# parthjaggi/flow

Hardware: AMD Instinct MI355X
Metric: env-steps/sec (higher is better)
Workload: dtype mixed

## Files before the change

flow_amd/build.py:

```python
import concurrent.futures
import hashlib
import os
import shutil
import subprocess

PKG = os.path.dirname(os.path.abspath(__file__))
ROOT = os.path.dirname(PKG)
CSRC = os.path.join(PKG, "csrc")
SRC = os.path.join(CSRC, "flowsim.hip")
PART = os.path.join(CSRC, "flowsim_part.hip")
OBJ = os.path.join(CSRC, "_obj")
LIB = os.path.join(PKG, "libflowsim.so")

VALIDATED_ROCM = "7.2"

HEADERS = ["flowsim_sim.h", "flowsim_launch.h", "flowsim_kernels.h", "flowsim_open.h", "flowsim_wide.h",
           "flowsim_pair.h", "flowsim_pair_step_a.inc", "flowsim_pair_step_a_sm.inc", "flowsim_fig8.h", "flowsim_ringrl.h", "flowsim_policy.h", "flowsim_queue.h", "flowsim_queue_consts.h", "flowsim_dropq.h",
           "flowsim_part.hip"]
DEPS = [SRC] + [os.path.join(CSRC, h) for h in HEADERS] + [os.path.join(ROOT, "include", "flowsim.h")]
assert all(os.path.exists(d) for d in DEPS)
_known = set(os.path.basename(d) for d in DEPS)
assert all(f in _known for f in os.listdir(CSRC) if f.endswith((".h", ".inc", ".hip"))), "flow_amd/build.py: a source under csrc/ is not in DEPS"

COMMON_FLAGS = ["--offload-arch=gfx950", "-O3", "-ffp-contract=off", "-std=c++17", "-Wall", "-Wno-unused-function"]
HIPCC_FLAGS = COMMON_FLAGS + ["-fPIC", "-shared"]


def parts():
    out = [("main", SRC, [])]
    for t, tn in (("float", "f32"), ("double", "f64")):
        for seg in (8, 16, 32, 64):
            out.append(("seg%d_%s" % (seg, tn), PART, ["-DFS_PART_T=" + t, "-DFS_PART_SEG=%d" % seg]))
        for w in (2, 4):
            out.append(("wide%d_%s" % (w, tn), PART, ["-DFS_PART_T=" + t, "-DFS_PART_WIDE=%d" % w]))
    out.append(("queue_f32", PART, ["-DFS_PART_T=float", "-DFS_PART_QUEUE=1"] +
                (["-DFS_QDIAG=1"] if os.environ.get("FLOWSIM_QDIAG") else [])))
    return out


def find_hipcc():
    for cand in (os.environ.get("HIPCC"), shutil.which("hipcc"), "/opt/rocm/bin/hipcc"):
        if cand and os.path.exists(cand):
            return cand
    raise RuntimeError("hipcc not found: libflowsim.so cannot be built (no CPU fallback exists)")


def include_flags():
    return ["-I" + os.path.join(ROOT, "include"), "-I" + CSRC]


def _stamp(extra):
    h = hashlib.sha256()
    for d in DEPS:
        h.update(os.path.relpath(d, ROOT).encode())
        with open(d, "rb") as f:
            h.update(hashlib.sha256(f.read()).digest())
    h.update(" ".join(COMMON_FLAGS + extra).encode())
    return h.hexdigest()[:16]


def _have_stamp(out):
    if not (os.path.exists(out) and os.path.exists(out + ".stamp")):
        return None
    with open(out + ".stamp") as f:
        return f.read().strip()


def needs_build():
    if not os.path.exists(LIB):
        return True
    t = os.path.getmtime(LIB)
    if any(os.path.getmtime(d) > t for d in DEPS):
        return True
    return any(_have_stamp(os.path.join(OBJ, name + ".o")) != _stamp(extra) for name, _, extra in parts())


def _compile(job):
    name, src, extra, out, verbose = job
    cmd = [find_hipcc()] + COMMON_FLAGS + ["-fPIC", "-c"] + extra + include_flags() + ["-o", out + ".tmp", src]
    if verbose:
        print(" ".join(cmd), flush=True)
    res = subprocess.run(cmd, capture_output=True, text=True)
    if res.returncode != 0:
        raise RuntimeError("hipcc failed (%s):\n%s%s" % (name, res.stdout, res.stderr))
    os.replace(out + ".tmp", out)
    return out


def _jobs():
    return max(1, min(len(parts()), int(os.environ.get("FLOWSIM_BUILD_JOBS", os.cpu_count() or 4))))


def build_variant(lib, defines, names=None, verbose=False):
    build()
    obj_dir = os.path.join(OBJ, os.path.basename(lib))
    os.makedirs(obj_dir, exist_ok=True)
    objs, todo = [], []
    for name, src, extra in parts():
        if names and name not in names:
            objs.append(os.path.join(OBJ, name + ".o"))
            continue
        out = os.path.join(obj_dir, name + ".o")
        objs.append(out)
        todo.append((name, src, extra + list(defines), out, verbose))
    with concurrent.futures.ThreadPoolExecutor(_jobs()) as pool:
        list(pool.map(_compile, todo))
    res = subprocess.run([find_hipcc(), "--offload-arch=gfx950", "-shared", "-fPIC", "-o", lib] + objs,
                         capture_output=True, text=True)
    if res.returncode != 0:
        raise RuntimeError("hipcc link failed:\n" + res.stdout + res.stderr)
    return lib


def build(force=False, verbose=False, only=None):
    if not force and not only and not needs_build():
        return LIB
    os.makedirs(OBJ, exist_ok=True)
    objs, todo, stamps = [], [], {}
    for name, src, extra in parts():
        out = os.path.join(OBJ, name + ".o")
        stamp, have = _stamp(extra), _have_stamp(out)
        objs.append(out)
        if force or (only and name in only) or (not only and have != stamp) or not os.path.exists(out):
            todo.append((name, src, extra, out, verbose))
            stamps[out] = stamp
    with concurrent.futures.ThreadPoolExecutor(_jobs()) as pool:
        for out in pool.map(_compile, todo):
            with open(out + ".stamp", "w") as f:
                f.write(stamps[out])
    cmd = [find_hipcc(), "--offload-arch=gfx950", "-shared", "-fPIC", "-o", LIB + ".tmp"] + objs
    if verbose:
        print(" ".join(cmd), flush=True)
    res = subprocess.run(cmd, capture_output=True, text=True)
    if res.returncode != 0:
        raise RuntimeError("hipcc link failed:\n" + res.stdout + res.stderr)
    os.replace(LIB + ".tmp", LIB)
    return LIB


USER_DIR = os.path.join(PKG, "_user")
USER_SIGNATURE = ("template <typename T>\n__device__ __forceinline__ T fs_user_accel(T v, T v_lead, T h, bool has_lead, "
                  "T v_follow, T h_follow, T dt, T max_accel, const T* p)")


def user_header(body):
    body = "\n".join("  " + ln.strip() for ln in str(body).strip().splitlines())
    return ("// generated by flow_amd.build.build_user -- the get_accel of a flow_amd.controllers.CompiledController\n"
            "%s {\n%s\n}\n" % (USER_SIGNATURE, body))


def build_user(body, verbose=False):
    text = user_header(body)
    tag = hashlib.sha256((text + _stamp([])).encode()).hexdigest()[:16]
    out_dir = os.path.join(USER_DIR, tag)
    lib = os.path.join(out_dir, "libflowsim.so")
    if os.path.exists(lib):
        return lib
    build()
    if not all(os.path.exists(os.path.join(OBJ, name + ".o")) for name, _, _ in parts()):
        build(force=True)
    os.makedirs(out_dir, exist_ok=True)
    for stale in os.listdir(USER_DIR):
        tagfile = os.path.join(USER_DIR, stale, "sources.stamp")
        if stale != tag and os.path.exists(tagfile) and open(tagfile).read().strip() != _stamp([]):
            shutil.rmtree(os.path.join(USER_DIR, stale), ignore_errors=True)
    with open(os.path.join(out_dir, "sources.stamp"), "w") as f:
        f.write(_stamp([]))
    hdr = os.path.join(out_dir, "user_controller.h")
    with open(hdr, "w") as f:
        f.write(text)
    objs, todo = [], []
    for name, src, extra in parts():
        if name.startswith("queue"):
            objs.append(os.path.join(OBJ, name + ".o"))
            continue
        out = os.path.join(out_dir, name + ".o")
        objs.append(out)
        todo.append((name, src, extra + ['-DFS_USER_CONTROLLER_HEADER="%s"' % hdr], out, verbose))
    with concurrent.futures.ThreadPoolExecutor(_jobs()) as pool:
        list(pool.map(_compile, todo))
    res = subprocess.run([find_hipcc(), "--offload-arch=gfx950", "-shared", "-fPIC", "-o", lib + ".tmp"] + objs,
                         capture_output=True, text=True)
    if res.returncode != 0:
        raise RuntimeError("hipcc link failed:\n" + res.stdout + res.stderr)
    os.replace(lib + ".tmp", lib)
    for job in todo:
        os.remove(job[3])
    return lib


def device_asm(out_dir, names=None):
    os.makedirs(out_dir, exist_ok=True)
    jobs = []
    for name, src, extra in parts():
        if names and name not in names:
            continue
        out = os.path.join(out_dir, name + ".s")
        jobs.append((name, [find_hipcc()] + COMMON_FLAGS + ["-S", "--cuda-device-only"] + extra + include_flags() +
                     ["-o", out, src], out))

    def run(job):
        res = subprocess.run(job[1], capture_output=True, text=True)
        if res.returncode != 0:
            raise RuntimeError("hipcc -S failed (%s):\n%s" % (job[0], res.stderr[-2000:]))
        return job[0], job[2]

    with concurrent.futures.ThreadPoolExecutor(_jobs()) as pool:
        return dict(pool.map(run, jobs))


if __name__ == "__main__":
    import sys
    print(build(force="--force" in sys.argv, verbose=True, only=[a for a in sys.argv[1:] if not a.startswith("-")]))
```

flow_amd/csrc/flowsim.hip:

```cpp
#include "flowsim_sim.h"

namespace fsim {

int validate(const fs_config* c) {
  if (!c) return fail(FS_ERR_INVALID, "fs_create: cfg is NULL");
  if (c->struct_size != sizeof(fs_config))
    return fail(FS_ERR_INVALID, "fs_create: struct_size mismatch (header/library out of sync)");
  if (c->abi_version != FS_ABI_VERSION) return fail(FS_ERR_INVALID, "fs_create: abi_version mismatch");
  if (c->precision != FS_F32 && c->precision != FS_F64 && c->precision != FS_MIXED && c->precision != FS_F16S)
    return fail(FS_ERR_INVALID, "fs_create: bad precision");
  if (c->precision == FS_F16S && (c->network != FS_NET_MERGE || c->num_vehicles > 64))
    return fail(FS_ERR_UNSUPPORTED, "fs_create: FS_F16S (half state, float32 integrator) is built for FS_NET_MERGE "
                                    "(k_steps_open, <= 64 vehicle slots)");
  if (c->precision == FS_MIXED && (c->network == FS_NET_MERGE || c->network == FS_NET_BOTTLENECK)) {
  } else if (c->precision == FS_MIXED) {
    const bool fig8 = c->network == FS_NET_FIGURE_EIGHT;
    const char* why = nullptr;
    if ((c->network != FS_NET_RING && !fig8) || c->num_lanes > 1) why = "network (single-lane ring or figure eight)";
    else if (c->env != FS_ENV_ACCEL && c->env != FS_ENV_WAVE_ATTENUATION_PO) why = "env (AccelEnv or WaveAttenuationPOEnv)";
    else if (c->evaluate) why = "evaluate";
    else if (c->sims_per_step != 1) why = "sims_per_step (1)";
    else if (c->integrator != FS_EULER) why = "integrator (Euler)";
    else if (c->junction_mode && !fig8) why = "junction_mode";
    else if (c->track_aux && !fig8) why = "track_aux (the scalar Env's previous-speed / acceleration fields: VecFlowEnv(track_aux=False))";
    else if (c->sort_vehicles || c->obs_perm) why = "sort_vehicles / shuffled ids";
    else if (!fig8 && (c->num_vehicles < 2 || c->num_vehicles > 64 || (c->num_vehicles % 2) != 0)) why = "num_vehicles (even, 2..64)";
    else if (!c->vehicles) why = "vehicles (NULL)";
    for (int i = 0; !why && i < c->num_vehicles; ++i) {
      const fs_vehicle_spec& v = c->vehicles[i];
      if (v.controller != FS_CTRL_IDM && v.controller != FS_CTRL_RL && !(fig8 && v.controller == FS_CTRL_SIM))
        why = "vehicles[].controller (IDMController / RLController)";
      else if (v.fail_safe != FS_FAILSAFE_NONE) why = "vehicles[].fail_safe";
    }
    if (why)
      return fail(FS_ERR_UNSUPPORTED, std::string("fs_create: FS_MIXED does not support this configuration: ") + why);
  }
  if (c->network < FS_NET_RING || c->network > FS_NET_BOTTLENECK)
    return fail(FS_ERR_UNSUPPORTED, "fs_create: network not built");
  const bool open_net = c->network == FS_NET_MERGE || c->network == FS_NET_BOTTLENECK;
  const bool merge_env = c->env == FS_ENV_MERGE_PO || c->env == FS_ENV_MERGE_MA;
  const bool bn_env = c->env == FS_ENV_BOTTLENECK_DV || c->env == FS_ENV_BOTTLENECK;
  if ((c->network == FS_NET_MERGE) != merge_env)
    return fail(FS_ERR_INVALID, "fs_create: the merge envs and FS_NET_MERGE go together");
  if (c->network == FS_NET_MERGE && !c->track_followers)
    return fail(FS_ERR_INVALID, "fs_create: the merge observations need track_followers = 1");
  if ((c->network == FS_NET_BOTTLENECK) != bn_env)
    return fail(FS_ERR_INVALID, "fs_create: the bottleneck envs and FS_NET_BOTTLENECK go together");
  if (c->network == FS_NET_BOTTLENECK) {
    if (c->num_vehicles <= 32)
      return fail(FS_ERR_UNSUPPORTED, "fs_create: the bottleneck heads need more than 32 vehicle slots per replica");
    if (!(c->merge1_x <= c->merge2_x) || !(c->merge2_x < c->end_x) || !(c->zipper_distance >= 0))
      return fail(FS_ERR_INVALID, "fs_create: need merge1_x <= merge2_x < end_x and zipper_distance >= 0");
    if (c->junction.enabled) return fail(FS_ERR_INVALID, "fs_create: the priority-junction model is for FS_NET_MERGE");
    if (c->obs_outflow_window < 1 || c->obs_outflow_window > 20 || c->reward_outflow_window < 1 ||
        c->reward_outflow_window > 20)
      return fail(FS_ERR_INVALID, "fs_create: outflow windows must be 1..20 sub-steps");
    if (c->evaluate) return fail(FS_ERR_UNSUPPORTED, "fs_create: evaluate mode of the bottleneck envs is not built");
    if (c->num_paths != 0 && c->num_paths != 4 && c->num_paths != 8)
      return fail(FS_ERR_UNSUPPORTED, "fs_create: num_paths (4 * scaling) must be 4 or 8");
    if (c->num_paths == 8 && c->num_vehicles <= 64)
      return fail(FS_ERR_UNSUPPORTED, "fs_create: num_paths = 8 (scaling 2) is built in the workgroup-per-replica kernel: "
                                      "more than 64 vehicle slots per replica");
    if (c->env == FS_ENV_BOTTLENECK_DV) {
      const int max_cells = c->num_vehicles > 64 ? 128 : 64;
      if (c->num_obs_cells < 1 || c->num_obs_cells > max_cells || !c->obs_cells)
        return fail(FS_ERR_INVALID, "fs_create: 1..64 observation cells (1..128 with more than 64 vehicle slots)");
      for (int k = 0; k < c->num_obs_cells; ++k)
        if (c->obs_cells[k].lane < 0 || c->obs_cells[k].lane > 63) return fail(FS_ERR_INVALID, "fs_create: cell lane");
      for (int k = 0; k < c->num_rl; ++k)
        if (c->act_cells && (c->act_cells[k].lane < 0 || c->act_cells[k].lane > 63))
          return fail(FS_ERR_INVALID, "fs_create: cell lane");
      if (c->num_rl < 0 || c->num_rl > 64 || (c->num_rl > 0 && !c->act_cells))
        return fail(FS_ERR_INVALID, "fs_create: 0..64 action cells");
    }
  }
  if (open_net) {
    if (c->num_lanes > 1) return fail(FS_ERR_UNSUPPORTED, "fs_create: multi-lane merge is not built");
    if (c->num_segments < 2 || c->num_segments > 2 * FS_MAX_SEGMENTS || !c->segments)
      return fail(FS_ERR_INVALID, "fs_create: FS_NET_MERGE needs the segment tables of both routes");
    int per_route[2] = {0, 0};
    for (int k = 0; k < c->num_segments; ++k) {
      const fs_segment& sg = c->segments[k];
      if (sg.route < 0 || sg.route > (c->network == FS_NET_MERGE ? 1 : 0))
        return fail(FS_ERR_INVALID, "fs_create: segment route out of range");
      if (k > 0 && sg.route < c->segments[k - 1].route)
        return fail(FS_ERR_INVALID, "fs_create: segment rows must be grouped by route");
      if (k > 0 && sg.route == c->segments[k - 1].route && !(sg.start > c->segments[k - 1].start))
        return fail(FS_ERR_INVALID, "fs_create: segment starts must increase");
      if (++per_route[sg.route] > FS_MAX_SEGMENTS) return fail(FS_ERR_INVALID, "fs_create: too many segments");
    }
    if (!per_route[0] || (c->network == FS_NET_MERGE && !per_route[1]))
      return fail(FS_ERR_INVALID, "fs_create: a route has no segment");
    if (c->num_inflows < 0 || c->num_inflows > FS_MAX_INFLOWS || (c->num_inflows > 0 && !c->inflows))
      return fail(FS_ERR_INVALID, "fs_create: bad inflow table");
    for (int f = 0; f < c->num_inflows; ++f) {
      const fs_inflow& fl = c->inflows[f];
      if (c->network == FS_NET_MERGE ? (fl.route < 0 || fl.route > 1)
                                     : (fl.route < -1 || fl.route > (c->num_paths == 8 ? 7 : 3)))
        return fail(FS_ERR_INVALID, "fs_create: inflow route out of range");
      if (fl.probability > 1.0) return fail(FS_ERR_INVALID, "fs_create: inflow probability > 1");
      if (!(fl.probability >= 0.0) && !(fl.period > 0)) return fail(FS_ERR_INVALID, "fs_create: inflow period <= 0");
      if (!(fl.depart_speed >= 0) || !(fl.depart_pos >= 0)) return fail(FS_ERR_INVALID, "fs_create: bad inflow departure");
      bool type_ok = false;
      for (int i = 0; i < c->num_vehicles; ++i) type_ok = type_ok || c->vehicles[i].type == fl.type;
      if (!type_ok) return fail(FS_ERR_INVALID, "fs_create: inflow of a vehicle type that has no slot");
    }
    if (!c->init_alive || !c->init_lane) return fail(FS_ERR_INVALID, "fs_create: FS_NET_MERGE needs init_alive and init_lane (routes)");
    if (!(c->box_in < c->merge_x) || !(c->merge_x < c->end_x) || !(c->net_length > 0))
      return fail(FS_ERR_INVALID, "fs_create: need box_in < merge_x < end_x and net_length > 0");
  }
  if (c->network == FS_NET_RING && (c->num_segments != 0 || c->junction.enabled))
    return fail(FS_ERR_INVALID, "fs_create: a ring takes no segment table / junction");
  if (c->network == FS_NET_FIGURE_EIGHT) {
    if (c->num_segments < 1 || c->num_segments > FS_MAX_SEGMENTS || !c->segments)
      return fail(FS_ERR_INVALID, "fs_create: figure eight needs 1..FS_MAX_SEGMENTS segments");
    if (c->num_lanes > 1) return fail(FS_ERR_UNSUPPORTED, "fs_create: multi-lane figure eight is not built");
    if (c->segments[0].start != 0.0) return fail(FS_ERR_INVALID, "fs_create: segment 0 must start at 0");
    for (int k = 1; k < c->num_segments; ++k)
      if (!(c->segments[k].start > c->segments[k - 1].start))
        return fail(FS_ERR_INVALID, "fs_create: segment starts must increase");
  }
  if (c->env < FS_ENV_ACCEL || c->env > FS_ENV_LANE_CHANGE_ACCEL_PO) return fail(FS_ERR_INVALID, "fs_create: bad env");
  const bool lc_env = c->env == FS_ENV_LANE_CHANGE_ACCEL || c->env == FS_ENV_LANE_CHANGE_ACCEL_PO;
  if (lc_env && c->network != FS_NET_RING)
    return fail(FS_ERR_UNSUPPORTED, "fs_create: the lane-change envs are built for rings (k_steps_ml)");
  if (c->env == FS_ENV_LANE_CHANGE_ACCEL_PO && (c->num_rl < 1 || c->obs_perm))
    return fail(FS_ERR_INVALID, "fs_create: LaneChangeAccelPOEnv needs an RL vehicle and takes no observation permutation");
  if (c->env == FS_ENV_WAVE_ATTENUATION_PO_MA || c->env == FS_ENV_ACCEL_PO_MA) {
    if (open_net || c->num_lanes > 1)
      return fail(FS_ERR_UNSUPPORTED, "fs_create: the multi-agent ring heads are built for single-lane closed loops");
    if (c->num_rl < 1) return fail(FS_ERR_INVALID, "fs_create: a multi-agent ring env needs an RL vehicle");
    if (c->sort_vehicles || c->obs_perm) return fail(FS_ERR_INVALID, "fs_create: sort_vehicles / shuffled ids belong to AccelEnv");
  }
  if (c->num_lanes > 1 && c->env == FS_ENV_WAVE_ATTENUATION_PO)
    return fail(FS_ERR_UNSUPPORTED, "fs_create: WaveAttenuationPOEnv on a multi-lane ring is not built");
  if (c->num_lanes > 64) return fail(FS_ERR_INVALID, "fs_create: num_lanes > 64");
  if (c->init_lane && !open_net)
    for (size_t e = 0; e < size_t(c->num_replicas > 0 ? c->num_replicas : 0) * (c->num_vehicles > 0 ? c->num_vehicles : 0); ++e)
      if (c->init_lane[e] < 0 || c->init_lane[e] >= (c->num_lanes < 1 ? 1 : c->num_lanes))
        return fail(FS_ERR_INVALID, "fs_create: init_lane out of range");
  if (c->num_replicas < 1) return fail(FS_ERR_INVALID, "fs_create: num_replicas < 1");
  if (c->replica_offset < 0) return fail(FS_ERR_INVALID, "fs_create: replica_offset < 0");
  if (c->sort_vehicles || c->obs_perm) {
    if (c->env != FS_ENV_ACCEL && !lc_env && c->sort_vehicles)
      return fail(FS_ERR_INVALID, "fs_create: sort_vehicles belongs to AccelEnv / LaneChangeAccelEnv");
    if (c->network == FS_NET_MERGE || c->network == FS_NET_BOTTLENECK ||
        (c->num_lanes > 1 && c->sort_vehicles && !lc_env))
      return fail(FS_ERR_UNSUPPORTED, "fs_create: sort_vehicles / shuffled ids are built for closed loops "
                                      "(sort_vehicles on multi-lane rings: LaneChangeAccelEnv)");
    if (c->obs_perm) {
      unsigned long long seen = 0ull;
      for (int i = 0; i < c->num_vehicles && i < 64; ++i) {
        const int q = c->obs_perm[i];
        if (q < 0 || q >= c->num_vehicles || (seen >> q) & 1ull)
          return fail(FS_ERR_INVALID, "fs_create: obs_perm is not a permutation");
        seen |= 1ull << q;
      }
    }
  }
  if (c->num_vehicles < 1) return fail(FS_ERR_INVALID, "fs_create: num_vehicles < 1");
  if (c->num_vehicles > 64 && c->network != FS_NET_BOTTLENECK)
    return fail(FS_ERR_UNSUPPORTED, "fs_create: more than 64 vehicles per replica is built for FS_NET_BOTTLENECK only");
  if (c->num_vehicles > FS_MAX_SLOTS_WIDE)
    return fail(FS_ERR_UNSUPPORTED, "fs_create: more than 256 vehicle slots per replica is not built");
  if (c->num_rl < 0 || (c->num_rl > c->num_vehicles && c->env != FS_ENV_BOTTLENECK_DV))
    return fail(FS_ERR_INVALID, "fs_create: bad num_rl");
  if (c->sims_per_step < 1) return fail(FS_ERR_INVALID, "fs_create: sims_per_step < 1");
  if (c->warmup_steps < 0) return fail(FS_ERR_INVALID, "fs_create: warmup_steps < 0");
  if (!(c->sim_step > 0)) return fail(FS_ERR_INVALID, "fs_create: sim_step <= 0");
  if (!(c->slowdown_ramp > 0) || c->slowdown_ramp > 1) return fail(FS_ERR_INVALID, "fs_create: slowdown_ramp not in (0,1]");
  if (c->junction_length < 0) return fail(FS_ERR_INVALID, "fs_create: junction_length < 0");
  if (!c->vehicles || (!c->ring_length && !open_net) || !c->init_pos)
    return fail(FS_ERR_INVALID, "fs_create: NULL table pointer");
  int seen_rl = 0;
  unsigned long long rl_mask = 0ull;
  for (int i = 0; i < c->num_vehicles; ++i) {
    const fs_vehicle_spec& v = c->vehicles[i];
    if (v.controller < FS_CTRL_SIM || v.controller > FS_CTRL_USER)
      return fail(FS_ERR_INVALID, "fs_create: unknown controller id");
    if (v.fail_safe < FS_FAILSAFE_NONE || v.fail_safe > FS_FAILSAFE_SAFE_VELOCITY)
      return fail(FS_ERR_INVALID, "fs_create: unknown fail_safe id");
    if (open_net && v.controller == FS_CTRL_PISATURATION)
      return fail(FS_ERR_UNSUPPORTED, "fs_create: PISaturation on an open network is not built");
    if (v.controller == FS_CTRL_RL && (c->env == FS_ENV_MERGE_PO || bn_env)) {
      ++seen_rl;
    } else if (v.controller == FS_CTRL_RL) {
      if (v.rl_index < 0 || v.rl_index >= c->num_rl) return fail(FS_ERR_INVALID, "fs_create: rl_index out of range");
      if (rl_mask & (1ull << v.rl_index)) return fail(FS_ERR_INVALID, "fs_create: rl_index used twice");
      rl_mask |= 1ull << v.rl_index;
      ++seen_rl;
    }
    if (!(v.length > 0)) return fail(FS_ERR_INVALID, "fs_create: vehicle length <= 0");
  }
  if (c->env == FS_ENV_MERGE_PO && c->num_rl > 32)
    return fail(FS_ERR_UNSUPPORTED, "fs_create: MergePOEnv with more than 32 controlled places (num_rl) is not built");
  if (seen_rl != c->num_rl && c->env != FS_ENV_MERGE_PO && !bn_env)
    return fail(FS_ERR_INVALID, "fs_create: num_rl does not match the RL slots");
  if (open_net) {
    for (size_t e = 0; e < size_t(c->num_replicas) * c->num_vehicles; ++e) {
      if (!c->init_alive[e]) continue;
      const int rt = c->init_lane[e];
      if (rt < 0 || rt > (c->network == FS_NET_MERGE ? 1 : (c->num_paths == 8 ? 7 : 3)))
        return fail(FS_ERR_INVALID, "fs_create: initial route out of range");
      const double x = c->init_pos[e];
      if (!(x >= c->route_start[c->network == FS_NET_MERGE ? rt : 0]) || !(x < c->end_x))
        return fail(FS_ERR_INVALID, "fs_create: init_pos outside the route");
    }
    return FS_OK;
  }
  if (c->env == FS_ENV_WAVE_ATTENUATION_PO && c->num_rl < 1)
    return fail(FS_ERR_INVALID, "fs_create: WaveAttenuationPOEnv needs an RL vehicle");
  for (int r = 0; r < c->num_replicas; ++r) {
    double need = 0;
    for (int i = 0; i < c->num_vehicles; ++i) need += c->vehicles[i].length;
    const double L = c->ring_length[r] + 4 * c->junction_length;
    if (!(c->ring_length[r] > 0) || need > L * (c->num_lanes < 1 ? 1 : c->num_lanes))
      return fail(FS_ERR_NOSPACE, "fs_create: vehicles do not fit on the ring");
    for (int i = 0; i < c->num_vehicles; ++i) {
      const double x = c->init_pos[size_t(r) * c->num_vehicles + i];
      if (!(x >= 0) || !(x < L)) return fail(FS_ERR_INVALID, "fs_create: init_pos outside [0, length)");
    }
  }
  return FS_OK;
}

template <typename T>
int create_typed(const fs_config* cfg, fs_handle* out) {
  Sim<T>* s = new (std::nothrow) Sim<T>();
  if (!s) return fail(FS_ERR_HIP, "fs_create: out of host memory");
  s->cfg = *cfg;
  s->mixed = cfg->precision == FS_MIXED;
  s->f16s = cfg->precision == FS_F16S;
  s->veh.assign(cfg->vehicles, cfg->vehicles + cfg->num_vehicles);
  if (cfg->num_segments > 0) s->segs.assign(cfg->segments, cfg->segments + cfg->num_segments);
  if (cfg->obs_perm) s->obs_perm.assign(cfg->obs_perm, cfg->obs_perm + cfg->num_vehicles);
  if (cfg->network == FS_NET_MERGE || cfg->network == FS_NET_BOTTLENECK) {
    if (cfg->num_inflows > 0) s->inflows.assign(cfg->inflows, cfg->inflows + cfg->num_inflows);
    s->init_alive.assign(cfg->init_alive, cfg->init_alive + size_t(cfg->num_replicas) * cfg->num_vehicles);
    if (cfg->env == FS_ENV_BOTTLENECK_DV) {
      s->obs_cells.assign(cfg->obs_cells, cfg->obs_cells + cfg->num_obs_cells);
      if (cfg->num_rl > 0) s->act_cells.assign(cfg->act_cells, cfg->act_cells + cfg->num_rl);
    }
  }
  s->obs_dim = (cfg->env == FS_ENV_WAVE_ATTENUATION_PO) ? 3
               : (cfg->env == FS_ENV_WAVE_ATTENUATION_PO_MA) ? 3 * cfg->num_rl
               : (cfg->env == FS_ENV_ACCEL_PO_MA) ? 6 * cfg->num_rl
               : (cfg->env == FS_ENV_BOTTLENECK_DV) ? 4 * cfg->num_obs_cells + 1
               : (cfg->env == FS_ENV_BOTTLENECK) ? 1
               : (cfg->env == FS_ENV_MERGE_PO || cfg->env == FS_ENV_MERGE_MA)
                     ? 5 * cfg->num_rl
                     : (cfg->env == FS_ENV_LANE_CHANGE_ACCEL_PO)
                           ? (4 * (cfg->num_lanes < 1 ? 1 : cfg->num_lanes) + 1) * cfg->num_rl
                           : (cfg->env == FS_ENV_LANE_CHANGE_ACCEL ? 3 : 2) * cfg->num_vehicles;
  if (s->obs_dim < 1) s->obs_dim = 1;
  s->act_dim = cfg->num_rl * ((cfg->env == FS_ENV_LANE_CHANGE_ACCEL || cfg->env == FS_ENV_LANE_CHANGE_ACCEL_PO) ? 2 : 1);
  int seg = 8;
  while (seg < cfg->num_vehicles) seg <<= 1;
  s->seg = seg;
  hipError_t e = hipSetDevice(cfg->device);
  if (e == hipSuccess) e = hipStreamCreateWithFlags(&s->own_stream, hipStreamNonBlocking);
  if (e != hipSuccess) {
    delete s;
    return fail(FS_ERR_HIP, std::string("fs_create: no usable HIP device: ") + hipGetErrorString(e));
  }
  s->stream = s->own_stream;
  {
    const std::pair<const char*, bool SimBase::*> switches[] = {
        {"FLOWSIM_FORCE_GENERIC", &SimBase::force_generic}, {"FLOWSIM_NO_FASTDIV", &SimBase::no_fastdiv},
        {"FLOWSIM_NO_LOOP_KERNEL", &SimBase::no_loop_kernel}, {"FLOWSIM_NO_LOOP_FULL", &SimBase::no_loop_full},
        {"FLOWSIM_NO_RING_RL", &SimBase::no_ring_rl}, {"FLOWSIM_NO_QUEUE", &SimBase::no_queue},
        {"FLOWSIM_NO_PAIR", &SimBase::no_pair}};
    for (const auto& sw : switches) {
      const char* v = std::getenv(sw.first);
      s->*sw.second = v && v[0] == '1';
    }
  }
  int rc = s->init();
  if (rc == FS_OK) {
    hipError_t e2 = hipStreamSynchronize(s->stream);
    if (e2 != hipSuccess) rc = fail(FS_ERR_HIP, std::string("fs_create: ") + hipGetErrorString(e2));
  }
  if (rc != FS_OK) {
    for (void* p : s->allocs) (void)hipFree(p);
    (void)hipStreamDestroy(s->own_stream);
    delete s;
    return rc;
  }
  s->cfg.vehicles = nullptr;
  s->cfg.ring_length = nullptr;
  s->cfg.init_pos = nullptr;
  s->cfg.init_vel = nullptr;
  s->cfg.init_lane = nullptr;
  s->cfg.segments = nullptr;
  s->cfg.inflows = nullptr;
  s->cfg.init_alive = nullptr;
  s->cfg.obs_cells = nullptr;
  s->cfg.obs_perm = nullptr;
  s->cfg.act_cells = nullptr;
  *out = reinterpret_cast<fs_handle>(static_cast<SimBase*>(s));
  return FS_OK;
}

inline SimBase* S(fs_handle h) { return reinterpret_cast<SimBase*>(h); }

struct DeviceGuard {
  int prev = -1;
  bool switched = false;
  explicit DeviceGuard(int want) {
    if (hipGetDevice(&prev) == hipSuccess && prev != want) switched = hipSetDevice(want) == hipSuccess;
  }
  ~DeviceGuard() {
    if (switched) (void)hipSetDevice(prev);
  }
};

}

using namespace fsim;

extern "C" {

int fs_abi_version(void) { return FS_ABI_VERSION; }

const char* fs_last_error(void) { return g_err.c_str(); }

int fs_create(const fs_config* cfg, fs_handle* out) {
  if (!out) return fail(FS_ERR_INVALID, "fs_create: out is NULL");
  *out = nullptr;
  int rc = validate(cfg);
  if (rc) return rc;
  int prev = -1;
  const bool have_prev = hipGetDevice(&prev) == hipSuccess;
  rc = (cfg->precision == FS_F32 || cfg->precision == FS_F16S) ? create_typed<float>(cfg, out)
                                                                 : create_typed<double>(cfg, out);
  if (have_prev && prev != cfg->device) (void)hipSetDevice(prev);
  return rc;
}

void fs_destroy(fs_handle h) {
  if (!h) return;
  SimBase* s = S(h);
  DeviceGuard guard(s->cfg.device);
  (void)hipStreamSynchronize(s->stream);
  for (void* p : s->allocs) (void)hipFree(p);
  (void)hipStreamDestroy(s->own_stream);
  delete s;
}

int fs_obs_dim(fs_handle h) { return h ? S(h)->obs_dim : fail(FS_ERR_INVALID, "fs_obs_dim: NULL handle"); }

int fs_action_dim(fs_handle h) { return h ? S(h)->act_dim : fail(FS_ERR_INVALID, "fs_action_dim: NULL handle"); }

int fs_set_stream(fs_handle h, void* hip_stream) {
  if (!h) return fail(FS_ERR_INVALID, "fs_set_stream: NULL handle");
  SimBase* s = S(h);
  DeviceGuard guard(s->cfg.device);
  HIP_TRY(hipStreamSynchronize(s->stream));
  s->stream = static_cast<hipStream_t>(hip_stream);
  return FS_OK;
}

int fs_use_own_stream(fs_handle h) {
  if (!h) return fail(FS_ERR_INVALID, "fs_use_own_stream: NULL handle");
  SimBase* s = S(h);
  DeviceGuard guard(s->cfg.device);
  HIP_TRY(hipStreamSynchronize(s->stream));
  s->stream = s->own_stream;
  return FS_OK;
}

int fs_sync(fs_handle h) {
  if (!h) return fail(FS_ERR_INVALID, "fs_sync: NULL handle");
  DeviceGuard guard(S(h)->cfg.device);
  HIP_TRY(hipStreamSynchronize(S(h)->stream));
  return S(h)->check_qflag();
}

int fs_reset_dev(fs_handle h, const uint8_t* mask_dev, float* obs_dev) {
  if (!h) return fail(FS_ERR_INVALID, "fs_reset_dev: NULL handle");
  SimBase* s = S(h);
  DeviceGuard guard(s->cfg.device);
  int rc = s->launch_reset(mask_dev);
  if (rc) return rc;
  float* obs = obs_dev ? obs_dev : s->d_obs;
  if (s->cfg.network == FS_NET_MERGE || s->cfg.network == FS_NET_BOTTLENECK) {
    s->after_reset = 1;
    rc = s->launch_steps(0, mask_dev, nullptr, 0, obs, s->d_rew, s->d_done, 0);
    s->after_reset = 0;
    if (rc) return rc;
    if (s->cfg.warmup_steps > 0)
      return s->launch_steps(s->cfg.warmup_steps, mask_dev, nullptr, 0, obs, s->d_rew, s->d_done, 0);
    return FS_OK;
  }
  if (s->cfg.warmup_steps > 0)
    return s->launch_steps(s->cfg.warmup_steps, mask_dev, nullptr, 0, obs, s->d_rew, s->d_done, 0);
  return s->launch_steps(0, mask_dev, nullptr, 0, obs, s->d_rew, s->d_done, 0);
}

int fs_reset(fs_handle h, const uint8_t* mask, float* obs_out) {
  if (!h) return fail(FS_ERR_INVALID, "fs_reset: NULL handle");
  SimBase* s = S(h);
  DeviceGuard guard(s->cfg.device);
  const size_t R = size_t(s->cfg.num_replicas);
  const uint8_t* dmask = nullptr;
  if (mask) {
    HIP_TRY(hipMemcpyAsync(s->d_mask, mask, R, hipMemcpyHostToDevice, s->stream));
    dmask = s->d_mask;
  }
  int rc = fs_reset_dev(h, dmask, s->d_obs);
  if (rc) return rc;
  if (obs_out)
    HIP_TRY(hipMemcpyAsync(obs_out, s->d_obs, R * s->obs_dim * sizeof(float), hipMemcpyDeviceToHost, s->stream));
  HIP_TRY(hipStreamSynchronize(s->stream));
  return FS_OK;
}

int fs_step_dev(fs_handle h, const float* actions_dev, float* obs_dev, float* rew_dev, uint8_t* done_dev) {
  if (!h) return fail(FS_ERR_INVALID, "fs_step_dev: NULL handle");
  if (!obs_dev || !rew_dev || !done_dev) return fail(FS_ERR_INVALID, "fs_step_dev: NULL output pointer");
  DeviceGuard guard(S(h)->cfg.device);
  return S(h)->launch_steps(1, nullptr, actions_dev, 0, obs_dev, rew_dev, done_dev, 0);
}

int fs_step(fs_handle h, const float* actions, float* obs, float* rew, uint8_t* done) {
  if (!h) return fail(FS_ERR_INVALID, "fs_step: NULL handle");
  if (!obs || !rew || !done) return fail(FS_ERR_INVALID, "fs_step: NULL output pointer");
  SimBase* s = S(h);
  DeviceGuard guard(s->cfg.device);
  const size_t R = size_t(s->cfg.num_replicas);
  const float* dact = nullptr;
  if (actions && s->act_dim > 0) {
    HIP_TRY(hipMemcpyAsync(s->d_actions, actions, R * s->act_dim * sizeof(float), hipMemcpyHostToDevice, s->stream));
    dact = s->d_actions;
  }
  int rc = s->launch_steps(1, nullptr, dact, 0, s->d_obs, s->d_rew, s->d_done, 0);
  if (rc) return rc;
  HIP_TRY(hipMemcpyAsync(obs, s->d_obs, R * s->obs_dim * sizeof(float), hipMemcpyDeviceToHost, s->stream));
  HIP_TRY(hipMemcpyAsync(rew, s->d_rew, R * sizeof(float), hipMemcpyDeviceToHost, s->stream));
  HIP_TRY(hipMemcpyAsync(done, s->d_done, R, hipMemcpyDeviceToHost, s->stream));
  HIP_TRY(hipStreamSynchronize(s->stream));
  return s->check_qflag();
}

int fs_rollout_dev(fs_handle h, int num_steps, const float* actions_dev, size_t action_stride_steps,
                   float* obs_dev, float* rew_dev, uint8_t* done_dev, int obs_every_step) {
  if (!h) return fail(FS_ERR_INVALID, "fs_rollout_dev: NULL handle");
  if (num_steps < 1) return fail(FS_ERR_INVALID, "fs_rollout_dev: num_steps < 1");
  if (!obs_dev || !rew_dev || !done_dev) return fail(FS_ERR_INVALID, "fs_rollout_dev: NULL output pointer");
  DeviceGuard guard(S(h)->cfg.device);
  return S(h)->launch_steps(num_steps, nullptr, actions_dev, action_stride_steps, obs_dev, rew_dev, done_dev,
                            obs_every_step ? 1 : 0);
}

int fs_get_state(fs_handle h, int field, void* dst, size_t bytes) {
  if (!h || !dst) return fail(FS_ERR_INVALID, "fs_get_state: NULL argument");
  DeviceGuard guard(S(h)->cfg.device);
  return S(h)->get_state(field, dst, bytes);
}

int fs_set_state(fs_handle h, int field, const void* src, size_t bytes) {
  if (!h || !src) return fail(FS_ERR_INVALID, "fs_set_state: NULL argument");
  DeviceGuard guard(S(h)->cfg.device);
  return S(h)->set_state(field, src, bytes);
}

int fs_add_vehicle(fs_handle h, int replica, int slot, int route, double x, double speed) {
  if (!h) return fail(FS_ERR_INVALID, "fs_add_vehicle: NULL handle");
  DeviceGuard guard(S(h)->cfg.device);
  return S(h)->add_vehicle(replica, slot, route, x, speed);
}

int fs_policy_act_dev(fs_handle h, const fs_policy* pol, const float* obs_dev, float* act_dev, float* logp_dev) {
  if (!h || !pol || !obs_dev || !act_dev || !logp_dev) return fail(FS_ERR_INVALID, "fs_policy_act_dev: NULL argument");
  DeviceGuard guard(S(h)->cfg.device);
  return S(h)->launch_policy(pol, 0, 0, obs_dev, nullptr, act_dev, logp_dev, nullptr, nullptr);
}

int fs_policy_rollout_dev(fs_handle h, const fs_policy* pol, int num_steps, int reset_done, float* obs_dev,
                          float* act_dev, float* logp_dev, float* rew_dev, uint8_t* done_dev) {
  if (!h || !pol || !obs_dev || !act_dev || !logp_dev || !rew_dev || !done_dev)
    return fail(FS_ERR_INVALID, "fs_policy_rollout_dev: NULL argument");
  if (num_steps < 1) return fail(FS_ERR_INVALID, "fs_policy_rollout_dev: num_steps < 1");
  DeviceGuard guard(S(h)->cfg.device);
  return S(h)->launch_policy(pol, num_steps, reset_done ? 1 : 0, nullptr, obs_dev, act_dev, logp_dev, rew_dev, done_dev);
}

const char* fs_last_kernel(fs_handle h) { return h ? reinterpret_cast<SimBase*>(h)->last_kernel : ""; }

int fs_dump_trajectory(fs_handle h, int replica, const char* csv_path) {
  if (!h || !csv_path) return fail(FS_ERR_INVALID, "fs_dump_trajectory: NULL argument");
  SimBase* s = S(h);
  if (replica < 0 || replica >= s->cfg.num_replicas) return fail(FS_ERR_INVALID, "fs_dump_trajectory: replica out of range");
  DeviceGuard guard(s->cfg.device);
  const size_t R = size_t(s->cfg.num_replicas), N = size_t(s->cfg.num_vehicles);
  const bool f32 = s->cfg.precision == FS_F32 || s->cfg.precision == FS_F16S;
  const size_t el = f32 ? sizeof(float) : sizeof(double);
  std::vector<char> pos(R * N * el), vel(R * N * el);
  std::vector<int32_t> tc(R), lane(R * N, 0);
  int rc = s->get_state(FS_FIELD_POS, pos.data(), pos.size());
  if (!rc) rc = s->get_state(FS_FIELD_VEL, vel.data(), vel.size());
  if (!rc) rc = s->get_state(FS_FIELD_TIME, tc.data(), R * sizeof(int32_t));
  const bool open_net = s->cfg.network == FS_NET_MERGE || s->cfg.network == FS_NET_BOTTLENECK;
  if (!rc && (open_net || s->cfg.num_lanes > 1))
    rc = s->get_state(open_net ? FS_FIELD_ROUTE : FS_FIELD_LANE, lane.data(), R * N * sizeof(int32_t));
  if (rc) return rc;
  FILE* probe = std::fopen(csv_path, "r");
  const bool fresh = probe == nullptr;
  if (probe) std::fclose(probe);
  FILE* f = std::fopen(csv_path, "a");
  if (!f) return fail(FS_ERR_INVALID, std::string("fs_dump_trajectory: cannot open ") + csv_path);
  if (fresh) std::fprintf(f, "time,id,x,speed,lane_number\n");
  const double t = double(tc[replica]) * s->cfg.sim_step;
  for (size_t i = 0; i < N; ++i) {
    const size_t e = size_t(replica) * N + i;
    if (open_net && lane[e] < 0) continue;
    const double x = f32 ? double(reinterpret_cast<const float*>(pos.data())[e]) : reinterpret_cast<const double*>(pos.data())[e];
    const double v = f32 ? double(reinterpret_cast<const float*>(vel.data())[e]) : reinterpret_cast<const double*>(vel.data())[e];
    std::fprintf(f, "%.6f,%zu,%.17g,%.17g,%d\n", t, i, x, v, int(lane[e]));
  }
  std::fclose(f);
  return FS_OK;
}

}
```

flow_amd/csrc/flowsim_launch.h:

```cpp
#pragma once
#include "flowsim_sim.h"
#ifdef FS_PART_QUEUE
#include "flowsim_queue.h"
#include "flowsim_dropq.h"
#endif

namespace fsim {

#ifdef FS_PART_QUEUE
  template <typename T>
  int Sim<T>::launch_queue(const StepArgs& a) {
    const bool po = dv.env == FS_ENV_MERGE_PO;
    const bool noise = (dv.flags & fs::FLAG_HAS_NOISE) != 0, act = a.actions != nullptr && (po || ov.ma_apply_actions != 0);
    const auto k = pick(noise, [&](auto NZ) {
      return pick(act, [&](auto ACT) {
        return pick(po, [&](auto PO) { return &fs::k_merge_queue<NZ, ACT, false, PO>; });
      });
    });
    last_kernel = "k_merge_queue";
    hipLaunchKernelGGL(k, dim3(dv.R), dim3(64), 0, stream, dv, ov, qc, a.num_steps, a.actions, a.act_stride, a.obs, a.rew,
                       a.done, a.obs_every_step, fs::PolicyView{}, static_cast<float*>(nullptr), static_cast<float*>(nullptr),
                       0);
    return launched();
  }
  template <typename T>
  int Sim<T>::launch_policy_queue(const fs::PolicyView& pv, int num_steps, int reset_done, float* obs, float* act,
                                  float* logp, float* rew, uint8_t* done) {
    const bool noise = (dv.flags & fs::FLAG_HAS_NOISE) != 0;
    if (dv.env == FS_ENV_MERGE_PO) {
      const auto kp = pick(noise, [&](auto NZ) { return &fs::k_merge_policy<NZ>; });
      last_kernel = "k_merge_policy<PO>";
      hipLaunchKernelGGL(kp, dim3(dv.R), dim3(64), 0, stream, dv, ov, qc, num_steps, obs, rew, done, pv, act, logp,
                         reset_done);
      return launched();
    }
    const auto k = pick(noise, [&](auto NZ) { return &fs::k_merge_queue<NZ, true, true>; });
    last_kernel = "k_merge_policy";
    hipLaunchKernelGGL(k, dim3(dv.R), dim3(64), 0, stream, dv, ov, qc, num_steps, static_cast<const float*>(nullptr),
                       size_t(0), obs, rew, done, 1, pv, act, logp, reset_done);
    return launched();
  }
  template <typename T>
  int Sim<T>::launch_policy_act_vec(const fs::PolicyView& pv, const float* obs_in, float* act, float* logp) {
    last_kernel = "k_policy_act_vec";
    hipLaunchKernelGGL(fs::k_policy_act_vec<16>, dim3(dv.R), dim3(64), 0, stream, pv, dv.R, dv.num_rl, dv.rep0, obs_in,
                       act, logp);
    return launched();
  }
  template <typename T>
  int Sim<T>::launch_dropq(const StepArgs& a) {
    const auto k = dv.env == FS_ENV_BOTTLENECK_DV ? &fs::k_drop_queue<true> : &fs::k_drop_queue<false>;
    last_kernel = "k_drop_queue";
    qflag_armed = true;
    hipLaunchKernelGGL(k, dim3(dv.R), dim3(256), 0, stream, dv, ov, qc, d_qflag, a.num_steps, a.actions, a.act_stride,
                       a.obs, a.rew, a.done, a.obs_every_step);
    return launched();
  }
#endif

  template <typename T>
  template <int W>
  int Sim<T>::launch_wide(const StepArgs& a) {
    constexpr int C1 = std::is_same<T, float>::value ? 1 : 0;
    const bool cset = C1 == 1 && (dv.flags & fs::FLAG_IDM_SET) && !force_generic && open_div_ok;
    const auto k = cfg.num_paths == 8 ? (cset ? &fs::k_steps_wide<T, W, C1, 8> : &fs::k_steps_wide<T, W, 0, 8>)
                                      : (cset ? &fs::k_steps_wide<T, W, C1, 4> : &fs::k_steps_wide<T, W, 0, 4>);
    last_kernel = "k_steps_wide";
    hipLaunchKernelGGL(k, dim3(dv.R), dim3(64 * W), 0, stream, dv, ov, a.num_steps, a.mask, a.actions, a.act_stride, a.obs,
                       a.rew, a.done, a.obs_every_step, after_reset);
    return launched();
  }

  template <typename T>
  template <int SEG>
  int Sim<T>::launch_open(const StepArgs& a) {
    constexpr int RPW = 64 / SEG;
    const bool idm_set = (dv.flags & fs::FLAG_IDM_SET) && !force_generic;
    const bool cset = std::is_same<T, float>::value ? idm_set && open_div_ok : idm_set && !mixed;
    const bool mset = mixed && idm_set && open_div_ok;
    constexpr int C2 = std::is_same<T, double>::value ? 2 : 0;
    auto kernel = [&](auto P, auto PO) {
      return pick(ov.n_prob > 0, [&](auto PR) {
        return cset ? &fs::k_steps_open<T, SEG, P, 1, PR, PO>
                    : mset ? &fs::k_steps_open<T, SEG, P, C2, PR, PO> : &fs::k_steps_open<T, SEG, P, 0, PR, PO>;
      });
    };
    decltype(kernel(Int<2>(), std::false_type())) k;
    last_kernel = "k_steps_open";
    if (cfg.network == FS_NET_BOTTLENECK) {
      if constexpr (SEG == 64) k = kernel(Int<4>(), std::false_type());
      else return fail(FS_ERR_UNSUPPORTED, "fs_step: FS_NET_BOTTLENECK runs on 64-lane segments only");
    } else {
      k = pick(dv.env == FS_ENV_MERGE_PO, [&](auto PO) { return kernel(Int<2>(), PO); });
      if (mset) last_kernel = "k_steps_open<mixed>";
    }
    hipLaunchKernelGGL(k, dim3((dv.R + RPW - 1) / RPW), dim3(64), 0, stream, dv, ov, a.num_steps, a.mask, a.actions,
                       a.act_stride, a.obs, a.rew, a.done, a.obs_every_step, after_reset);
    return launched();
  }

  template <typename T>
  template <int SEG>
  int Sim<T>::launch_ml(const StepArgs& a) {
    constexpr int RPW = 64 / SEG;
    const bool lcpo = dv.env == FS_ENV_LANE_CHANGE_ACCEL_PO;
    const auto k = pick(dv.lc_enabled, [&](auto LC) {
      return pick(lcpo, [&](auto PO) { return &fs::k_steps_ml<T, SEG, LC, PO>; });
    });
    last_kernel = "k_steps_ml";
    hipLaunchKernelGGL(k, dim3((dv.R + RPW - 1) / RPW), dim3(64), 0, stream, dv, a.num_steps, a.mask, a.actions,
                       a.act_stride, a.obs, a.rew, a.done, a.obs_every_step);
    return launched();
  }

  template <typename T>
  int Sim<T>::launch_loop(const StepArgs& a) {
    constexpr bool MX = !std::is_same<T, float>::value;
    const int f = dv.flags;
    const bool full = (f & fs::FLAG_HAS_NOISE) && (f & fs::FLAG_NEED_SUMO) && dv.junction_on && a.actions != nullptr &&
                      loop_delta4 && !no_loop_full && loop_fastc_ok();
    auto kernel = [&](auto H) {
      return full ? &fs::k_rollout_loop<H, true, true, MX>
                  : loop_delta4 ? &fs::k_rollout_loop<H, true, false, MX> : &fs::k_rollout_loop<H, false, false, MX>;
    };
    auto k = dv.env == FS_ENV_ACCEL ? kernel(Int<0>()) : kernel(Int<1>());
    last_kernel = full ? "k_rollout_loop<FULL>" : "k_rollout_loop";
    if constexpr (!MX) {
      if (dv.env == FS_ENV_ACCEL_PO_MA) {
        k = kernel(Int<2>());
        last_kernel = full ? "k_rollout_loop<FULL,AccelMA>" : "k_rollout_loop<AccelMA>";
      }
    }
    const int waves = (dv.R + 3) / 4;
    hipLaunchKernelGGL(k, dim3((waves + 3) / 4), dim3(256), 0, stream, dv, a.num_steps, a.actions, a.act_stride, a.obs,
                       a.rew, a.done);
    return launched();
  }

  template <typename T>
  template <int SEG>
  int Sim<T>::launch_ring(const StepArgs& a) {
    constexpr int ROW = SEG >= 16 ? SEG / 2 : 8;
    const bool fast = ringrl_fast_ok();
    const bool po = dv.env == FS_ENV_WAVE_ATTENUATION_PO;
    const bool ma_head = dv.env == FS_ENV_WAVE_ATTENUATION_PO_MA || dv.env == FS_ENV_ACCEL_PO_MA;
    const bool mc = ROW == 16 && std::is_same<T, float>::value && (ma_head || (a.actions != nullptr && dv.num_rl > 1));
    auto kernel = [&](auto H, auto MC) {
      return pick(dv.flags & fs::FLAG_HAS_NOISE, [&](auto NZ) {
        return pick(fast, [&](auto FA) { return &fs::k_ring_pair<T, ROW, H, NZ, FA, MC>; });
      });
    };
    auto single = [&](auto MC) { return po ? kernel(Int<1>(), MC) : kernel(Int<0>(), MC); };
    decltype(single(std::false_type())) k;
    if constexpr (std::is_same<T, float>::value && ROW == 16) {
      const auto MC = std::true_type();
      k = !ma_head ? pick(mc, single) : dv.env == FS_ENV_ACCEL_PO_MA ? kernel(Int<3>(), MC) : kernel(Int<2>(), MC);
    } else if constexpr (std::is_same<T, float>::value) {
      const auto MC = std::false_type();
      k = !ma_head ? single(MC) : dv.env == FS_ENV_ACCEL_PO_MA ? kernel(Int<3>(), MC) : kernel(Int<2>(), MC);
    } else {
      k = single(std::false_type());
    }
    last_kernel = ma_head ? (dv.env == FS_ENV_ACCEL_PO_MA ? "k_ring_pair<AccelMA>" : "k_ring_pair<POMA>")
                          : (po ? "k_ring_pair<PO>" : "k_ring_pair<Accel>");
    const int waves = (dv.R + (64 / ROW) - 1) / (64 / ROW);
    hipLaunchKernelGGL(k, dim3((waves + 3) / 4), dim3(256), 0, stream, dv, a.num_steps, a.mask, a.actions, a.act_stride,
                       a.obs, a.rew, a.done, a.obs_every_step);
    return launched();
  }

  template <typename T>
  int Sim<T>::launch_obs_mixed(const StepArgs& a) {
    if constexpr (std::is_same<T, double>::value) {
      const int n = dv.R * dv.N;
      last_kernel = "k_obs_mixed";
      hipLaunchKernelGGL((fs::k_obs_mixed<T>), dim3((n + 255) / 256), dim3(256), 0, stream, dv, a.obs);
      return launched();
    } else {
      return fail(FS_ERR_UNSUPPORTED, "k_obs_mixed is a float64 kernel");
    }
  }

  template <typename T>
  template <int SEG>
  int Sim<T>::launch_pair(const StepArgs& a) {
    constexpr int ROW = SEG >= 16 ? SEG / 2 : 8;
    const bool fd = fastdiv_ok(), bc = neg_speed_possible, sm = speed_mode_any;
    const bool noise = std::is_same<T, float>::value && (dv.flags & fs::FLAG_HAS_NOISE);
    auto clamped = [&](auto SM, auto NZ) {
      return delta4 && fd && !bc ? &fs::k_rollout_pair<T, ROW, true, true, false, SM, NZ>
                                 : &fs::k_rollout_pair<T, ROW, false, false, true, SM, NZ>;
    };
    decltype(&fs::k_rollout_pair<T, ROW, false, false, true>) k = nullptr;
    if (noise) {
      if constexpr (std::is_same<T, float>::value) k = pick(sm, [&](auto SM) { return clamped(SM, std::true_type()); });
    } else if (sm) {
      k = clamped(std::true_type(), std::false_type());
    } else {
      k = pick(bc, [&](auto BC) {
        return delta4 && fd ? &fs::k_rollout_pair<T, ROW, true, true, BC>
                            : delta4 ? &fs::k_rollout_pair<T, ROW, true, false, BC> : &fs::k_rollout_pair<T, ROW, false, false, BC>;
      });
    }
    last_kernel = noise ? (sm ? "k_rollout_pair+speed_mode+noise" : "k_rollout_pair+noise")
                        : (sm ? "k_rollout_pair+speed_mode" : "k_rollout_pair");
    const int waves = (dv.R + (64 / ROW) - 1) / (64 / ROW);
    hipLaunchKernelGGL(k, dim3((waves + 3) / 4), dim3(256), 0, stream, dv, a.num_steps, a.obs, a.rew, a.done);
    return launched();
  }

  template <typename T>
  template <int SEG>
  int Sim<T>::launch_idm(const StepArgs& a) {
    constexpr int RPW = 64 / SEG;
    const bool fd = fastdiv_ok();
    const auto k = pick(neg_speed_possible, [&](auto BC) {
      return delta4 && fd ? &fs::k_rollout_idm<T, SEG, true, true, BC>
                          : delta4 ? &fs::k_rollout_idm<T, SEG, true, false, BC> : &fs::k_rollout_idm<T, SEG, false, false, BC>;
    });
    last_kernel = "k_rollout_idm";
    const int waves = (dv.R + RPW - 1) / RPW;
    hipLaunchKernelGGL(k, dim3((waves + 7) / 8), dim3(512), 0, stream, dv, a.num_steps, a.obs, a.rew, a.done, d_dump);
    return launched();
  }

  template <typename T>
  template <int SEG>
  int Sim<T>::launch_k_steps(const StepArgs& a) {
    constexpr int RPW = 64 / SEG;
    auto k = &fs::k_steps<T, SEG, 0, 0>;
    last_kernel = "k_steps";
    if (fast_ok(a)) {
      k = &fs::k_steps<T, SEG, 1, 0>;
      last_kernel = "k_steps<FAST>";
    } else if ((dv.flags & fs::FLAG_IDM_SET) && !force_generic) {
      k = &fs::k_steps<T, SEG, 0, 1>;
      last_kernel = "k_steps<CSET>";
    }
    hipLaunchKernelGGL(k, dim3((dv.R + RPW - 1) / RPW), dim3(64), 0, stream, dv, a.num_steps, a.mask, a.actions,
                       a.act_stride, a.obs, a.rew, a.done, a.obs_every_step);
    return launched();
  }

  template <typename T>
  int Sim<T>::launch_policy_act(const fs::PolicyView& pv, int n_ag, const float* obs_in, float* act, float* logp) {
    last_kernel = "k_policy_act";
    const bool merge = dv.env == FS_ENV_MERGE_MA;
    hipLaunchKernelGGL(fs::k_policy_act<16>, dim3((dv.R * 16 + 255) / 256), dim3(256), 0, stream, pv, dv.R, n_ag, dv.rep0,
                       obs_in, act, logp, merge ? static_cast<const int*>(dv.lane) : nullptr,
                       merge ? static_cast<const int*>(dv.ctrl) : nullptr,
                       merge ? static_cast<const int*>(dv.rl_index) : nullptr, dv.N);
    return launched();
  }

  template <typename T>
  int Sim<T>::launch_policy_row16(const fs::PolicyView& pv, int num_steps, int reset_done, float* obs, float* act,
                                  float* logp, float* rew, uint8_t* done) {
    const bool fast = ringrl_fast_ok();
    auto kernel = [&](auto H) {
      return pick(dv.flags & fs::FLAG_HAS_NOISE, [&](auto NZ) {
        return pick(fast, [&](auto FA) { return &fs::k_ring_policy<T, H, NZ, FA>; });
      });
    };
    auto k = kernel(Int<1>());
    last_kernel = "k_ring_policy";
    if constexpr (std::is_same<T, float>::value) {
      if (dv.env == FS_ENV_WAVE_ATTENUATION_PO_MA) {
        k = kernel(Int<2>());
        last_kernel = "k_ring_policy<POMA>";
      }
    }
    const int waves = (dv.R + 3) / 4;
    hipLaunchKernelGGL(k, dim3((waves + 3) / 4), dim3(256), 0, stream, dv, pv, num_steps, reset_done, cfg.warmup_steps,
                       obs, act, logp, rew, done);
    return launched();
  }

  template <typename T>
  int Sim<T>::launch_policy_loop16(const fs::PolicyView& pv, int num_steps, int reset_done, float* obs, float* act,
                                   float* logp, float* rew, uint8_t* done) {
    if constexpr (std::is_same<T, float>::value) {
      const bool fastc = loop_delta4 && loop_fastc_ok();
      auto kernel = [&](auto H) {
        return fastc ? &fs::k_loop_policy<H, true, true>
                     : loop_delta4 ? &fs::k_loop_policy<H, true, false> : &fs::k_loop_policy<H, false, false>;
      };
      const auto k = dv.env == FS_ENV_WAVE_ATTENUATION_PO ? kernel(Int<1>())
                     : dv.env == FS_ENV_ACCEL_PO_MA ? kernel(Int<2>()) : kernel(Int<0>());
      last_kernel = dv.env == FS_ENV_ACCEL_PO_MA ? "k_loop_policy<AccelMA>" : "k_loop_policy";
      const int waves = (dv.R + 3) / 4;
      hipLaunchKernelGGL(k, dim3((waves + 3) / 4), dim3(256), 0, stream, dv, pv, num_steps, reset_done, obs, act, logp, rew,
                         done);
      return launched();
    } else {
      return fail(FS_ERR_UNSUPPORTED, "k_loop_policy is a float32 kernel");
    }
  }

}
```

flow_amd/csrc/flowsim_pair.h:

```cpp
#pragma once
#include "flowsim_kernels.h"

namespace fs {

typedef float f2 __attribute__((ext_vector_type(2)));
typedef unsigned u2v __attribute__((__vector_size__(8)));

enum : int { DPP_ROW_NEWBCAST0 = 0x150, DPP_ROW_NEWBCAST8 = 0x158 };

__device__ __forceinline__ f2 fma2(f2 a, f2 b, f2 c) { return __builtin_elementwise_fma(a, b, c); }
__device__ __forceinline__ f2 splat(float a) { return f2{a, a}; }

__device__ __forceinline__ f2 pk_mul(f2 a, f2 b) { return a * b; }
__device__ __forceinline__ f2 pk_add(f2 a, f2 b) { return a + b; }
__device__ __forceinline__ f2 pk_sub(f2 a, f2 b) { return a - b; }
__device__ __forceinline__ f2 pk_fma(f2 a, f2 b, f2 c) { return fma2(a, b, c); }
__device__ __forceinline__ f2 pk_fnma(f2 a, f2 b, f2 c) { return fma2(-a, b, c); }
__device__ __forceinline__ float nonneg_else(float x, float y) {
  const unsigned a = __builtin_bit_cast(unsigned, x), b = __builtin_bit_cast(unsigned, y);
  return __builtin_bit_cast(float, min(a, b));
}

template <int ROW>
__device__ __forceinline__ float next_a(float v, bool last, int lane) {
  if (ROW == 16) {
    const float t = dpp<DPP_ROW_SHL1>(v), w = dpp<DPP_ROW_NEWBCAST0>(v);
    return last ? w : t;
  } else if (ROW == 8) {
    const float t = dpp<DPP_ROW_SHL1>(v), w0 = dpp<DPP_ROW_NEWBCAST0>(v), w8 = dpp<DPP_ROW_NEWBCAST8>(v);
    return last ? ((lane & 8) ? w8 : w0) : t;
  } else if (ROW == 32) {
    const float t = dpp<DPP_WAVE_SHL1>(v), w0 = read_lane(v, 0), w1 = read_lane(v, 32);
    return last ? ((lane & 32) ? w1 : w0) : t;
  } else {
    const float t = dpp<DPP_WAVE_SHL1>(v), w = read_lane(v, 0);
    return last ? w : t;
  }
}
template <int ROW>
__device__ __forceinline__ double next_a(double v, bool last, int lane) {
  const unsigned long long b = __builtin_bit_cast(unsigned long long, v);
  const float lo = next_a<ROW>(__builtin_bit_cast(float, unsigned(b)), last, lane);
  const float hi = next_a<ROW>(__builtin_bit_cast(float, unsigned(b >> 32)), last, lane);
  return __builtin_bit_cast(double, ((unsigned long long)__builtin_bit_cast(unsigned, hi) << 32) |
                                        __builtin_bit_cast(unsigned, lo));
}

template <bool FASTDIV>
__device__ __forceinline__ f2 div_const2(f2 x, f2 c, f2 rc) {
  if (FASTDIV) {
    const f2 q0 = pk_mul(x, rc);
    const f2 r = pk_fnma(q0, c, x);
    return pk_fma(r, rc, q0);
  }
  return f2{x.x / c.x, x.y / c.y};
}
__device__ __forceinline__ f2 div_core2(f2 n, f2 d, f2 one) {
  const f2 y0 = {__builtin_amdgcn_rcpf(d.x), __builtin_amdgcn_rcpf(d.y)};
  const f2 e = pk_fnma(d, y0, one);
  const f2 y = pk_fma(e, y0, y0);
  const f2 q0 = pk_mul(n, y);
  const f2 r0 = pk_fnma(d, q0, n);
  const f2 q1 = pk_fma(r0, y, q0);
  const f2 r1 = pk_fnma(d, q1, n);
  return pk_fma(r1, y, q1);
}

template <bool DELTA4, bool FASTDIV>
__device__ __forceinline__ f2 idm_pair(f2 v, f2 vl, f2 h, const f2* p, f2 two_sqrt_ab, f2 rc_ab, f2 rc_v0, f2 one) {
  f2 hh;
  hh.x = tabs(h.x) < 1e-3f ? 1e-3f : h.x;
  hh.y = tabs(h.y) < 1e-3f ? 1e-3f : h.y;
  const f2 num = pk_mul(v, pk_sub(v, vl));
  const f2 dq = div_const2<FASTDIV>(num, two_sqrt_ab, rc_ab);
  const f2 ratio = div_const2<FASTDIV>(v, p[0], rc_v0);
  const f2 dyn = pk_add(pk_mul(v, p[1]), dq);
  f2 s_star;
  s_star.x = tmax(dyn.x, 0.0f);
  s_star.y = tmax(dyn.y, 0.0f);
  s_star = pk_add(p[5], s_star);
  const f2 q = FASTDIV ? div_core2(s_star, hh, one) : f2{s_star.x / hh.x, s_star.y / hh.y};
  f2 pw;
  if (DELTA4) {
    const f2 r2 = pk_mul(ratio, ratio);
    pw = pk_mul(r2, r2);
  } else {
    pw = f2{pow_delta(ratio.x, p[4].x), pow_delta(ratio.y, p[4].y)};
  }
  return pk_mul(p[2], pk_sub(pk_sub(one, pw), pk_mul(q, q)));
}

struct SumoPair {
  f2 tau, min_gap, maxa, smax, rc_smax, ts, rc_ts;
  f2 floor0;
  f2 adt, ddt;
};
template <bool FASTDIV>
__device__ __forceinline__ f2 sumo_acc_pair(f2 v, f2 vl, f2 h, const SumoPair& c, f2 one) {
  f2 gap;
  gap.x = tmax(h.x, 1e-3f);
  gap.y = tmax(h.y, 1e-3f);
  const f2 num = pk_mul(v, pk_sub(v, vl));
  const f2 dq = div_const2<FASTDIV>(num, c.ts, c.rc_ts);
  const f2 dyn = pk_add(pk_mul(v, c.tau), dq);
  f2 ss;
  ss.x = tmax(0.0f, dyn.x);
  ss.y = tmax(0.0f, dyn.y);
  ss = pk_add(c.min_gap, ss);
  const f2 q = FASTDIV ? div_core2(ss, gap, one) : f2{ss.x / gap.x, ss.y / gap.y};
  const f2 r = div_const2<FASTDIV>(v, c.smax, c.rc_smax);
  const f2 r2 = pk_mul(r, r);
  return pk_mul(c.maxa, pk_sub(pk_sub(one, pk_mul(r2, r2)), pk_mul(q, q)));
}

struct PairConsts {
  f2 p0, p1, p2, p5, rc_v0, tsab, rc_ab, one, dt2, ramp2, L2, rc_L2, len_lead, gap2, vmask, tvm;
  float c1e3;
  double ms64, rc_ms64;
  unsigned long long last_mask;
};
#define FS_PAIR_A_NAME pair_step_asm_a
#define FS_PAIR_A_NZ 0
#define FS_PAIR_A_NZ_PARAM
#include "flowsim_pair_step_a.inc"
#undef FS_PAIR_A_NAME
#undef FS_PAIR_A_NZ
#undef FS_PAIR_A_NZ_PARAM
#define FS_PAIR_A_NAME pair_step_asm_a_nz
#define FS_PAIR_A_NZ 1
#define FS_PAIR_A_NZ_PARAM , f2 nz
#include "flowsim_pair_step_a.inc"
#undef FS_PAIR_A_NAME
#undef FS_PAIR_A_NZ
#undef FS_PAIR_A_NZ_PARAM
#define FS_PAIR_A_NAME pair_step_asm_a_sm
#define FS_PAIR_A_NZ 0
#define FS_PAIR_A_NZ_PARAM
#include "flowsim_pair_step_a_sm.inc"
#undef FS_PAIR_A_NAME
#undef FS_PAIR_A_NZ
#undef FS_PAIR_A_NZ_PARAM
#define FS_PAIR_A_NAME pair_step_asm_a_sm_nz
#define FS_PAIR_A_NZ 1
#define FS_PAIR_A_NZ_PARAM , f2 nz
#include "flowsim_pair_step_a_sm.inc"
#undef FS_PAIR_A_NAME
#undef FS_PAIR_A_NZ
#undef FS_PAIR_A_NZ_PARAM
__device__ __forceinline__ void pair_step_asm_b(f2& V, f2& X, f2& H, f2& DVL, f2& OV, unsigned& crash_bits, float& sq,
                                                const PairConsts& c) {
  asm volatile(
      "v_sub_f32_e32 v118, v112, v113\n"
      "v_sub_f32_e32 v132, v115, v114\n"
      "v_subrev_f32_dpp v119, v112, v113 row_shl:1 row_mask:0xf bank_mask:0xf bound_ctrl:1\n"
      "v_subrev_f32_dpp v134, v112, v113 row_newbcast:0 row_mask:0xf bank_mask:0xf\n"
      "v_sub_f32_dpp v133, v114, v115 row_shl:1 row_mask:0xf bank_mask:0xf bound_ctrl:1\n"
      "v_sub_f32_dpp v135, v114, v115 row_newbcast:0 row_mask:0xf bank_mask:0xf\n"
      "v_cndmask_b32_e64 v119, v119, v134, %[last]\n"
      "v_cndmask_b32_e64 v133, v133, v135, %[last]\n"
      "v_pk_add_f32 v[126:127], v[132:133], %[L2]\n"
      "v_min_u32_e32 v132, v132, v126\n"
      "v_min_u32_e32 v133, v133, v127\n"
      "v_pk_add_f32 v[116:117], v[132:133], %[lenlead] neg_lo:[0,1] neg_hi:[0,1]\n"
      "v_pk_add_f32 v[126:127], v[116:117], %[gap2] neg_lo:[0,1] neg_hi:[0,1]\n"
      "v_min_f32_e32 v126, v126, v127\n"
      "v_alignbit_b32 %[cb], %[cb], v126, 31\n"
      "v_pk_fma_f32 v[124:125], v[112:113], %[vmask], %[tvm]\n"
      "v_pk_mul_f32 v[124:125], v[124:125], v[124:125]\n"
      "v_add_f32_e32 %[sq], v124, v125\n"
      "v_cvt_f64_f32_e32 v[130:131], v112\n"
      "v_cvt_f64_f32_e32 v[132:133], v113\n"
      "v_mul_f64 v[134:135], v[130:131], %[rcms]\n"
      "v_mul_f64 v[136:137], v[132:133], %[rcms]\n"
      "v_fma_f64 v[130:131], -v[134:135], %[ms], v[130:131]\n"
      "v_fma_f64 v[132:133], -v[136:137], %[ms], v[132:133]\n"
      "v_fma_f64 v[134:135], v[130:131], %[rcms], v[134:135]\n"
      "v_fma_f64 v[136:137], v[132:133], %[rcms], v[136:137]\n"
      "v_cvt_f32_f64_e32 v128, v[134:135]\n"
      "v_cvt_f32_f64_e32 v129, v[136:137]\n"
      : "+{v[112:113]}"(V), "+{v[114:115]}"(X), "+{v[116:117]}"(H), "+{v[118:119]}"(DVL), "={v[128:129]}"(OV),
        [cb] "+v"(crash_bits), [sq] "=&v"(sq)
      : [L2] "v"(c.L2), [lenlead] "v"(c.len_lead), [gap2] "v"(c.gap2), [vmask] "v"(c.vmask), [tvm] "v"(c.tvm),
        [ms] "v"(c.ms64), [rcms] "v"(c.rc_ms64), [last] "s"(c.last_mask)
      : "v124", "v125", "v126", "v127", "v130", "v131", "v132", "v133", "v134", "v135", "v136", "v137");
}

struct MixedConsts {
  f2 p0, p1, p2, p5, rc_v0, tsab, rc_ab, one, gap2, vmask, tvm;
  float c1e3;
  double dt, ramp, L, rc_L, rc_ms, len_b, len_next, zero;
  unsigned long long last_mask;
};
__device__ __forceinline__ void mixed_step_asm_a(f2& V32, double& XA, double& XB, double& VA, double& VB, f2& H, f2& DVL,
                                                 f2& OV, const MixedConsts& c) {
  unsigned long long sa, sb;
  asm volatile(
      "v_cmp_nlt_f32_e64 %[sa], |v140|, %[c1e3]\n"
      "v_cmp_nlt_f32_e64 %[sb], |v141|, %[c1e3]\n"
      "v_pk_mul_f32 v[124:125], v[112:113], v[142:143]\n"
      "v_pk_mul_f32 v[126:127], v[124:125], %[rcab]\n"
      "v_pk_fma_f32 v[130:131], v[126:127], %[tsab], v[124:125] neg_lo:[1,0,0] neg_hi:[1,0,0]\n"
      "v_pk_fma_f32 v[126:127], v[130:131], %[rcab], v[126:127]\n"
      "v_cndmask_b32_e64 v120, %[c1e3], v140, %[sa]\n"
      "v_cndmask_b32_e64 v121, %[c1e3], v141, %[sb]\n"
      "v_pk_mul_f32 v[124:125], v[112:113], %[rcv0]\n"
      "v_rcp_f32_e32 v122, v120\n"
      "v_rcp_f32_e32 v123, v121\n"
      "v_pk_fma_f32 v[130:131], v[124:125], %[p0], v[112:113] neg_lo:[1,0,0] neg_hi:[1,0,0]\n"
      "v_pk_fma_f32 v[124:125], v[130:131], %[rcv0], v[124:125]\n"
      "v_pk_mul_f32 v[130:131], v[112:113], %[p1]\n"
      "v_pk_add_f32 v[130:131], v[130:131], v[126:127]\n"
      "v_pk_fma_f32 v[126:127], v[120:121], v[122:123], %[one] neg_lo:[1,0,0] neg_hi:[1,0,0]\n"
      "v_max_f32_e32 v130, 0, v130\n"
      "v_max_f32_e32 v131, 0, v131\n"
      "v_pk_fma_f32 v[122:123], v[126:127], v[122:123], v[122:123]\n"
      "v_pk_add_f32 v[130:131], %[p5], v[130:131]\n"
      "v_pk_mul_f32 v[124:125], v[124:125], v[124:125]\n"
      "v_pk_mul_f32 v[126:127], v[130:131], v[122:123]\n"
      "v_pk_mul_f32 v[124:125], v[124:125], v[124:125]\n"
      "v_pk_fma_f32 v[132:133], v[120:121], v[126:127], v[130:131] neg_lo:[1,0,0] neg_hi:[1,0,0]\n"
      "v_pk_add_f32 v[124:125], %[one], v[124:125] neg_lo:[0,1] neg_hi:[0,1]\n"
      "v_pk_fma_f32 v[126:127], v[132:133], v[122:123], v[126:127]\n"
      "v_pk_fma_f32 v[132:133], v[120:121], v[126:127], v[130:131] neg_lo:[1,0,0] neg_hi:[1,0,0]\n"
      "v_pk_fma_f32 v[126:127], v[132:133], v[122:123], v[126:127]\n"
      "v_pk_mul_f32 v[126:127], v[126:127], v[126:127]\n"
      "v_pk_add_f32 v[124:125], v[124:125], v[126:127] neg_lo:[0,1] neg_hi:[0,1]\n"
      "v_pk_mul_f32 v[124:125], %[p2], v[124:125]\n"
      "v_cvt_f64_f32_e32 v[130:131], v124\n"
      "v_cvt_f64_f32_e32 v[132:133], v125\n"
      "v_mul_f64 v[130:131], v[130:131], %[dt]\n"
      "v_mul_f64 v[132:133], v[132:133], %[dt]\n"
      "v_add_f64 v[130:131], v[118:119], v[130:131]\n"
      "v_add_f64 v[132:133], v[138:139], v[132:133]\n"
      "v_max_f64 v[130:131], v[130:131], %[zero]\n"
      "v_max_f64 v[132:133], v[132:133], %[zero]\n"
      "v_add_f64 v[130:131], v[130:131], -v[118:119]\n"
      "v_add_f64 v[132:133], v[132:133], -v[138:139]\n"
      "v_mul_f64 v[130:131], v[130:131], %[ramp]\n"
      "v_mul_f64 v[132:133], v[132:133], %[ramp]\n"
      "v_add_f64 v[118:119], v[118:119], v[130:131]\n"
      "v_add_f64 v[138:139], v[138:139], v[132:133]\n"
      "v_mul_f64 v[130:131], v[118:119], %[dt]\n"
      "v_mul_f64 v[132:133], v[138:139], %[dt]\n"
      "v_add_f64 v[130:131], v[114:115], v[130:131]\n"
      "v_add_f64 v[132:133], v[116:117], v[132:133]\n"
      "v_add_f64 v[134:135], v[130:131], -%[L]\n"
      "v_add_f64 v[136:137], v[132:133], -%[L]\n"
      "v_cvt_f32_f64_e32 v112, v[118:119]\n"
      "v_cvt_f32_f64_e32 v113, v[138:139]\n"
      "v_cmp_gt_i32_e64 %[sa], 0, v135\n"
      "v_cmp_gt_i32_e64 %[sb], 0, v137\n"
      "v_mul_f64 v[120:121], v[118:119], %[rcms]\n"
      "v_mul_f64 v[122:123], v[138:139], %[rcms]\n"
      "v_cndmask_b32_e64 v114, v134, v130, %[sa]\n"
      "v_cndmask_b32_e64 v115, v135, v131, %[sa]\n"
      "v_cndmask_b32_e64 v116, v136, v132, %[sb]\n"
      "v_cndmask_b32_e64 v117, v137, v133, %[sb]\n"
      "v_cvt_f32_f64_e32 v128, v[120:121]\n"
      "v_cvt_f32_f64_e32 v129, v[122:123]\n"
      : "+{v[112:113]}"(V32), "+{v[114:115]}"(XA), "+{v[116:117]}"(XB), "+{v[118:119]}"(VA), "+{v[138:139]}"(VB),
        "+{v[140:141]}"(H), "+{v[142:143]}"(DVL), "={v[128:129]}"(OV), [sa] "=&s"(sa), [sb] "=&s"(sb)
      : [c1e3] "v"(c.c1e3), [rcab] "v"(c.rc_ab), [tsab] "v"(c.tsab), [rcv0] "v"(c.rc_v0), [p0] "v"(c.p0),
        [p1] "v"(c.p1), [p2] "v"(c.p2), [p5] "v"(c.p5), [one] "v"(c.one), [dt] "v"(c.dt), [ramp] "v"(c.ramp),
        [L] "v"(c.L), [rcms] "v"(c.rc_ms), [zero] "v"(c.zero)
      : "v120", "v121", "v122", "v123", "v124", "v125", "v126", "v127", "v130", "v131", "v132", "v133", "v134",
        "v135", "v136", "v137");
}
struct MixedSumoConsts { double fl0a, fl0b, adta, adtb, ddta, ddtb; };
__device__ __forceinline__ void mixed_step_asm_a_sm(f2& V32, double& XA, double& XB, double& VA, double& VB, f2& H,
                                                    f2& DVL, f2& OV, const MixedConsts& c, const SumoPair& m,
                                                    const MixedSumoConsts& d) {
  unsigned long long sa, sb;
  asm volatile(
      "v_cmp_nlt_f32_e64 %[sa], |v140|, %[c1e3]\n"
      "v_cmp_nlt_f32_e64 %[sb], |v141|, %[c1e3]\n"
      "v_pk_mul_f32 v[124:125], v[112:113], v[142:143]\n"
      "v_pk_mul_f32 v[126:127], v[124:125], %[rcab]\n"
      "v_pk_mul_f32 v[150:151], v[124:125], %[rcts]\n"
      "v_pk_fma_f32 v[130:131], v[126:127], %[tsab], v[124:125] neg_lo:[1,0,0] neg_hi:[1,0,0]\n"
      "v_pk_fma_f32 v[152:153], v[150:151], %[ts], v[124:125] neg_lo:[1,0,0] neg_hi:[1,0,0]\n"
      "v_pk_fma_f32 v[126:127], v[130:131], %[rcab], v[126:127]\n"
      "v_pk_fma_f32 v[150:151], v[152:153], %[rcts], v[150:151]\n"
      "v_cndmask_b32_e64 v120, %[c1e3], v140, %[sa]\n"
      "v_cndmask_b32_e64 v121, %[c1e3], v141, %[sb]\n"
      "v_max_f32_e32 v146, v140, %[c1e3]\n"
      "v_max_f32_e32 v147, v141, %[c1e3]\n"
      "v_pk_mul_f32 v[124:125], v[112:113], %[rcv0]\n"
      "v_rcp_f32_e32 v122, v120\n"
      "v_rcp_f32_e32 v123, v121\n"
      "v_rcp_f32_e32 v148, v146\n"
      "v_rcp_f32_e32 v149, v147\n"
      "v_pk_fma_f32 v[130:131], v[124:125], %[p0], v[112:113] neg_lo:[1,0,0] neg_hi:[1,0,0]\n"
      "v_pk_mul_f32 v[154:155], v[112:113], %[rcsm]\n"
      "v_pk_fma_f32 v[124:125], v[130:131], %[rcv0], v[124:125]\n"
      "v_pk_fma_f32 v[152:153], v[154:155], %[smax], v[112:113] neg_lo:[1,0,0] neg_hi:[1,0,0]\n"
      "v_pk_mul_f32 v[130:131], v[112:113], %[p1]\n"
      "v_pk_fma_f32 v[154:155], v[152:153], %[rcsm], v[154:155]\n"
      "v_pk_add_f32 v[130:131], v[130:131], v[126:127]\n"
      "v_pk_mul_f32 v[152:153], v[112:113], %[tau]\n"
      "v_pk_fma_f32 v[126:127], v[120:121], v[122:123], %[one] neg_lo:[1,0,0] neg_hi:[1,0,0]\n"
      "v_pk_add_f32 v[150:151], v[152:153], v[150:151]\n"
      "v_pk_fma_f32 v[152:153], v[146:147], v[148:149], %[one] neg_lo:[1,0,0] neg_hi:[1,0,0]\n"
      "v_max_f32_e32 v130, 0, v130\n"
      "v_max_f32_e32 v131, 0, v131\n"
      "v_max_f32_e32 v150, 0, v150\n"
      "v_max_f32_e32 v151, 0, v151\n"
      "v_pk_fma_f32 v[122:123], v[126:127], v[122:123], v[122:123]\n"
      "v_pk_fma_f32 v[148:149], v[152:153], v[148:149], v[148:149]\n"
      "v_pk_add_f32 v[130:131], %[p5], v[130:131]\n"
      "v_pk_add_f32 v[150:151], %[mgap], v[150:151]\n"
      "v_pk_mul_f32 v[124:125], v[124:125], v[124:125]\n"
      "v_pk_mul_f32 v[154:155], v[154:155], v[154:155]\n"
      "v_pk_mul_f32 v[126:127], v[130:131], v[122:123]\n"
      "v_pk_mul_f32 v[152:153], v[150:151], v[148:149]\n"
      "v_pk_mul_f32 v[124:125], v[124:125], v[124:125]\n"
      "v_pk_mul_f32 v[154:155], v[154:155], v[154:155]\n"
      "v_pk_fma_f32 v[132:133], v[120:121], v[126:127], v[130:131] neg_lo:[1,0,0] neg_hi:[1,0,0]\n"
      "v_pk_fma_f32 v[134:135], v[146:147], v[152:153], v[150:151] neg_lo:[1,0,0] neg_hi:[1,0,0]\n"
      "v_pk_add_f32 v[124:125], %[one], v[124:125] neg_lo:[0,1] neg_hi:[0,1]\n"
      "v_pk_add_f32 v[154:155], %[one], v[154:155] neg_lo:[0,1] neg_hi:[0,1]\n"
      "v_pk_fma_f32 v[126:127], v[132:133], v[122:123], v[126:127]\n"
      "v_pk_fma_f32 v[152:153], v[134:135], v[148:149], v[152:153]\n"
      "v_pk_fma_f32 v[132:133], v[120:121], v[126:127], v[130:131] neg_lo:[1,0,0] neg_hi:[1,0,0]\n"
      "v_pk_fma_f32 v[134:135], v[146:147], v[152:153], v[150:151] neg_lo:[1,0,0] neg_hi:[1,0,0]\n"
      "v_pk_fma_f32 v[126:127], v[132:133], v[122:123], v[126:127]\n"
      "v_pk_fma_f32 v[152:153], v[134:135], v[148:149], v[152:153]\n"
      "v_pk_mul_f32 v[126:127], v[126:127], v[126:127]\n"
      "v_pk_mul_f32 v[152:153], v[152:153], v[152:153]\n"
      "v_pk_add_f32 v[124:125], v[124:125], v[126:127] neg_lo:[0,1] neg_hi:[0,1]\n"
      "v_pk_add_f32 v[154:155], v[154:155], v[152:153] neg_lo:[0,1] neg_hi:[0,1]\n"
      "v_pk_mul_f32 v[124:125], %[p2], v[124:125]\n"
      "v_pk_mul_f32 v[154:155], %[maxa], v[154:155]\n"
      "v_cvt_f64_f32_e32 v[130:131], v124\n"
      "v_cvt_f64_f32_e32 v[132:133], v125\n"
      "v_cvt_f64_f32_e32 v[134:135], v154\n"
      "v_cvt_f64_f32_e32 v[136:137], v155\n"
      "v_mul_f64 v[130:131], v[130:131], %[dt]\n"
      "v_mul_f64 v[132:133], v[132:133], %[dt]\n"
      "v_mul_f64 v[134:135], v[134:135], %[dt]\n"
      "v_mul_f64 v[136:137], v[136:137], %[dt]\n"
      "v_add_f64 v[130:131], v[118:119], v[130:131]\n"
      "v_add_f64 v[132:133], v[138:139], v[132:133]\n"
      "v_add_f64 v[134:135], v[118:119], v[134:135]\n"
      "v_add_f64 v[136:137], v[138:139], v[136:137]\n"
      "v_max_f64 v[130:131], v[130:131], %[zero]\n"
      "v_max_f64 v[132:133], v[132:133], %[zero]\n"
      "v_max_f64 v[134:135], v[134:135], %[fl0a]\n"
      "v_max_f64 v[136:137], v[136:137], %[fl0b]\n"
      "v_add_f64 v[130:131], v[130:131], -v[118:119]\n"
      "v_add_f64 v[132:133], v[132:133], -v[138:139]\n"
      "v_mul_f64 v[130:131], v[130:131], %[ramp]\n"
      "v_mul_f64 v[132:133], v[132:133], %[ramp]\n"
      "v_add_f64 v[130:131], v[118:119], v[130:131]\n"
      "v_add_f64 v[132:133], v[138:139], v[132:133]\n"
      "v_min_f64 v[130:131], v[130:131], v[134:135]\n"
      "v_min_f64 v[132:133], v[132:133], v[136:137]\n"
      "v_add_f64 v[134:135], v[118:119], %[adta]\n"
      "v_add_f64 v[136:137], v[138:139], %[adtb]\n"
      "v_min_f64 v[130:131], v[130:131], v[134:135]\n"
      "v_min_f64 v[132:133], v[132:133], v[136:137]\n"
      "v_add_f64 v[134:135], v[118:119], -%[ddta]\n"
      "v_add_f64 v[136:137], v[138:139], -%[ddtb]\n"
      "v_max_f64 v[118:119], v[130:131], v[134:135]\n"
      "v_max_f64 v[138:139], v[132:133], v[136:137]\n"
      "v_mul_f64 v[130:131], v[118:119], %[dt]\n"
      "v_mul_f64 v[132:133], v[138:139], %[dt]\n"
      "v_add_f64 v[130:131], v[114:115], v[130:131]\n"
      "v_add_f64 v[132:133], v[116:117], v[132:133]\n"
      "v_add_f64 v[134:135], v[130:131], -%[L]\n"
      "v_add_f64 v[136:137], v[132:133], -%[L]\n"
      "v_cvt_f32_f64_e32 v112, v[118:119]\n"
      "v_cvt_f32_f64_e32 v113, v[138:139]\n"
      "v_cmp_gt_i32_e64 %[sa], 0, v135\n"
      "v_cmp_gt_i32_e64 %[sb], 0, v137\n"
      "v_mul_f64 v[120:121], v[118:119], %[rcms]\n"
      "v_mul_f64 v[122:123], v[138:139], %[rcms]\n"
      "v_cndmask_b32_e64 v114, v134, v130, %[sa]\n"
      "v_cndmask_b32_e64 v115, v135, v131, %[sa]\n"
      "v_cndmask_b32_e64 v116, v136, v132, %[sb]\n"
      "v_cndmask_b32_e64 v117, v137, v133, %[sb]\n"
      "v_cvt_f32_f64_e32 v128, v[120:121]\n"
      "v_cvt_f32_f64_e32 v129, v[122:123]\n"
      : "+{v[112:113]}"(V32), "+{v[114:115]}"(XA), "+{v[116:117]}"(XB), "+{v[118:119]}"(VA), "+{v[138:139]}"(VB),
        "+{v[140:141]}"(H), "+{v[142:143]}"(DVL), "={v[128:129]}"(OV), [sa] "=&s"(sa), [sb] "=&s"(sb)
      : [c1e3] "v"(c.c1e3), [rcab] "v"(c.rc_ab), [tsab] "v"(c.tsab), [rcv0] "v"(c.rc_v0), [p0] "v"(c.p0),
        [p1] "v"(c.p1), [p2] "v"(c.p2), [p5] "v"(c.p5), [one] "v"(c.one), [dt] "v"(c.dt), [ramp] "v"(c.ramp),
        [L] "v"(c.L), [rcms] "v"(c.rc_ms), [zero] "v"(c.zero), [rcts] "v"(m.rc_ts), [ts] "v"(m.ts),
        [rcsm] "v"(m.rc_smax), [smax] "v"(m.smax), [tau] "v"(m.tau), [mgap] "v"(m.min_gap), [maxa] "v"(m.maxa),
        [fl0a] "v"(d.fl0a), [fl0b] "v"(d.fl0b), [adta] "v"(d.adta), [adtb] "v"(d.adtb), [ddta] "v"(d.ddta),
        [ddtb] "v"(d.ddtb)
      : "v120", "v121", "v122", "v123", "v124", "v125", "v126", "v127", "v130", "v131", "v132", "v133", "v134",
        "v135", "v136", "v137", "v146", "v147", "v148", "v149", "v150", "v151", "v152", "v153", "v154", "v155");
}
__device__ __forceinline__ void mixed_step_asm_b(f2& V32, double& XA, double& XB, f2& H, f2& DVL, f2& OX,
                                                 unsigned& crash_bits, float& sq, const MixedConsts& c) {
  unsigned long long sa, sb;
  asm volatile(
      "v_sub_f32_e32 v142, v112, v113\n"
      "v_subrev_f32_dpp v143, v112, v113 row_shl:1 row_mask:0xf bank_mask:0xf bound_ctrl:1\n"
      "v_subrev_f32_dpp v124, v112, v113 row_newbcast:0 row_mask:0xf bank_mask:0xf\n"
      "v_mov_b32_dpp v130, v114 row_shl:1 row_mask:0xf bank_mask:0xf bound_ctrl:1\n"
      "v_mov_b32_dpp v131, v115 row_shl:1 row_mask:0xf bank_mask:0xf bound_ctrl:1\n"
      "v_mov_b32_dpp v132, v114 row_newbcast:0 row_mask:0xf bank_mask:0xf\n"
      "v_mov_b32_dpp v133, v115 row_newbcast:0 row_mask:0xf bank_mask:0xf\n"
      "v_cndmask_b32_e64 v143, v143, v124, %[last]\n"
      "v_cndmask_b32_e64 v130, v130, v132, %[last]\n"
      "v_cndmask_b32_e64 v131, v131, v133, %[last]\n"
      "v_mul_f64 v[120:121], v[114:115], %[rcL]\n"
      "v_mul_f64 v[122:123], v[116:117], %[rcL]\n"
      "v_add_f64 v[134:135], v[116:117], -v[114:115]\n"
      "v_add_f64 v[136:137], v[130:131], -v[116:117]\n"
      "v_cvt_f32_f64_e32 v144, v[120:121]\n"
      "v_cvt_f32_f64_e32 v145, v[122:123]\n"
      "v_add_f64 v[130:131], v[134:135], %[L]\n"
      "v_add_f64 v[132:133], v[136:137], %[L]\n"
      "v_cmp_gt_i32_e64 %[sa], 0, v135\n"
      "v_cmp_gt_i32_e64 %[sb], 0, v137\n"
      "v_pk_fma_f32 v[124:125], v[112:113], %[vmask], %[tvm]\n"
      "v_pk_mul_f32 v[124:125], v[124:125], v[124:125]\n"
      "v_cndmask_b32_e64 v134, v134, v130, %[sa]\n"
      "v_cndmask_b32_e64 v135, v135, v131, %[sa]\n"
      "v_cndmask_b32_e64 v136, v136, v132, %[sb]\n"
      "v_cndmask_b32_e64 v137, v137, v133, %[sb]\n"
      "v_add_f32_e32 %[sq], v124, v125\n"
      "v_add_f64 v[134:135], v[134:135], -%[lenb]\n"
      "v_add_f64 v[136:137], v[136:137], -%[lennext]\n"
      "v_cvt_f32_f64_e32 v140, v[134:135]\n"
      "v_cvt_f32_f64_e32 v141, v[136:137]\n"
      "v_pk_add_f32 v[126:127], v[140:141], %[gap2] neg_lo:[0,1] neg_hi:[0,1]\n"
      "v_min_f32_e32 v126, v126, v127\n"
      "v_alignbit_b32 %[cb], %[cb], v126, 31\n"
      : "+{v[112:113]}"(V32), "+{v[114:115]}"(XA), "+{v[116:117]}"(XB), "+{v[140:141]}"(H), "+{v[142:143]}"(DVL),
        "={v[144:145]}"(OX), [cb] "+v"(crash_bits), [sq] "=&v"(sq), [sa] "=&s"(sa), [sb] "=&s"(sb)
      : [L] "v"(c.L), [rcL] "v"(c.rc_L), [gap2] "v"(c.gap2), [vmask] "v"(c.vmask), [tvm] "v"(c.tvm),
        [lenb] "v"(c.len_b), [lennext] "v"(c.len_next), [last] "s"(c.last_mask)
      : "v120", "v121", "v122", "v123", "v124", "v125", "v126", "v127", "v130", "v131", "v132", "v133", "v134",
        "v135", "v136", "v137");
}

template <typename T, int ROW, bool DELTA4, bool FASTDIV, bool BADCHK, bool SM = false, bool NOISE = false>
__global__ __launch_bounds__(256) void k_rollout_pair(DevView<T> s, int num_steps, float* __restrict__ obs,
                                                      float* __restrict__ rew, uint8_t* __restrict__ done) {
  constexpr bool MIXED = sizeof(T) == 8;
  static_assert(!(NOISE && MIXED), "FS_MIXED has no noise form (its C twin cannot reproduce the hardware's log / cos)");
  constexpr bool ASM = ROW == 16 && DELTA4 && FASTDIV && !BADCHK;
  constexpr int RPW = 64 / ROW;
  constexpr int PERIOD = ROW < 16 ? ROW : 16;
  const int lane = threadIdx.x & 63;
  const int wave = (blockIdx.x * blockDim.x + threadIdx.x) >> 6;
  const int row = lane / ROW;
  const int k = lane % ROW;
  const int r = wave * RPW + row;
  const int N = s.N;
  const int LP = N >> 1;
  const bool rvalid = r < s.R;
  const bool valid = rvalid && k < LP;
  const int rr = rvalid ? r : s.R - 1;
  const int kk = k < LP ? k : LP - 1;
  const bool last = (kk == LP - 1);
  const int iA = 2 * kk, iB = iA + 1;
  const size_t idx = size_t(rr) * N + iA;

  f2 p[6];
#pragma unroll
  for (int q = 0; q < 6; ++q) p[q] = f2{float(s.p[q * N + iA]), float(s.p[q * N + iB])};
  const T lenB = s.length[iB];
  const T len_nextA = next_a<ROW>(T(s.length[iA]), last, lane);
  const T base_len = s.ring_len[rr];
  const T L = base_len + T(4) * s.jlen;
  int tcount = s.time[rr];
  uint32_t nctr = NOISE ? s.noise_ctr[rr] : 0u;
  const f2 sigma = NOISE ? f2{float(s.noise[iA]), float(s.noise[iB])} : f2{0.0f, 0.0f};
  const bool noisyA = NOISE && sigma.x > 0.0f, noisyB = NOISE && sigma.y > 0.0f;
  float gA[4] = {0.0f, 0.0f, 0.0f, 0.0f}, gB[4] = {0.0f, 0.0f, 0.0f, 0.0f};
  if constexpr (NOISE) {
    if ((nctr & 3u) != 0u) {
      gauss4<float>(s.seed_lo, s.seed_hi, s.rep0 + uint32_t(rr), uint32_t(iA), nctr >> 2, gA, s.noise_exact != 0);
      gauss4<float>(s.seed_lo, s.seed_hi, s.rep0 + uint32_t(rr), uint32_t(iB), nctr >> 2, gB, s.noise_exact != 0);
      for (uint32_t q = 0; q < (nctr & 3u); ++q) {
        gA[0] = gA[1]; gA[1] = gA[2]; gA[2] = gA[3];
        gB[0] = gB[1]; gB[1] = gB[2]; gB[2] = gB[3];
      }
    }
  }

  const float dt = float(s.dt), ramp = float(s.ramp);
  const f2 two_sqrt_ab = {2.0f * tsqrt(p[2].x * p[3].x), 2.0f * tsqrt(p[2].y * p[3].y)};
  const f2 rc_v0 = {1.0f / p[0].x, 1.0f / p[0].y}, rc_ab = {1.0f / two_sqrt_ab.x, 1.0f / two_sqrt_ab.y};
  const float Lf = float(L);
  const f2 L2 = splat(Lf), rc_L2 = splat(1.0f / Lf), one = splat(1.0f), dt2 = splat(dt), ramp2 = splat(ramp);
  const f2 gap2 = splat(float(s.crash_gap)), m100 = splat(-100.0f);
  const f2 vmask = splat(valid ? 1.0f : 0.0f), tvm = splat(valid ? -float(s.target_velocity) : 0.0f);
  const double ms64 = double(s.max_speed), rc_ms64 = 1.0 / ms64;
  const double L64 = double(L), rc_L64 = 1.0 / L64, dt64 = double(s.dt), ramp64 = double(s.ramp);

  f2 x, v;
  double xdA = 0, xdB = 0, vdA = 0, vdB = 0;
  if (MIXED) {
    xdA = double(s.pos[idx]); xdB = double(s.pos[idx + 1]);
    vdA = double(s.vel[idx]); vdB = double(s.vel[idx + 1]);
    v = f2{float(vdA), float(vdB)};
    x = f2{0.0f, 0.0f};
  } else {
    x = f2{float(s.pos[idx]), float(s.pos[idx + 1])};
    v = f2{float(s.vel[idx]), float(s.vel[idx + 1])};
  }
  const f2 len_lead = {float(lenB), float(len_nextA)};

  auto headway = [&]() -> f2 {
    if (MIXED) {
      const double xn = next_a<ROW>(xdA, last, lane);
      double dA = xdB - xdA, dB = xn - xdB;
      dA = dA < 0.0 ? dA + L64 : dA;
      dB = dB < 0.0 ? dB + L64 : dB;
      return f2{float(dA - double(lenB)), float(dB - double(len_nextA))};
    } else {
      const f2 xl = {x.y, next_a<ROW>(x.x, last, lane)};
      f2 d = pk_sub(xl, x);
      const f2 dw = pk_add(d, L2);
      d.x = nonneg_else(d.x, dw.x);
      d.y = nonneg_else(d.y, dw.y);
      return pk_sub(d, len_lead);
    }
  };
  f2 h = headway();
  f2 vl = {v.y, next_a<ROW>(v.x, last, lane)};
  f2 dvl = v - vl;
  PairConsts pc;
  pc.p0 = p[0]; pc.p1 = p[1]; pc.p2 = p[2]; pc.p5 = p[5]; pc.rc_v0 = rc_v0; pc.tsab = two_sqrt_ab; pc.rc_ab = rc_ab;
  pc.one = one; pc.dt2 = dt2; pc.ramp2 = ramp2; pc.L2 = L2; pc.rc_L2 = rc_L2; pc.len_lead = len_lead;
  pc.gap2 = gap2; pc.vmask = vmask; pc.tvm = tvm; pc.c1e3 = 1e-3f; pc.ms64 = ms64; pc.rc_ms64 = rc_ms64;
  pc.last_mask = __ballot(last);
  MixedConsts mc;
  mc.p0 = p[0]; mc.p1 = p[1]; mc.p2 = p[2]; mc.p5 = p[5]; mc.rc_v0 = rc_v0; mc.tsab = two_sqrt_ab; mc.rc_ab = rc_ab;
  mc.one = one; mc.gap2 = gap2; mc.vmask = vmask; mc.tvm = tvm; mc.c1e3 = 1e-3f; mc.dt = dt64; mc.ramp = ramp64;
  mc.L = L64; mc.rc_L = rc_L64; mc.rc_ms = rc_ms64; mc.len_b = double(lenB); mc.len_next = double(len_nextA);
  mc.zero = 0.0; mc.last_mask = pc.last_mask;
  SumoPair sc{};
  double floor0A = 0, floor0B = 0, adtA = 0, adtB = 0, ddtA = 0, ddtB = 0;
  if constexpr (SM) {
    const int mA = s.speed_mode[iA], mB = s.speed_mode[iB];
    const float maA = float(s.max_accel[iA]), maB = float(s.max_accel[iB]);
    const float mdA = float(s.max_decel[iA]), mdB = float(s.max_decel[iB]);
    sc.tau = f2{float(s.sumo_tau[iA]), float(s.sumo_tau[iB])};
    sc.min_gap = f2{float(s.sumo_min_gap[iA]), float(s.sumo_min_gap[iB])};
    sc.maxa = f2{maA, maB};
    sc.smax = f2{float(s.sumo_max_speed[iA]), float(s.sumo_max_speed[iB])};
    sc.rc_smax = f2{1.0f / sc.smax.x, 1.0f / sc.smax.y};
    sc.ts = f2{2.0f * tsqrt(maA * mdA), 2.0f * tsqrt(maB * mdB)};
    sc.rc_ts = f2{1.0f / sc.ts.x, 1.0f / sc.ts.y};
    const float BIG = 3.0e38f;
    sc.floor0 = f2{(mA & 1) ? 0.0f : BIG, (mB & 1) ? 0.0f : BIG};
    sc.adt = f2{(mA & 2) ? maA * dt : BIG, (mB & 2) ? maB * dt : BIG};
    sc.ddt = f2{(mA & 4) ? mdA * dt : BIG, (mB & 4) ? mdB * dt : BIG};
    floor0A = double(sc.floor0.x); floor0B = double(sc.floor0.y);
    adtA = (mA & 2) ? double(s.max_accel[iA]) * dt64 : double(BIG);
    adtB = (mB & 2) ? double(s.max_accel[iB]) * dt64 : double(BIG);
    ddtA = (mA & 4) ? double(s.max_decel[iA]) * dt64 : double(BIG);
    ddtB = (mB & 4) ? double(s.max_decel[iB]) * dt64 : double(BIG);
  }
  const MixedSumoConsts msc = {floor0A, floor0B, adtA, adtB, ddtA, ddtB};

  const unsigned rowb = 2u * unsigned(N) * 4u;
  const unsigned off_v = unsigned(rr) * rowb + unsigned(iA) * 4u;
  const unsigned off_x = off_v + unsigned(N) * 4u;
  const size_t step_bytes = size_t(s.R) * rowb;
  const unsigned step_b32 = unsigned(step_bytes);
  char* ob = reinterpret_cast<char*>(obs);
  unsigned crash_bits = 0u, bad_bits = 0u;

  typedef unsigned u4v __attribute__((__vector_size__(16)));
  constexpr bool XPOSE = ASM;
  __shared__ float row_img[XPOSE ? 4 : 1][XPOSE ? RPW * 64 : 1];
  float* const my_img = row_img[XPOSE ? (threadIdx.x >> 6) & 3 : 0] + (XPOSE ? row * 2 * N : 0);
  const unsigned off_16 = unsigned(rr) * rowb + unsigned(kk) * 16u;
  u4v piece = {0u, 0u, 0u, 0u};
  auto transpose_in = [&](f2 ov, f2 ox) {
    *reinterpret_cast<f2*>(my_img + 2 * kk) = ov;
    *reinterpret_cast<f2*>(my_img + N + 2 * kk) = ox;
    __builtin_amdgcn_fence(__ATOMIC_RELEASE, "wavefront");
    __builtin_amdgcn_wave_barrier();
    __builtin_amdgcn_fence(__ATOMIC_ACQUIRE, "wavefront");
    piece = *reinterpret_cast<const u4v*>(my_img + 4 * kk);
  };

  auto noise_term = [&]() -> f2 {
    f2 nz = {-0.0f, -0.0f};
    if constexpr (NOISE) {
      const bool fresh = (nctr & 3u) == 0u;
      if (__ballot(fresh) != 0ull) {
        if (fresh) {
          gauss4<float>(s.seed_lo, s.seed_hi, s.rep0 + uint32_t(rr), uint32_t(iA), nctr >> 2, gA, s.noise_exact != 0);
          gauss4<float>(s.seed_lo, s.seed_hi, s.rep0 + uint32_t(rr), uint32_t(iB), nctr >> 2, gB, s.noise_exact != 0);
        }
      }
      const float tA = sigma.x * gA[0], tB = sigma.y * gB[0];
      nz.x = noisyA ? tA : -0.0f;
      nz.y = noisyB ? tB : -0.0f;
      gA[0] = gA[1]; gA[1] = gA[2]; gA[2] = gA[3];
      gB[0] = gB[1]; gB[1] = gB[2]; gB[2] = gB[3];
      nctr += 1u;
    }
    return nz;
  };

  auto one_step = [&](int slot, __amdgpu_buffer_rsrc_t rs, float& sq_out) {
    if constexpr (ASM) {
      f2 ov, ox;
      const unsigned so = unsigned(slot) * step_b32;
      if constexpr (MIXED) {
        if constexpr (SM) mixed_step_asm_a_sm(v, xdA, xdB, vdA, vdB, h, dvl, ov, mc, sc, msc);
        else mixed_step_asm_a(v, xdA, xdB, vdA, vdB, h, dvl, ov, mc);
        if (slot > 0) __builtin_amdgcn_raw_buffer_store_b128(piece, rs, off_16, so - step_b32, 0);
        mixed_step_asm_b(v, xdA, xdB, h, dvl, ox, crash_bits, sq_out, mc);
        transpose_in(ov, ox);
      } else {
#if defined(FS_DIAG_NOSTORE)
        pair_step_asm_a(v, x, h, dvl, ox, pc);
        pair_step_asm_b(v, x, h, dvl, ov, crash_bits, sq_out, pc);
        asm volatile("" :: "v"(ov), "v"(ox), "s"(so));
#elif defined(FS_DIAG_NOXPOSE)
        pair_step_asm_a(v, x, h, dvl, ox, pc);
        __builtin_amdgcn_raw_buffer_store_b64(__builtin_bit_cast(u2v, ox), rs, off_x, so, 0);
        pair_step_asm_b(v, x, h, dvl, ov, crash_bits, sq_out, pc);
        __builtin_amdgcn_raw_buffer_store_b64(__builtin_bit_cast(u2v, ov), rs, off_v, so, 0);
#else
        if constexpr (NOISE) {
          const f2 nz = noise_term();
          if constexpr (SM) pair_step_asm_a_sm_nz(v, x, h, dvl, ox, pc, sc, nz);
          else pair_step_asm_a_nz(v, x, h, dvl, ox, pc, nz);
        } else {
          if constexpr (SM) pair_step_asm_a_sm(v, x, h, dvl, ox, pc, sc);
          else pair_step_asm_a(v, x, h, dvl, ox, pc);
        }
        if (slot > 0) __builtin_amdgcn_raw_buffer_store_b128(piece, rs, off_16, so - step_b32, 0);
        pair_step_asm_b(v, x, h, dvl, ov, crash_bits, sq_out, pc);
        transpose_in(ov, ox);
#endif
      }
      return;
    }
    f2 acc = idm_pair<DELTA4, FASTDIV>(v, vl, h, p, two_sqrt_ab, rc_ab, rc_v0, one);
    if constexpr (NOISE) acc = pk_add(acc, noise_term());
    f2 acc_s = {0.0f, 0.0f};
    if constexpr (SM) acc_s = sumo_acc_pair<FASTDIV>(v, vl, h, sc, one);
    f2 ox;
    if (MIXED) {
      const double aA = double(acc.x), aB = double(acc.y);
      const double nA = tmax(vdA + aA * dt64, 0.0), nB = tmax(vdB + aB * dt64, 0.0);
      double cA = vdA + (nA - vdA) * ramp64, cB = vdB + (nB - vdB) * ramp64;
      if constexpr (SM) {
        const double sA = tmax(vdA + double(acc_s.x) * dt64, floor0A), sB = tmax(vdB + double(acc_s.y) * dt64, floor0B);
        cA = tmin(cA, sA); cB = tmin(cB, sB);
        cA = tmin(cA, vdA + adtA); cB = tmin(cB, vdB + adtB);
        cA = tmax(cA, vdA - ddtA); cB = tmax(cB, vdB - ddtB);
      }
      vdA = cA;
      vdB = cB;
      const double xA = xdA + vdA * dt64, xB = xdB + vdB * dt64;
      xdA = xA >= L64 ? xA - L64 : xA;
      xdB = xB >= L64 ? xB - L64 : xB;
      v = f2{float(vdA), float(vdB)};
      ox = f2{float(xdA * rc_L64), float(xdB * rc_L64)};
    } else {
      f2 nv = pk_add(v, pk_mul(acc, dt2));
      nv.x = tmax(nv.x, 0.0f);
      nv.y = tmax(nv.y, 0.0f);
      f2 vc = pk_add(v, pk_mul(pk_sub(nv, v), ramp2));
      if constexpr (SM) {
        const f2 vs = pk_add(v, pk_mul(acc_s, dt2));
        const f2 cap1 = pk_add(v, sc.adt), flo = pk_sub(v, sc.ddt);
        vc.x = tmin(vc.x, tmax(sc.floor0.x, vs.x));
        vc.y = tmin(vc.y, tmax(sc.floor0.y, vs.y));
        vc.x = tmax(tmin(vc.x, cap1.x), flo.x);
        vc.y = tmax(tmin(vc.y, cap1.y), flo.y);
      }
      v = vc;
      const f2 xn = pk_add(x, pk_mul(v, dt2));
      const f2 xw = pk_sub(xn, L2);
      x.x = nonneg_else(xw.x, xn.x);
      x.y = nonneg_else(xw.y, xn.y);
      ox = div_const2<FASTDIV>(x, L2, rc_L2);
    }
    h = headway();
    vl = f2{v.y, next_a<ROW>(v.x, last, lane)};
    const f2 hc = pk_sub(h, gap2);
    crash_bits = __builtin_amdgcn_alignbit(crash_bits, __builtin_bit_cast(unsigned, __builtin_fminf(hc.x, hc.y)), 31);
    if (BADCHK) {
      const f2 vb = pk_sub(v, m100);
      bad_bits = __builtin_amdgcn_alignbit(bad_bits, __builtin_bit_cast(unsigned, __builtin_fminf(vb.x, vb.y)), 31);
    }
    f2 ov;
    if (MIXED) ov = f2{float(vdA * rc_ms64), float(vdB * rc_ms64)};
    else ov = f2{div_via_f64(v.x, ms64, rc_ms64), div_via_f64(v.y, ms64, rc_ms64)};
    const unsigned so = unsigned(slot) * step_b32;
    __builtin_amdgcn_raw_buffer_store_b64(__builtin_bit_cast(u2v, ov), rs, off_v, so, 0);
// ... 90 lines not shown
```

flow_amd/csrc/flowsim_pair_step_a_sm.inc:

```
__device__ __forceinline__ void FS_PAIR_A_NAME(f2& V, f2& X, f2& H, f2& DVL, f2& OX, const PairConsts& c,
                                                const SumoPair& m FS_PAIR_A_NZ_PARAM) {
  unsigned long long sa, sb;
  asm volatile(
      "v_cmp_nlt_f32_e64 %[sa], |v116|, %[c1e3]\n"
      "v_cmp_nlt_f32_e64 %[sb], |v117|, %[c1e3]\n"
      "v_pk_mul_f32 v[124:125], v[112:113], v[118:119]\n"
      "v_pk_mul_f32 v[126:127], v[124:125], %[rcab]\n"
      "v_pk_mul_f32 v[142:143], v[124:125], %[rcts]\n"
      "v_pk_fma_f32 v[130:131], v[126:127], %[tsab], v[124:125] neg_lo:[1,0,0] neg_hi:[1,0,0]\n"
      "v_pk_fma_f32 v[144:145], v[142:143], %[ts], v[124:125] neg_lo:[1,0,0] neg_hi:[1,0,0]\n"
      "v_pk_fma_f32 v[126:127], v[130:131], %[rcab], v[126:127]\n"
      "v_pk_fma_f32 v[142:143], v[144:145], %[rcts], v[142:143]\n"
      "v_cndmask_b32_e64 v120, %[c1e3], v116, %[sa]\n"
      "v_cndmask_b32_e64 v121, %[c1e3], v117, %[sb]\n"
      "v_max_f32_e32 v138, v116, %[c1e3]\n"
      "v_max_f32_e32 v139, v117, %[c1e3]\n"
      "v_pk_mul_f32 v[124:125], v[112:113], %[rcv0]\n"
      "v_rcp_f32_e32 v122, v120\n"
      "v_rcp_f32_e32 v123, v121\n"
      "v_rcp_f32_e32 v140, v138\n"
      "v_rcp_f32_e32 v141, v139\n"
      "v_pk_fma_f32 v[130:131], v[124:125], %[p0], v[112:113] neg_lo:[1,0,0] neg_hi:[1,0,0]\n"
      "v_pk_mul_f32 v[146:147], v[112:113], %[rcsm]\n"
      "v_pk_fma_f32 v[124:125], v[130:131], %[rcv0], v[124:125]\n"
      "v_pk_fma_f32 v[144:145], v[146:147], %[smax], v[112:113] neg_lo:[1,0,0] neg_hi:[1,0,0]\n"
      "v_pk_mul_f32 v[130:131], v[112:113], %[p1]\n"
      "v_pk_fma_f32 v[146:147], v[144:145], %[rcsm], v[146:147]\n"
      "v_pk_add_f32 v[130:131], v[130:131], v[126:127]\n"
      "v_pk_mul_f32 v[144:145], v[112:113], %[tau]\n"
      "v_pk_fma_f32 v[126:127], v[120:121], v[122:123], %[one] neg_lo:[1,0,0] neg_hi:[1,0,0]\n"
      "v_pk_add_f32 v[142:143], v[144:145], v[142:143]\n"
      "v_pk_fma_f32 v[144:145], v[138:139], v[140:141], %[one] neg_lo:[1,0,0] neg_hi:[1,0,0]\n"
      "v_max_f32_e32 v130, 0, v130\n"
      "v_max_f32_e32 v131, 0, v131\n"
      "v_max_f32_e32 v142, 0, v142\n"
      "v_max_f32_e32 v143, 0, v143\n"
      "v_pk_fma_f32 v[122:123], v[126:127], v[122:123], v[122:123]\n"
      "v_pk_fma_f32 v[140:141], v[144:145], v[140:141], v[140:141]\n"
      "v_pk_add_f32 v[130:131], %[p5], v[130:131]\n"
      "v_pk_add_f32 v[142:143], %[mgap], v[142:143]\n"
      "v_pk_mul_f32 v[124:125], v[124:125], v[124:125]\n"
      "v_pk_mul_f32 v[146:147], v[146:147], v[146:147]\n"
      "v_pk_mul_f32 v[126:127], v[130:131], v[122:123]\n"
      "v_pk_mul_f32 v[144:145], v[142:143], v[140:141]\n"
      "v_pk_mul_f32 v[124:125], v[124:125], v[124:125]\n"
      "v_pk_mul_f32 v[146:147], v[146:147], v[146:147]\n"
      "v_pk_fma_f32 v[132:133], v[120:121], v[126:127], v[130:131] neg_lo:[1,0,0] neg_hi:[1,0,0]\n"
      "v_pk_fma_f32 v[134:135], v[138:139], v[144:145], v[142:143] neg_lo:[1,0,0] neg_hi:[1,0,0]\n"
      "v_pk_add_f32 v[124:125], %[one], v[124:125] neg_lo:[0,1] neg_hi:[0,1]\n"
      "v_pk_add_f32 v[146:147], %[one], v[146:147] neg_lo:[0,1] neg_hi:[0,1]\n"
      "v_pk_fma_f32 v[126:127], v[132:133], v[122:123], v[126:127]\n"
      "v_pk_fma_f32 v[144:145], v[134:135], v[140:141], v[144:145]\n"
      "v_pk_fma_f32 v[132:133], v[120:121], v[126:127], v[130:131] neg_lo:[1,0,0] neg_hi:[1,0,0]\n"
      "v_pk_fma_f32 v[134:135], v[138:139], v[144:145], v[142:143] neg_lo:[1,0,0] neg_hi:[1,0,0]\n"
      "v_pk_fma_f32 v[126:127], v[132:133], v[122:123], v[126:127]\n"
      "v_pk_fma_f32 v[144:145], v[134:135], v[140:141], v[144:145]\n"
      "v_pk_mul_f32 v[126:127], v[126:127], v[126:127]\n"
      "v_pk_mul_f32 v[144:145], v[144:145], v[144:145]\n"
      "v_pk_add_f32 v[124:125], v[124:125], v[126:127] neg_lo:[0,1] neg_hi:[0,1]\n"
      "v_pk_add_f32 v[146:147], v[146:147], v[144:145] neg_lo:[0,1] neg_hi:[0,1]\n"
      "v_pk_mul_f32 v[124:125], %[p2], v[124:125]\n"
      "v_pk_mul_f32 v[146:147], %[maxa], v[146:147]\n"
#if FS_PAIR_A_NZ
      "v_pk_add_f32 v[124:125], v[124:125], %[nz]\n"
#endif
      "v_pk_mul_f32 v[124:125], v[124:125], %[dt2]\n"
      "v_pk_mul_f32 v[146:147], v[146:147], %[dt2]\n"
      "v_pk_add_f32 v[124:125], v[112:113], v[124:125]\n"
      "v_pk_add_f32 v[146:147], v[112:113], v[146:147]\n"
      "v_max_f32_e32 v124, 0, v124\n"
      "v_max_f32_e32 v125, 0, v125\n"
      "v_max_f32_e32 v146, %[fl0], v146\n"
      "v_max_f32_e32 v147, %[fl1], v147\n"
      "v_pk_add_f32 v[124:125], v[124:125], v[112:113] neg_lo:[0,1] neg_hi:[0,1]\n"
      "v_pk_add_f32 v[144:145], v[112:113], %[adt]\n"
      "v_pk_mul_f32 v[124:125], v[124:125], %[ramp2]\n"
      "v_pk_add_f32 v[142:143], v[112:113], %[ddt] neg_lo:[0,1] neg_hi:[0,1]\n"
      "v_pk_add_f32 v[124:125], v[112:113], v[124:125]\n"
      "v_min_f32_e32 v124, v124, v146\n"
      "v_min_f32_e32 v125, v125, v147\n"
      "v_min_f32_e32 v124, v124, v144\n"
      "v_min_f32_e32 v125, v125, v145\n"
      "v_max_f32_e32 v112, v124, v142\n"
      "v_max_f32_e32 v113, v125, v143\n"
      "v_pk_mul_f32 v[124:125], v[112:113], %[dt2]\n"
      "v_pk_add_f32 v[124:125], v[114:115], v[124:125]\n"
      "v_pk_add_f32 v[126:127], v[124:125], %[L2] neg_lo:[0,1] neg_hi:[0,1]\n"
      "v_min_u32_e32 v114, v126, v124\n"
      "v_min_u32_e32 v115, v127, v125\n"
      "v_pk_mul_f32 v[124:125], v[114:115], %[rcL2]\n"
      "v_pk_fma_f32 v[126:127], v[124:125], %[L2], v[114:115] neg_lo:[1,0,0] neg_hi:[1,0,0]\n"
      "v_pk_fma_f32 %[ox], v[126:127], %[rcL2], v[124:125]\n"
      : "+{v[112:113]}"(V), "+{v[114:115]}"(X), "+{v[116:117]}"(H), "+{v[118:119]}"(DVL), [ox] "=&v"(OX),
        [sa] "=&s"(sa), [sb] "=&s"(sb)
      : [c1e3] "v"(c.c1e3), [rcab] "v"(c.rc_ab), [tsab] "v"(c.tsab), [rcv0] "v"(c.rc_v0), [p0] "v"(c.p0),
        [p1] "v"(c.p1), [p2] "v"(c.p2), [p5] "v"(c.p5), [one] "v"(c.one), [dt2] "v"(c.dt2), [ramp2] "v"(c.ramp2),
        [L2] "v"(c.L2), [rcL2] "v"(c.rc_L2), [rcts] "v"(m.rc_ts), [ts] "v"(m.ts), [rcsm] "v"(m.rc_smax),
        [smax] "v"(m.smax), [tau] "v"(m.tau), [mgap] "v"(m.min_gap), [maxa] "v"(m.maxa), [fl0] "v"(m.floor0.x),
        [fl1] "v"(m.floor0.y), [adt] "v"(m.adt), [ddt] "v"(m.ddt)
#if FS_PAIR_A_NZ
        , [nz] "v"(nz)
#endif
      : "v120", "v121", "v122", "v123", "v124", "v125", "v126", "v127", "v130", "v131", "v132", "v133", "v134", "v135",
        "v138", "v139", "v140", "v141", "v142", "v143", "v144", "v145", "v146", "v147");
}
```

flow_amd/csrc/flowsim_ringrl.h:

```cpp
#pragma once
#include "flowsim_pair.h"

namespace fs {

template <int N, int I = 0, typename F>
__device__ __forceinline__ void static_for(F&& f) {
  if constexpr (I < N) {
    f(std::integral_constant<int, I>{});
    static_for<N, I + 1>(f);
  }
}

template <typename T, int ROW, bool NOISE, bool FAST>
struct RingPairCore {
  static constexpr bool MIXED = sizeof(T) == 8;
  static constexpr int RPW = 64 / ROW;
  const DevView<T>& s;
  int lane, k, r, N, LP, rr, kk, iA, iB;
  bool rvalid, valid, last, rlA, rlB;
  f2 p[6];
  T lenB, len_nextA;
  f2 two_sqrt_ab, rc_v0, rc_ab, one, dt2, ramp2, gap2, len_lead;
  double dt64, ramp64;
  f2 L2;
  double L64;
  SumoPair sc;
  double floor0A, floor0B, adtA, adtB, ddtA, ddtB;
  float act_lo, act_hi;
  uint32_t nctr;
  f2 sigma;
  bool noisyA, noisyB;
  float gA[4], gB[4];
  int tcount;
  f2 x, v;
  double xdA = 0, xdB = 0, vdA = 0, vdB = 0;
  f2 h, vl;
  f2 dgap = {0.0f, 0.0f};
  double dgA = 0, dgB = 0;

  __device__ __forceinline__ explicit RingPairCore(const DevView<T>& s_) : s(s_) {
    lane = threadIdx.x & 63;
    const int wave = (blockIdx.x * blockDim.x + threadIdx.x) >> 6;
    const int row = lane / ROW;
    k = lane % ROW;
    r = wave * RPW + row;
    N = s.N;
    LP = N >> 1;
    rvalid = r < s.R;
    valid = rvalid && k < LP;
    rr = rvalid ? r : s.R - 1;
    kk = k < LP ? k : LP - 1;
    last = (kk == LP - 1);
    iA = 2 * kk;
    iB = iA + 1;
    rlA = s.ctrl[iA] == FS_CTRL_RL;
    rlB = s.ctrl[iB] == FS_CTRL_RL;
#pragma unroll
    for (int q = 0; q < 6; ++q) p[q] = f2{float(s.p[q * N + iA]), float(s.p[q * N + iB])};
    {
      const float dflt[6] = {30.0f, 1.0f, 1.0f, 1.5f, 4.0f, 2.0f};
#pragma unroll
      for (int q = 0; q < 6; ++q) {
        p[q].x = rlA ? dflt[q] : p[q].x;
        p[q].y = rlB ? dflt[q] : p[q].y;
      }
    }
    lenB = s.length[iB];
    len_nextA = next_a<ROW>(T(s.length[iA]), last, lane);
    tcount = s.time[rr];
    nctr = NOISE ? s.noise_ctr[rr] : 0u;
    sigma = NOISE ? f2{float(s.noise[iA]), float(s.noise[iB])} : f2{0.0f, 0.0f};
    noisyA = NOISE && sigma.x > 0.0f && !rlA;
    noisyB = NOISE && sigma.y > 0.0f && !rlB;
    clear_draws();
    if constexpr (NOISE) {
      if ((nctr & 3u) != 0u) {
        draw_block();
        for (uint32_t q = 0; q < (nctr & 3u); ++q) rotate_draws();
      }
    }
    const float dt = float(s.dt);
    two_sqrt_ab = f2{2.0f * tsqrt(p[2].x * p[3].x), 2.0f * tsqrt(p[2].y * p[3].y)};
    rc_v0 = f2{1.0f / p[0].x, 1.0f / p[0].y};
    rc_ab = f2{1.0f / two_sqrt_ab.x, 1.0f / two_sqrt_ab.y};
    one = splat(1.0f);
    dt2 = splat(dt);
    ramp2 = splat(float(s.ramp));
    gap2 = splat(float(s.crash_gap));
    dt64 = double(s.dt);
    ramp64 = double(s.ramp);
    len_lead = f2{float(lenB), float(len_nextA)};
    {
      const int mA = s.speed_mode[iA], mB = s.speed_mode[iB];
      const float maA = float(s.max_accel[iA]), maB = float(s.max_accel[iB]);
      const float mdA = float(s.max_decel[iA]), mdB = float(s.max_decel[iB]);
      sc.tau = f2{float(s.sumo_tau[iA]), float(s.sumo_tau[iB])};
      sc.min_gap = f2{float(s.sumo_min_gap[iA]), float(s.sumo_min_gap[iB])};
      sc.maxa = f2{maA, maB};
      sc.smax = f2{float(s.sumo_max_speed[iA]), float(s.sumo_max_speed[iB])};
      sc.rc_smax = f2{1.0f / sc.smax.x, 1.0f / sc.smax.y};
      sc.ts = f2{2.0f * tsqrt(maA * mdA), 2.0f * tsqrt(maB * mdB)};
      sc.rc_ts = f2{1.0f / sc.ts.x, 1.0f / sc.ts.y};
      const float BIG = 3.0e38f;
      sc.floor0 = f2{(mA & 1) ? 0.0f : BIG, (mB & 1) ? 0.0f : BIG};
      sc.adt = f2{(mA & 2) ? maA * dt : BIG, (mB & 2) ? maB * dt : BIG};
      sc.ddt = f2{(mA & 4) ? mdA * dt : BIG, (mB & 4) ? mdB * dt : BIG};
      floor0A = double(sc.floor0.x); floor0B = double(sc.floor0.y);
      adtA = (mA & 2) ? double(s.max_accel[iA]) * dt64 : double(BIG);
      adtB = (mB & 2) ? double(s.max_accel[iB]) * dt64 : double(BIG);
      ddtA = (mA & 4) ? double(s.max_decel[iA]) * dt64 : double(BIG);
      ddtB = (mB & 4) ? double(s.max_decel[iB]) * dt64 : double(BIG);
    }
    const bool clip_on = s.clip_actions != 0;
    act_lo = clip_on ? float(s.act_lo) : -3.0e38f;
    act_hi = clip_on ? float(s.act_hi) : 3.0e38f;
  }

  __device__ __forceinline__ void set_length(T L) {
    L2 = splat(float(L));
    L64 = double(L);
  }
  __device__ __forceinline__ void load_state(const T* px, const T* pv) {
    const size_t idx = size_t(rr) * N + iA;
    if (MIXED) {
      xdA = double(px[idx]); xdB = double(px[idx + 1]);
      vdA = double(pv[idx]); vdB = double(pv[idx + 1]);
      v = f2{float(vdA), float(vdB)};
      x = f2{0.0f, 0.0f};
    } else {
      x = f2{float(px[idx]), float(px[idx + 1])};
      v = f2{float(pv[idx]), float(pv[idx + 1])};
    }
  }
  __device__ __forceinline__ f2 headway() {
    if (MIXED) {
      const double xn = next_a<ROW>(xdA, last, lane);
      double dA = xdB - xdA, dB = xn - xdB;
      dA = dA < 0.0 ? dA + L64 : dA;
      dB = dB < 0.0 ? dB + L64 : dB;
      dgA = dA;
      dgB = dB;
      return f2{float(dA - double(lenB)), float(dB - double(len_nextA))};
    } else {
      const f2 xl = {x.y, next_a<ROW>(x.x, last, lane)};
      f2 d = pk_sub(xl, x);
      const f2 dw = pk_add(d, L2);
      d.x = nonneg_else(d.x, dw.x);
      d.y = nonneg_else(d.y, dw.y);
      dgap = d;
      return pk_sub(d, len_lead);
    }
  }
  __device__ __forceinline__ void snapshot() {
    h = headway();
    vl = f2{v.y, next_a<ROW>(v.x, last, lane)};
  }
  __device__ __forceinline__ float clip(float a) const { return hmin(hmax(a, act_lo), act_hi); }

  __device__ __forceinline__ void draw_block() {
    gauss4<float>(s.seed_lo, s.seed_hi, s.rep0 + uint32_t(rr), uint32_t(iA), nctr >> 2, gA, s.noise_exact != 0);
    gauss4<float>(s.seed_lo, s.seed_hi, s.rep0 + uint32_t(rr), uint32_t(iB), nctr >> 2, gB, s.noise_exact != 0);
  }
  __device__ __forceinline__ void rotate_draws() {
    gA[0] = gA[1]; gA[1] = gA[2]; gA[2] = gA[3];
    gB[0] = gB[1]; gB[1] = gB[2]; gB[2] = gB[3];
  }
  __device__ __forceinline__ void clear_draws() {
    gA[0] = gA[1] = gA[2] = gA[3] = 0.0f;
    gB[0] = gB[1] = gB[2] = gB[3] = 0.0f;
  }
  template <int SLOT>
  __device__ __forceinline__ f2 noise_of() const {
    const float tA = sigma.x * gA[SLOT], tB = sigma.y * gB[SLOT];
    return f2{noisyA ? tA : -0.0f, noisyB ? tB : -0.0f};
  }
  __device__ __forceinline__ f2 noise_term(bool live) {
    f2 nz = {-0.0f, -0.0f};
    if constexpr (NOISE) {
      const bool fresh = live && (nctr & 3u) == 0u;
      if (__ballot(fresh) != 0ull) {
        if (fresh) draw_block();
      }
      nz = noise_of<0>();
      if (live) {
        rotate_draws();
        nctr += 1u;
      }
    }
    return nz;
  }

  template <bool LIVE_ALL>
  __device__ __forceinline__ void advance(bool live_in, bool have_act, float ownA, float ownB, f2 nz_in = f2{-0.0f, -0.0f}) {
    const bool live = LIVE_ALL ? true : live_in;
    f2 acc = idm_pair<FAST, FAST>(v, vl, h, p, two_sqrt_ab, rc_ab, rc_v0, one);
    if constexpr (NOISE) acc = pk_add(acc, LIVE_ALL ? nz_in : noise_term(live));
    const float clA = clip(ownA), clB = clip(ownB);
    acc.x = rlA ? clA : acc.x;
    acc.y = rlB ? clB : acc.y;
    const bool cmdA = !rlA || have_act, cmdB = !rlB || have_act;
    const f2 acc_s = sumo_acc_pair<FAST>(v, vl, h, sc, one);
    if (MIXED) {
      const double aA = double(acc.x), aB = double(acc.y);
      const double nA = tmax(vdA + aA * dt64, 0.0), nB = tmax(vdB + aB * dt64, 0.0);
      double cA = vdA + (nA - vdA) * ramp64, cB = vdB + (nB - vdB) * ramp64;
      {
        const double vsA = vdA + double(acc_s.x) * dt64, vsB = vdB + double(acc_s.y) * dt64;
        cA = tmin(cA, tmax(vsA, floor0A)); cB = tmin(cB, tmax(vsB, floor0B));
        cA = tmin(cA, vdA + adtA); cB = tmin(cB, vdB + adtB);
        cA = tmax(cA, vdA - ddtA); cB = tmax(cB, vdB - ddtB);
        cA = cmdA ? cA : tmax(vsA, 0.0);
        cB = cmdB ? cB : tmax(vsB, 0.0);
      }
      const double xA = xdA + cA * dt64, xB = xdB + cB * dt64;
      const double wA = xA >= L64 ? xA - L64 : xA, wB = xB >= L64 ? xB - L64 : xB;
      if (live) {
        vdA = cA; vdB = cB;
        xdA = wA; xdB = wB;
      }
      v = f2{float(vdA), float(vdB)};
    } else {
      f2 nv = pk_add(v, pk_mul(acc, dt2));
      nv.x = hmax(nv.x, 0.0f);
      nv.y = hmax(nv.y, 0.0f);
      f2 vc = pk_add(v, pk_mul(pk_sub(nv, v), ramp2));
      {
        const f2 vs = pk_add(v, pk_mul(acc_s, dt2));
        const f2 cap1 = pk_add(v, sc.adt), flo = pk_sub(v, sc.ddt);
        vc.x = hmin(vc.x, hmax(sc.floor0.x, vs.x));
        vc.y = hmin(vc.y, hmax(sc.floor0.y, vs.y));
        vc.x = hmax(hmin(vc.x, cap1.x), flo.x);
        vc.y = hmax(hmin(vc.y, cap1.y), flo.y);
        const float zA = hmax(0.0f, vs.x), zB = hmax(0.0f, vs.y);
        vc.x = cmdA ? vc.x : zA;
        vc.y = cmdB ? vc.y : zB;
      }
      const f2 xn = pk_add(x, pk_mul(vc, dt2));
      const f2 xw = pk_sub(xn, L2);
      f2 xq;
      xq.x = nonneg_else(xw.x, xn.x);
      xq.y = nonneg_else(xw.y, xn.y);
      if (live) {
        v = vc;
        x = xq;
      }
    }
    if (live) tcount += 1;
    snapshot();
  }

  __device__ __forceinline__ unsigned step_flags() const {
    const f2 hc = pk_sub(h, gap2), vb = pk_sub(v, f2{-100.0f, -100.0f});
    return ((__builtin_bit_cast(unsigned, hmin(hc.x, hc.y)) >> 31) | ((__builtin_bit_cast(unsigned, hmin(vb.x, vb.y)) >> 31) << 1)) &
           (valid ? 3u : 0u);
  }
  __device__ __forceinline__ void store_state() const {
    const size_t idx = size_t(r) * N + iA;
    if (MIXED) {
      s.pos[idx] = T(xdA); s.pos[idx + 1] = T(xdB);
      s.vel[idx] = T(vdA); s.vel[idx + 1] = T(vdB);
    } else {
      s.pos[idx] = T(x.x); s.pos[idx + 1] = T(x.y);
      s.vel[idx] = T(v.x); s.vel[idx + 1] = T(v.y);
    }
    if (kk == 0) s.time[rr] = tcount;
    if (NOISE && kk == 0) s.noise_ctr[rr] = nctr;
  }
};

__device__ __forceinline__ float wave_reward(float sum_v, int N, float mean_a, bool bad) {
  const float mean_v = div_via_f64(sum_v, double(N), 1.0 / double(N));
  float reward = div_via_f64(4.0f * mean_v, 20.0, 1.0 / 20.0);
  if (mean_a > 0.0f) reward = reward + 4.0f * (0.0f - mean_a);
  return bad ? 0.0f : reward;
}

template <typename T, int ROW, int HEAD, bool NOISE, bool FAST, bool MC = false>
__global__ __launch_bounds__(256) void k_ring_pair(DevView<T> s, int num_steps_arg, const uint8_t* __restrict__ mask,
                                                   const float* __restrict__ actions, size_t act_stride,
                                                   float* __restrict__ obs, float* __restrict__ rew,
                                                   uint8_t* __restrict__ done, int obs_every_step) {
  constexpr bool MIXED = sizeof(T) == 8;
  constexpr bool WA = HEAD == 1 || HEAD == 2;
  constexpr bool MA = HEAD >= 2;
  static_assert(!(MA && MIXED), "the multi-agent heads exist in float32 only");
  RingPairCore<T, ROW, NOISE, FAST> core(s);
  const int lane = core.lane, k = core.k, N = core.N, rr = core.rr, iA = core.iA, iB = core.iB;
  const bool rvalid = core.rvalid, valid = core.valid, last = core.last, rlA = core.rlA, rlB = core.rlB;
  const bool live_replica = mask == nullptr || mask[rr] != 0;
  const int num_steps = (mask != nullptr && __ballot(live_replica) == 0ull) ? 0 : num_steps_arg;
  const int colA = rlA ? s.rl_index[iA] : 0, colB = rlB ? s.rl_index[iB] : 0;
  const T L = s.ring_len[rr] + T(4) * s.jlen;
  const float Lf = float(L);
  const f2 rc_L2 = splat(1.0f / Lf);
  const double rc_L64 = 1.0 / double(L);
  const double ms64 = double(s.max_speed), rc_ms64 = 1.0 / ms64;
  const bool have_act = actions != nullptr;
  core.set_length(L);
  core.load_state(s.pos, s.vel);
  core.snapshot();
  const f2 &x = core.x, &v = core.v, &vl = core.vl, &h = core.h, &dgap = core.dgap;

  const int num_rl = s.num_rl;
  const bool single_rl = num_rl == 1;
  const bool redA = WA && valid && iA < num_rl, redB = WA && valid && iB < num_rl;
  float ownA_n = 0.0f, ownB_n = 0.0f, redA_n = 0.0f, redB_n = 0.0f;
  auto load_actions = [&](int step) {
    const float* a0 = actions + size_t(step) * act_stride + size_t(rr) * num_rl;
    if (single_rl) {
      ownA_n = a0[0];
    } else {
      if (rlA) ownA_n = a0[colA];
      if (rlB) ownB_n = a0[colB];
      if (redA) redA_n = a0[iA];
      if (redB) redB_n = a0[iB];
    }
  };
  if (have_act && num_steps > 0) load_actions(0);

  const int obs_dim = HEAD == 1 ? 3 : (HEAD == 2 ? 3 * num_rl : (HEAD == 3 ? 6 * num_rl : 2 * N));
  const size_t step_rows = obs_every_step ? size_t(s.R) : 0;
  float* orow = obs + size_t(rr) * obs_dim;
  float* rrow = rew + rr;
  uint8_t* drow = done + rr;
  const bool poA = HEAD == 1 && valid && rlA && colA == 0, poB = HEAD == 1 && valid && rlB && colB == 0;
  const double rc15 = 1.0 / 15.0, pml64 = double(s.po_max_length), rc_pml64 = 1.0 / pml64;
  const bool maA = MA && valid && rlA, maB = MA && valid && rlB;
  const int col_nextA = MA ? __builtin_bit_cast(int, next_a<ROW>(__builtin_bit_cast(float, rlA ? colA : -1), last, lane)) : -1;
  const bool fwB = HEAD == 3 && valid && col_nextA >= 0;
  const double Lq64 = double(Lf), rc_Lq64 = 1.0 / Lq64;
  const float len_meA = float(s.length[iA]), len_meB = float(core.lenB);
  auto write_obs = [&]() {
    if constexpr (HEAD == 2) {
      if (maA || maB) {
        const float v_me = maB ? v.y : v.x, v_ld = maB ? vl.y : vl.x, h_me = maB ? h.y : h.x;
        float* o = orow + 3 * (maB ? colB : colA);
        o[0] = div_via_f64(v_me, 15.0, rc15);
        o[1] = div_via_f64(v_ld - v_me, 15.0, rc15);
        o[2] = div_via_f64(h_me, pml64, rc_pml64);
      }
      if (maA && maB) {
        float* o = orow + 3 * colA;
        o[0] = div_via_f64(v.x, 15.0, rc15);
        o[1] = div_via_f64(vl.x - v.x, 15.0, rc15);
        o[2] = div_via_f64(h.x, pml64, rc_pml64);
      }
    } else if constexpr (HEAD == 3) {
      const float xn = next_a<ROW>(x.x, last, lane);
      if (maA) {
        float* o = orow + 6 * colA;
        o[0] = div_via_f64(x.x, Lq64, rc_Lq64);
        o[1] = div_via_f64(v.x, ms64, rc_ms64);
        o[2] = div_via_f64(vl.x - v.x, ms64, rc_ms64);
        o[3] = div_via_f64((x.y - x.x) - len_meA, Lq64, rc_Lq64);
      }
      if (maB) {
        float* o = orow + 6 * colB;
        o[0] = div_via_f64(x.y, Lq64, rc_Lq64);
        o[1] = div_via_f64(v.y, ms64, rc_ms64);
        o[2] = div_via_f64(vl.y - v.y, ms64, rc_ms64);
        o[3] = div_via_f64((xn - x.y) - len_meB, Lq64, rc_Lq64);
        o[4] = div_via_f64(v.y - v.x, ms64, rc_ms64);
        o[5] = div_via_f64(h.x, Lq64, rc_Lq64);
      }
      if (fwB) {
        float* o = orow + 6 * col_nextA;
        o[4] = div_via_f64(vl.y - v.y, ms64, rc_ms64);
        o[5] = div_via_f64(h.y, Lq64, rc_Lq64);
      }
    } else if (HEAD == 1) {
      if (MIXED) {
        const double vdn = next_a<ROW>(core.vdA, last, lane);
        const double v_me = poB ? core.vdB : core.vdA, v_ld = poB ? vdn : core.vdB, d_me = poB ? core.dgB : core.dgA;
        if (poA || poB) {
          orow[0] = float(v_me * rc15);
          orow[1] = float((v_ld - v_me) * rc15);
          orow[2] = float(d_me * rc_pml64);
        }
      } else {
        const float v_me = poB ? v.y : v.x, v_ld = poB ? vl.y : vl.x, d_me = poB ? dgap.y : dgap.x;
        if (poA || poB) {
          orow[0] = div_via_f64(v_me, 15.0, rc15);
          orow[1] = div_via_f64(v_ld - v_me, 15.0, rc15);
          orow[2] = div_via_f64(d_me, pml64, rc_pml64);
        }
      }
    } else if (valid) {
      f2 ov, ox;
      if (MIXED) {
        ov = f2{float(core.vdA * rc_ms64), float(core.vdB * rc_ms64)};
        ox = f2{float(core.xdA * rc_L64), float(core.xdB * rc_L64)};
      } else {
        ov = f2{div_via_f64(v.x, ms64, rc_ms64), div_via_f64(v.y, ms64, rc_ms64)};
        ox = FAST ? div_const2<true>(x, core.L2, rc_L2) : f2{x.x / core.L2.x, x.y / core.L2.y};
      }
      *reinterpret_cast<f2*>(orow + iA) = ov;
      *reinterpret_cast<f2*>(orow + N + iA) = ox;
    }
  };

  auto terms = [&](float aredA, float aredB, unsigned& fl, float& t0, float& t1) {
    fl = core.step_flags();
    if (WA) {
      t0 = valid ? v.x + v.y : 0.0f;
      const float caA = tabs(core.clip(aredA)), caB = tabs(core.clip(aredB));
      t1 = (redA ? caA : 0.0f) + (redB ? caB : 0.0f);
    } else {
      const float tv = float(s.target_velocity);
      const f2 dv = {valid ? v.x - tv : 0.0f, valid ? v.y - tv : 0.0f};
      t0 = dv.x * dv.x + dv.y * dv.y;
      t1 = 0.0f;
    }
  };
  auto finish = [&](unsigned fany, float s0, float s1, bool live, int t_after, float& reward, uint8_t& dflag) {
    const bool crashed = !MA && live && (fany & 1u) != 0u;
    const bool bad = (fany & 2u) != 0u || crashed;
    if (WA) {
      reward = wave_reward(s0, N, div_via_f64(s1, double(num_rl), 1.0 / double(num_rl)), bad);
      reward = have_act ? reward : 0.0f;
    } else {
      const float cost = tsqrt(s0);
      const float max_cost = float(s.max_cost);
      reward = tmax(max_cost - cost, 0.0f) / (max_cost + 1.1920928955078125e-07f);
      reward = bad ? 0.0f : reward;
    }
    dflag = done_flag(t_after >= s.step_limit, crashed);
  };

  auto single_step = [&](int step) {
    const float ownA = ownA_n, ownB = single_rl ? ownA_n : ownB_n;
    const float aredA = single_rl ? ownA_n : redA_n, aredB = redB_n;
    if (have_act && step + 1 < num_steps) load_actions(step + 1);
    core.template advance<false>(live_replica, have_act, ownA, ownB);
    const bool emit = obs_every_step || (step == num_steps - 1);
    if (emit) {
      unsigned fl;
      float t0, t1;
      terms(aredA, aredB, fl, t0, t1);
      const unsigned fany = seg_or<ROW>(fl);
      write_obs();
      const float s0 = seg_sum<ROW>(t0), s1 = WA ? seg_sum<ROW>(t1) : 0.0f;
      float reward;
      uint8_t dflag;
      finish(fany, s0, s1, live_replica, core.tcount, reward, dflag);
      if (rvalid && k == 0) {
        *rrow = reward;
        *drow = dflag;
      }
      orow += step_rows * obs_dim;
      rrow += step_rows;
      drow += step_rows;
    }
  };

  int step = 0;
  constexpr bool GROUPS = ROW == 16;
  if (GROUPS && obs_every_step && mask == nullptr && (single_rl || !have_act || MC)) {
    if constexpr (NOISE) {
#pragma unroll 1
      while (step < num_steps && (core.nctr & 3u) != 0u) {
        single_step(step);
        step += 1;
      }
    }
    const bool deep = !MC && single_rl && have_act;
    float qA[4] = {0.0f, 0.0f, 0.0f, 0.0f}, qB[4] = {0.0f, 0.0f, 0.0f, 0.0f};
    float qrA[4] = {0.0f, 0.0f, 0.0f, 0.0f}, qrB[4] = {0.0f, 0.0f, 0.0f, 0.0f};
    const int rcA = redA ? iA : 0, rcB = redB ? iB : 0;
    const bool mc_act = MC && have_act;
    const float* mc_p = actions + size_t(rr) * num_rl;
    if (mc_act) {
#pragma unroll
      for (int q = 0; q < 4; ++q) {
        if (step + q < num_steps) {
          const float* a0 = mc_p + size_t(step + q) * act_stride;
          qA[q] = a0[colA];
          qB[q] = a0[colB];
          if (WA) { qrA[q] = a0[rcA]; qrB[q] = a0[rcB]; }
        }
      }
      mc_p += size_t(step + 4) * act_stride;
    }
    auto group_actions = [&](int first) -> float {
      const int st = first + k < num_steps ? first + k : num_steps - 1;
      return actions[size_t(st) * act_stride + size_t(rr)];
    };
    float a_cur = 0.0f, a_nxt = 0.0f;
    if (deep && step + 16 <= num_steps) a_nxt = group_actions(step);
    constexpr bool PO_ROWS = HEAD == 1 && !MIXED;
    const bool po_lane = poA || poB;
    const unsigned long long po_m = __ballot(po_lane);
    const int k_po = po_m ? (__builtin_ctzll(po_m) & 15) : 0;
    const int po_idx = 11 - ((k - k_po) & 15);
    const int po_st = po_idx < 0 ? 0 : po_idx / 3, po_c = po_idx < 0 ? 0 : po_idx % 3;
    const double po_div = po_c == 2 ? pml64 : 15.0, po_rc = po_c == 2 ? rc_pml64 : rc15;
    const size_t po_off = size_t(po_st) * step_rows * obs_dim + po_c;
    const bool po_store = rvalid && po_idx >= 0;
    float oacc = 0.0f;
    auto po_push = [&](float n) {
      oacc = dpp<0x120 + 1>(oacc);
      oacc = po_lane ? n : oacc;
    };
#pragma unroll 1
    for (; step + 16 <= num_steps; step += 16) {
      a_cur = a_nxt;
      if (deep && step + 32 <= num_steps) a_nxt = group_actions(step + 16);
#pragma unroll 1
      for (int blk = 0; blk < 4; ++blk) {
        if constexpr (NOISE) {
          core.draw_block();
          core.nctr += 4u;
        }
        float t0[4], t1[4];
        unsigned crash_bits = 0u, bad_bits = 0u;
        static_for<4>([&](auto slot_c) {
          constexpr int slot = decltype(slot_c)::value;
          const float a = deep ? dpp<DPP_ROW_NEWBCAST0 + slot>(a_cur) : 0.0f;
          f2 nz = {-0.0f, -0.0f};
          if constexpr (NOISE) nz = core.template noise_of<slot>();
          const float oA = MC ? qA[slot] : a, oB = MC ? qB[slot] : a;
          const float rA = MC ? qrA[slot] : a, rB = MC ? qrB[slot] : 0.0f;
          if constexpr (MC) {
            if (mc_act && step + 4 * blk + slot + 4 < num_steps) {
              qA[slot] = mc_p[colA];
              qB[slot] = mc_p[colB];
              if (WA) { qrA[slot] = mc_p[rcA]; qrB[slot] = mc_p[rcB]; }
            }
            mc_p += act_stride;
          }
          core.template advance<true>(true, have_act, oA, oB, nz);
          if constexpr (PO_ROWS) {
            const float v_me = poB ? v.y : v.x, v_ld = poB ? vl.y : vl.x, d_me = poB ? dgap.y : dgap.x;
            po_push(v_me);
            po_push(v_ld - v_me);
            po_push(d_me);
          } else {
            write_obs();
            orow += step_rows * obs_dim;
          }
          unsigned fl;
          terms(rA, rB, fl, t0[slot], t1[slot]);
          crash_bits = (crash_bits << 1) | (fl & 1u);
          bad_bits = (bad_bits << 1) | (fl >> 1);
        });
        if constexpr (PO_ROWS) {
          const float q = div_via_f64(oacc, po_div, po_rc);
          if (po_store) orow[po_off] = q;
          orow += size_t(4) * step_rows * obs_dim;
        }
        const float s0 = transposed_sum<ROW, 4>(t0, lane);
        const float s1 = WA ? transposed_sum<ROW, 4>(t1, lane) : 0.0f;
        const unsigned crash_any = seg_or<ROW>(crash_bits), bad_any = seg_or<ROW>(bad_bits);
        if (k < 4) {
          const unsigned fany = ((crash_any >> (3 - k)) & 1u) | (((bad_any >> (3 - k)) & 1u) << 1);
          float reward;
          uint8_t dflag;
          finish(fany, s0, s1, true, core.tcount - (3 - k), reward, dflag);
          if (rvalid) {
            rrow[size_t(k) * s.R] = reward;
            drow[size_t(k) * s.R] = dflag;
          }
        }
        rrow += size_t(4) * s.R;
        drow += size_t(4) * s.R;
        a_cur = dpp<0x120 + 12>(a_cur);
      }
    }
    if constexpr (NOISE) core.clear_draws();
  }
  if (have_act && step > 0 && step < num_steps) load_actions(step);
#pragma unroll 1
  for (; step < num_steps; ++step) single_step(step);

  if (num_steps == 0) {
    write_obs();
    return;
  }
  if (valid && live_replica) core.store_state();
}

}
```

flow_amd/csrc/flowsim_sim.h:

```cpp
#pragma once
#include <hip/hip_runtime.h>

#include <algorithm>
#include <climits>
#include <cmath>
#include <cstdio>
#include <cstdlib>
#include <cstring>
#include <map>
#include <mutex>
#include <new>
#include <string>
#include <type_traits>
#include <vector>

#include "flowsim.h"
#include "flowsim_kernels.h"
#include "flowsim_open.h"
#include "flowsim_pair.h"
#include "flowsim_fig8.h"
#include "flowsim_ringrl.h"
#include "flowsim_policy.h"
#include "flowsim_wide.h"
#include "flowsim_queue_consts.h"


namespace fsim {

inline thread_local std::string g_err;

inline int fail(int code, const std::string& msg) {
  g_err = msg;
  return code;
}

#define HIP_TRY(expr)                                                                      \
  do {                                                                                     \
    hipError_t e_ = (expr);                                                                \
    if (e_ != hipSuccess)                                                                  \
      return fail(FS_ERR_HIP, std::string(#expr) + " failed: " + hipGetErrorString(e_));   \
  } while (0)

struct StepArgs {
  int num_steps;
  const uint8_t* mask;
  const float* actions;
  size_t act_stride;
  float* obs;
  float* rew;
  uint8_t* done;
  int obs_every_step;
};

template <int N>
using Int = std::integral_constant<int, N>;

template <typename F>
auto pick(bool b, F&& f) {
  return b ? f(std::true_type()) : f(std::false_type());
}

struct SimBase {
  virtual ~SimBase() {}
  fs_config cfg{};
  std::vector<fs_vehicle_spec> veh;
  std::vector<fs_segment> segs;
  std::vector<fs_inflow> inflows;
  std::vector<fs_cell> obs_cells, act_cells;
  std::vector<int32_t> obs_perm;
  std::vector<uint8_t> init_alive;
  int obs_dim = 0;
  int act_dim = 0;
  int seg = 0;
  hipStream_t own_stream = nullptr;
  hipStream_t stream = nullptr;
  float* d_actions = nullptr;
  float* d_obs = nullptr;
  float* d_rew = nullptr;
  uint8_t* d_done = nullptr;
  uint8_t* d_mask = nullptr;
  float* d_dump = nullptr;
  std::vector<void*> allocs;
  int after_reset = 0;
  bool force_generic = false;
  bool no_fastdiv = false;
  bool f16s = false;
  bool mixed = false;
  bool no_pair = false;
  bool no_loop_kernel = false;
  bool no_loop_full = false;
  bool no_ring_rl = false;
  bool no_queue = false;
  int* d_qflag = nullptr;
  bool qflag_armed = false;
  int check_qflag() {
    if (!qflag_armed || !d_qflag) return FS_OK;
    int f = 0;
    HIP_TRY(hipMemcpy(&f, d_qflag, sizeof(int), hipMemcpyDeviceToHost));
    if (f != 0)
      return fail(FS_ERR_UNSUPPORTED, "k_drop_queue: a path of the lane-drop network held more than 64 vehicles (or more than 8 "
                                      "arrived in one sub-step): the results of this handle are invalid -- create it "
                                      "with FLOWSIM_NO_QUEUE=1 (slot-order kernels)");
    qflag_armed = false;
    return FS_OK;
  }
  bool has_user_ctrl = false;
  const char* last_kernel = "";
  int launched() {
    HIP_TRY(hipGetLastError());
    return FS_OK;
  }

  virtual int launch_steps(int num_steps, const uint8_t* mask, const float* actions, size_t act_stride,
                           float* obs, float* rew, uint8_t* done, int obs_every_step) = 0;
  virtual int launch_reset(const uint8_t* mask) = 0;
  virtual int launch_policy(const fs_policy* pol, int num_steps, int reset_done, const float* obs_in, float* obs,
                            float* act, float* logp, float* rew, uint8_t* done) = 0;
  uint32_t* d_pol_ctr = nullptr;
  virtual int get_state(int field, void* dst, size_t bytes) = 0;
  virtual int set_state(int field, const void* src, size_t bytes) = 0;
  virtual int add_vehicle(int replica, int slot, int route, double x, double speed) = 0;
};

template <typename T>
struct Sim : SimBase {
  fs::DevView<T> dv{};
  fs::OpenView<T> ov{};
  fs::QueueConsts qc{};
  bool open_net = false;
  std::vector<T> h_len;
  std::vector<T> h_ring_len;

  template <typename U>
  int dev_alloc(U** out, size_t count) {
    void* p = nullptr;
    HIP_TRY(hipMalloc(&p, (count ? count : 1) * sizeof(U)));
    allocs.push_back(p);
    *out = static_cast<U*>(p);
    return FS_OK;
  }

  template <typename U>
  int upload(const U** out, const std::vector<U>& host) {
    U* p = nullptr;
    int rc = dev_alloc(&p, host.size());
    if (rc) return rc;
    HIP_TRY(hipMemcpy(p, host.data(), host.size() * sizeof(U), hipMemcpyHostToDevice));
    *out = p;
    return FS_OK;
  }

  int init() {
    const int R = cfg.num_replicas, N = cfg.num_vehicles;
    const size_t RN = size_t(R) * N;
    int rc;
    if ((rc = dev_alloc(&dv.pos, RN))) return rc;
    if ((rc = dev_alloc(&dv.vel, RN))) return rc;
    if ((rc = dev_alloc(&dv.prev_vel, RN))) return rc;
    if ((rc = dev_alloc(&dv.accel, RN))) return rc;
    if ((rc = dev_alloc(&dv.ctrl_state, RN))) return rc;
    if ((rc = dev_alloc(&dv.lane, RN))) return rc;
    if ((rc = dev_alloc(&dv.last_lc, RN))) return rc;
    {
      std::vector<int32_t> il(RN, 0);
      if (cfg.init_lane)
        for (size_t e = 0; e < RN; ++e) il[e] = cfg.init_lane[e];
      if ((rc = upload(&dv.init_lane, il))) return rc;
    }
    if ((rc = dev_alloc(&dv.time, size_t(R)))) return rc;
    if ((rc = dev_alloc(&dv.sort_key, RN))) return rc;
    dv.sort_vehicles = cfg.sort_vehicles;
    dv.obs_perm = nullptr;
    if (!obs_perm.empty()) {
      if ((rc = upload(&dv.obs_perm, obs_perm))) return rc;
    }
    if ((rc = dev_alloc(&dv.noise_ctr, size_t(R)))) return rc;
    HIP_TRY(hipMemset(dv.noise_ctr, 0, size_t(R) * sizeof(uint32_t)));
    HIP_TRY(hipMemset(dv.time, 0, size_t(R) * sizeof(int32_t)));

    std::vector<T> ipos(RN), ivel(RN), rlen(R);
    for (size_t e = 0; e < RN; ++e) {
      ipos[e] = T(cfg.init_pos[e]);
      ivel[e] = cfg.init_vel ? T(cfg.init_vel[e]) : T(veh[e % N].initial_speed);
    }
    for (int r = 0; r < R; ++r) rlen[r] = cfg.ring_length ? T(cfg.ring_length[r]) : T(0);
    for (T vv : ivel) init_vel_negative = init_vel_negative || !(vv >= T(-100));
    neg_speed_possible = init_vel_negative;
    if ((rc = upload(&dv.init_pos, ipos))) return rc;
    if ((rc = upload(&dv.init_vel, ivel))) return rc;
    if ((rc = upload(&dv.ring_len, rlen))) return rc;
    if ((rc = upload(&dv.init_ring_len, rlen))) return rc;
    dv.st16 = nullptr;
    if (f16s && (rc = dev_alloc(&dv.st16, 3 * RN))) return rc;
    h_ring_len = rlen;

    std::vector<int32_t> ctrl(N), fsafe(N), smode(N), rli(N), pisi(N, -1);
    int n_pis = 0;
    std::vector<T> p(size_t(FS_MAX_CTRL_PARAMS) * N), noise(N), delay(N), maxa(N), maxd(N), len(N), stau(N),
        sgap(N), smax(N);
    int flags = 0;
    bool all_idm = true, idm_set = true;
    for (int i = 0; i < N; ++i) {
      const fs_vehicle_spec& v = veh[i];
      ctrl[i] = v.controller;
      fsafe[i] = v.fail_safe;
      smode[i] = v.speed_mode;
      rli[i] = v.rl_index;
      for (int k = 0; k < FS_MAX_CTRL_PARAMS; ++k) p[size_t(k) * N + i] = T(v.p[k]);
      noise[i] = T(v.noise);
      delay[i] = T(v.delay);
      maxa[i] = T(v.max_accel);
      maxd[i] = T(v.max_decel);
      len[i] = T(v.length);
      stau[i] = T(v.sumo_tau);
      sgap[i] = T(v.sumo_min_gap);
      smax[i] = T(v.sumo_max_speed);
      if (v.controller == FS_CTRL_BCM || v.controller == FS_CTRL_USER) flags |= fs::FLAG_NEED_FOLLOWER;
      if (v.controller == FS_CTRL_USER) has_user_ctrl = true;
      if (v.controller == FS_CTRL_NONLOCAL_FOLLOWER_STOPPER) flags |= fs::FLAG_NEED_MEAN;
      if (v.controller == FS_CTRL_LAC) flags |= fs::FLAG_HAS_LAC;
      if (v.controller == FS_CTRL_PISATURATION) {
        flags |= fs::FLAG_HAS_LAC;
        pisi[i] = n_pis++;
      }
      if (v.noise > 0 && v.controller != FS_CTRL_SIM && v.controller != FS_CTRL_RL) flags |= fs::FLAG_HAS_NOISE;
      if (v.fail_safe != FS_FAILSAFE_NONE) flags |= fs::FLAG_HAS_FAILSAFE;
      if (v.controller == FS_CTRL_SIM || v.controller == FS_CTRL_RL || (v.speed_mode & 1) || cfg.junction_mode)
        flags |= fs::FLAG_NEED_SUMO;
      if (v.speed_mode & 6) flags |= fs::FLAG_NEED_SUMO;
      if (v.controller == FS_CTRL_SIM || v.controller == FS_CTRL_RL || cfg.junction_mode) sumo_beyond_speed_mode = true;
      if (v.speed_mode & 7) speed_mode_any = true;
      if (v.controller == FS_CTRL_SIM) any_sim = true;
      if (v.controller != FS_CTRL_IDM) all_idm = false;
      if (v.controller != FS_CTRL_IDM && v.controller != FS_CTRL_RL && v.controller != FS_CTRL_SIM) idm_set = false;
    }
    loop_div_ok = true;
    for (int i = 0; i < N; ++i)
      loop_div_ok = loop_div_ok && float(veh[i].sumo_min_gap) >= 1e-3f && float(veh[i].sumo_min_gap) <= 1e6f &&
                    (veh[i].controller != FS_CTRL_IDM || (float(veh[i].p[5]) >= 1e-3f && float(veh[i].p[5]) <= 1e6f));
    loop_delta4 = true;
    for (int i = 0; i < N; ++i) loop_delta4 = loop_delta4 && (veh[i].controller != FS_CTRL_IDM || veh[i].p[4] == 4.0);
    if (loop_delta4) flags |= fs::FLAG_DELTA4;
    open_div_ok = loop_div_ok && (cfg.speed_limit <= 0 ||
                                  (float(cfg.speed_limit) >= 9.5367431640625e-07f && float(cfg.speed_limit) <= 1048576.0f));
    for (int i = 0; i < N; ++i) {
      auto in_range = [](float c) { return c >= 9.5367431640625e-07f && c <= 1048576.0f; };
      open_div_ok = open_div_ok && in_range(float(veh[i].sumo_max_speed)) &&
                    in_range(2.0f * std::sqrt(float(veh[i].max_accel) * float(veh[i].max_decel))) &&
                    (veh[i].controller != FS_CTRL_IDM ||
                     (in_range(float(veh[i].p[0])) && in_range(2.0f * std::sqrt(float(veh[i].p[2]) * float(veh[i].p[3])))));
    }
    {
      bool no_ctrl = true;
      for (int i = 0; i < N; ++i) no_ctrl = no_ctrl && (veh[i].controller == FS_CTRL_SIM || veh[i].controller == FS_CTRL_RL);
      if (no_ctrl) flags |= fs::FLAG_NO_FLOW_CTRL;
    }
    if (all_idm) flags |= fs::FLAG_ALL_IDM;
    if (idm_set) flags |= fs::FLAG_IDM_SET;
    delta4 = all_idm;
    for (int i = 0; i < N; ++i) delta4 = delta4 && (veh[i].p[4] == 4.0);
    h_len = len;
    if ((rc = upload(&dv.ctrl, ctrl))) return rc;
    if ((rc = upload(&dv.failsafe, fsafe))) return rc;
    if ((rc = upload(&dv.speed_mode, smode))) return rc;
    if ((rc = upload(&dv.rl_index, rli))) return rc;
    if ((rc = upload(&dv.pis_index, pisi))) return rc;
    dv.n_pis = n_pis;
    dv.pis_H = int(38.0 / cfg.sim_step) - 1;
    if (dv.pis_H < 1) dv.pis_H = 1;
    if ((rc = dev_alloc(&dv.pis_hist, size_t(R) * (n_pis ? n_pis : 1) * (n_pis ? dv.pis_H : 1)))) return rc;
    if ((rc = dev_alloc(&dv.pis_n, size_t(R) * (n_pis ? n_pis : 1)))) return rc;
    HIP_TRY(hipMemset(dv.pis_n, 0, size_t(R) * (n_pis ? n_pis : 1) * sizeof(int32_t)));
    if ((rc = upload(&dv.p, p))) return rc;
    if ((rc = upload(&dv.noise, noise))) return rc;
    if ((rc = upload(&dv.delay, delay))) return rc;
    if ((rc = upload(&dv.max_accel, maxa))) return rc;
    if ((rc = upload(&dv.max_decel, maxd))) return rc;
    if ((rc = upload(&dv.length, len))) return rc;
    if ((rc = upload(&dv.sumo_tau, stau))) return rc;
    if ((rc = upload(&dv.sumo_min_gap, sgap))) return rc;
    if ((rc = upload(&dv.sumo_max_speed, smax))) return rc;

    dv.R = R;
    dv.N = N;
    dv.num_rl = cfg.num_rl;
    dv.env = cfg.env;
    dv.integrator = cfg.integrator;
    dv.sims_per_step = cfg.sims_per_step;
    dv.junction_mode = cfg.junction_mode;
    dv.clip_actions = cfg.clip_actions;
    dv.evaluate = cfg.evaluate;
    dv.track_aux = cfg.track_aux;
    dv.num_lanes = cfg.num_lanes < 1 ? 1 : cfg.num_lanes;
    dv.lane_change_mode = cfg.lane_change_mode;
    dv.last_lc_quirk = cfg.last_lc_quirk;
    dv.noise_exact = cfg.noise_exact != 0 ? 1 : 0;
    dv.lc_duration = T(cfg.lane_change_duration);
    {
      std::vector<int32_t> lca(N, 0);
      int any_lc = 0;
      for (int i = 0; i < N; ++i) {
        lca[i] = (veh[i].lane_change_mode & 0x55) != 0 && veh[i].controller != FS_CTRL_RL;
        any_lc |= lca[i];
      }
      if ((rc = upload(&dv.lc_auto, lca))) return rc;
      dv.lc_enabled = (cfg.network == FS_NET_RING && cfg.num_lanes > 1 && any_lc) ? 1 : 0;
      dv.lc_cooldown = cfg.lane_change_cooldown_steps > 0 ? cfg.lane_change_cooldown_steps : 1;
      dv.lc_min_gain = T(cfg.lane_change_min_gain);
    }
    dv.nseg = cfg.num_segments;
    dv.seg_internal = 0u;
    for (int k = 0; k < FS_MAX_SEGMENTS; ++k) {
      const bool in = k < cfg.num_segments;
      dv.seg_start[k] = in ? T(segs[k].start) : T(0);
      dv.seg_flow_start[k] = in ? T(segs[k].flow_start) : T(0);
      dv.seg_flow_slope[k] = in ? T(segs[k].flow_slope) : T(0);
      if (in && segs[k].internal) dv.seg_internal |= (1u << k);
    }
    dv.junction_on = cfg.junction.enabled;
    dv.ja_in = T(cfg.junction.a_in);
    dv.ja_out = T(cfg.junction.a_out);
    dv.jb_in = T(cfg.junction.b_in);
    dv.jb_out = T(cfg.junction.b_out);
    dv.j_lookahead = T(cfg.junction.lookahead);
    dv.j_time_gap = T(cfg.junction.time_gap);
    dv.za_lo = T(cfg.junction.za_lo);
    dv.za_hi = T(cfg.junction.za_hi);
    dv.zb_lo = T(cfg.junction.zb_lo);
    dv.zb_hi = T(cfg.junction.zb_hi);
    if (cfg.horizon < 0) {
      dv.step_limit = INT_MAX;
    } else {
      long long lim = (long long)cfg.sims_per_step * ((long long)cfg.warmup_steps + cfg.horizon);
      dv.step_limit = lim > INT_MAX ? INT_MAX : int(lim);
    }
    dv.flags = flags;
    dv.seed_lo = uint32_t(cfg.seed & 0xFFFFFFFFull);
    dv.seed_hi = uint32_t(cfg.seed >> 32);
    dv.rep0 = uint32_t(cfg.replica_offset);
    dv.dt = T(cfg.sim_step);
    dv.ramp = T(cfg.slowdown_ramp);
    dv.jlen = T(cfg.junction_length);
    dv.crash_gap = T(cfg.crash_gap);
    dv.max_speed = T(cfg.max_speed);
    dv.target_velocity = T(cfg.target_velocity);
    {
      double ss = 0.0;
      for (int i = 0; i < N; ++i) ss += cfg.target_velocity * cfg.target_velocity;
      dv.max_cost = T(std::sqrt(ss));
    }
    dv.act_lo = T(cfg.action_low);
    dv.act_hi = T(cfg.action_high);
    dv.po_max_length = T(cfg.po_max_length);

    open_net = (cfg.network == FS_NET_MERGE || cfg.network == FS_NET_BOTTLENECK);
    if (open_net && (rc = init_open())) return rc;

    if ((rc = dev_alloc(&d_actions, size_t(R) * (act_dim > 0 ? act_dim : 1)))) return rc;
    if ((rc = dev_alloc(&d_obs, size_t(R) * obs_dim))) return rc;
    if ((rc = dev_alloc(&d_rew, size_t(R)))) return rc;
    if ((rc = dev_alloc(&d_done, size_t(R)))) return rc;
    if ((rc = dev_alloc(&d_mask, size_t(R)))) return rc;
    if ((rc = dev_alloc(&d_dump, size_t(256)))) return rc;
    if ((rc = launch_reset(nullptr))) return rc;
    if (open_net) HIP_TRY(hipMemsetAsync(ov.episode, 0xFF, size_t(R) * sizeof(int32_t), stream));
    return FS_OK;
  }

  int init_open() {
    const int R = cfg.num_replicas, N = cfg.num_vehicles;
    const size_t RN = size_t(R) * N;
    int rc;
    if ((rc = dev_alloc(&ov.seq, RN))) return rc;
    if ((rc = dev_alloc(&ov.origin, RN))) return rc;
    if ((rc = dev_alloc(&ov.foll, RN))) return rc;
    if ((rc = dev_alloc(&ov.ctl_seq, RN))) return rc;
    if ((rc = dev_alloc(&ov.lead, RN))) return rc;
    if ((rc = dev_alloc(&ov.arrived_rl, RN))) return rc;
    if ((rc = dev_alloc(&ov.foll_h, RN))) return rc;
    if ((rc = dev_alloc(&ov.headway, RN))) return rc;
    if ((rc = dev_alloc(&ov.vmax, RN))) return rc;
    if ((rc = dev_alloc(&ov.arr_hist, size_t(R) * 20))) return rc;
    if ((rc = dev_alloc(&ov.counters, size_t(R) * 8))) return rc;
    if ((rc = dev_alloc(&ov.emitted, size_t(R) * FS_MAX_INFLOWS))) return rc;
    if ((rc = dev_alloc(&ov.generated, size_t(R) * FS_MAX_INFLOWS))) return rc;
    if ((rc = dev_alloc(&ov.episode, size_t(R)))) return rc;
    if ((rc = dev_alloc(&d_qflag, size_t(1)))) return rc;
    HIP_TRY(hipMemset(d_qflag, 0, sizeof(int)));
    HIP_TRY(hipMemset(ov.episode, 0xFF, size_t(R) * sizeof(int32_t)));
    HIP_TRY(hipMemset(ov.ctl_seq, 0xFF, RN * sizeof(int32_t)));
    HIP_TRY(hipMemset(ov.origin, 0xFF, RN * sizeof(int32_t)));
    HIP_TRY(hipMemset(ov.counters, 0, size_t(R) * 8 * sizeof(int32_t)));
    if ((rc = upload(&ov.init_alive, init_alive))) return rc;
    std::vector<int32_t> st(N);
// ... 730 lines not shown
```

Baseline: 13.60 billion.

## Add hand-scheduled inline-asm ring pair kernel for 16-lane rows

```diff
diff --git a/flow_amd/build.py b/flow_amd/build.py
--- a/flow_amd/build.py
+++ b/flow_amd/build.py
@@ -15,7 +15,7 @@
 VALIDATED_ROCM = "7.2"
 
 HEADERS = ["flowsim_sim.h", "flowsim_launch.h", "flowsim_kernels.h", "flowsim_open.h", "flowsim_wide.h",
-           "flowsim_pair.h", "flowsim_pair_step_a.inc", "flowsim_pair_step_a_sm.inc", "flowsim_fig8.h", "flowsim_ringrl.h", "flowsim_policy.h", "flowsim_queue.h", "flowsim_queue_consts.h", "flowsim_dropq.h",
+           "flowsim_pair.h", "flowsim_pair_step_a.inc", "flowsim_pair_step_a_sm.inc", "flowsim_mixed_step_a_sm.inc", "flowsim_fig8.h", "flowsim_ringrl.h", "flowsim_policy.h", "flowsim_queue.h", "flowsim_queue_consts.h", "flowsim_dropq.h",
            "flowsim_part.hip"]
 DEPS = [SRC] + [os.path.join(CSRC, h) for h in HEADERS] + [os.path.join(ROOT, "include", "flowsim.h")]
 assert all(os.path.exists(d) for d in DEPS)
diff --git a/flow_amd/csrc/flowsim.hip b/flow_amd/csrc/flowsim.hip
--- a/flow_amd/csrc/flowsim.hip
+++ b/flow_amd/csrc/flowsim.hip
@@ -269,7 +269,7 @@
         {"FLOWSIM_FORCE_GENERIC", &SimBase::force_generic}, {"FLOWSIM_NO_FASTDIV", &SimBase::no_fastdiv},
         {"FLOWSIM_NO_LOOP_KERNEL", &SimBase::no_loop_kernel}, {"FLOWSIM_NO_LOOP_FULL", &SimBase::no_loop_full},
         {"FLOWSIM_NO_RING_RL", &SimBase::no_ring_rl}, {"FLOWSIM_NO_QUEUE", &SimBase::no_queue},
-        {"FLOWSIM_NO_PAIR", &SimBase::no_pair}};
+        {"FLOWSIM_NO_PAIR", &SimBase::no_pair}, {"FLOWSIM_NO_RING_ASM", &SimBase::no_ring_asm}};
     for (const auto& sw : switches) {
       const char* v = std::getenv(sw.first);
       s->*sw.second = v && v[0] == '1';
diff --git a/flow_amd/csrc/flowsim_launch.h b/flow_amd/csrc/flowsim_launch.h
--- a/flow_amd/csrc/flowsim_launch.h
+++ b/flow_amd/csrc/flowsim_launch.h
@@ -147,6 +147,9 @@
     const bool mc = ROW == 16 && std::is_same<T, float>::value && (ma_head || (a.actions != nullptr && dv.num_rl > 1));
     auto kernel = [&](auto H, auto MC) {
       return pick(dv.flags & fs::FLAG_HAS_NOISE, [&](auto NZ) {
+        if constexpr (ROW == 16) {
+          if (fast && !no_ring_asm) return &fs::k_ring_pair_hand<T, H, NZ, MC>;
+        }
         return pick(fast, [&](auto FA) { return &fs::k_ring_pair<T, ROW, H, NZ, FA, MC>; });
       });
     };
diff --git a/flow_amd/csrc/flowsim_mixed_step_a_sm.inc b/flow_amd/csrc/flowsim_mixed_step_a_sm.inc
--- /dev/null
+++ b/flow_amd/csrc/flowsim_mixed_step_a_sm.inc
@@ -0,0 +1,168 @@
+__device__ __forceinline__ void FS_MIXED_A_NAME(f2& V32, double& XA, double& XB, double& VA, double& VB, f2& H,
+                                                    f2& DVL, f2& OV, const MixedConsts& c, const SumoPair& m,
+                                                    const MixedSumoConsts& d FS_MIXED_A_PARAM) {
+  unsigned long long sa, sb;
+  asm volatile(
+      "v_cmp_nlt_f32_e64 %[sa], |v140|, %[c1e3]\n"
+      "v_cmp_nlt_f32_e64 %[sb], |v141|, %[c1e3]\n"
+      "v_pk_mul_f32 v[124:125], v[112:113], v[142:143]\n"
+      "v_pk_mul_f32 v[126:127], v[124:125], %[rcab]\n"
+      "v_pk_mul_f32 v[150:151], v[124:125], %[rcts]\n"
+      "v_pk_fma_f32 v[130:131], v[126:127], %[tsab], v[124:125] neg_lo:[1,0,0] neg_hi:[1,0,0]\n"
+      "v_pk_fma_f32 v[152:153], v[150:151], %[ts], v[124:125] neg_lo:[1,0,0] neg_hi:[1,0,0]\n"
+      "v_pk_fma_f32 v[126:127], v[130:131], %[rcab], v[126:127]\n"
+      "v_pk_fma_f32 v[150:151], v[152:153], %[rcts], v[150:151]\n"
+      "v_cndmask_b32_e64 v120, %[c1e3], v140, %[sa]\n"
+      "v_cndmask_b32_e64 v121, %[c1e3], v141, %[sb]\n"
+      "v_max_f32_e32 v146, v140, %[c1e3]\n"
+      "v_max_f32_e32 v147, v141, %[c1e3]\n"
+      "v_pk_mul_f32 v[124:125], v[112:113], %[rcv0]\n"
+      "v_rcp_f32_e32 v122, v120\n"
+      "v_rcp_f32_e32 v123, v121\n"
+      "v_rcp_f32_e32 v148, v146\n"
+      "v_rcp_f32_e32 v149, v147\n"
+      "v_pk_fma_f32 v[130:131], v[124:125], %[p0], v[112:113] neg_lo:[1,0,0] neg_hi:[1,0,0]\n"
+      "v_pk_mul_f32 v[154:155], v[112:113], %[rcsm]\n"
+      "v_pk_fma_f32 v[124:125], v[130:131], %[rcv0], v[124:125]\n"
+      "v_pk_fma_f32 v[152:153], v[154:155], %[smax], v[112:113] neg_lo:[1,0,0] neg_hi:[1,0,0]\n"
+      "v_pk_mul_f32 v[130:131], v[112:113], %[p1]\n"
+      "v_pk_fma_f32 v[154:155], v[152:153], %[rcsm], v[154:155]\n"
+      "v_pk_add_f32 v[130:131], v[130:131], v[126:127]\n"
+      "v_pk_mul_f32 v[152:153], v[112:113], %[tau]\n"
+      "v_pk_fma_f32 v[126:127], v[120:121], v[122:123], %[one] neg_lo:[1,0,0] neg_hi:[1,0,0]\n"
+      "v_pk_add_f32 v[150:151], v[152:153], v[150:151]\n"
+      "v_pk_fma_f32 v[152:153], v[146:147], v[148:149], %[one] neg_lo:[1,0,0] neg_hi:[1,0,0]\n"
+      "v_max_f32_e32 v130, 0, v130\n"
+      "v_max_f32_e32 v131, 0, v131\n"
+      "v_max_f32_e32 v150, 0, v150\n"
+      "v_max_f32_e32 v151, 0, v151\n"
+      "v_pk_fma_f32 v[122:123], v[126:127], v[122:123], v[122:123]\n"
+      "v_pk_fma_f32 v[148:149], v[152:153], v[148:149], v[148:149]\n"
+      "v_pk_add_f32 v[130:131], %[p5], v[130:131]\n"
+      "v_pk_add_f32 v[150:151], %[mgap], v[150:151]\n"
+      "v_pk_mul_f32 v[124:125], v[124:125], v[124:125]\n"
+      "v_pk_mul_f32 v[154:155], v[154:155], v[154:155]\n"
+      "v_pk_mul_f32 v[126:127], v[130:131], v[122:123]\n"
+      "v_pk_mul_f32 v[152:153], v[150:151], v[148:149]\n"
+      "v_pk_mul_f32 v[124:125], v[124:125], v[124:125]\n"
+      "v_pk_mul_f32 v[154:155], v[154:155], v[154:155]\n"
+      "v_pk_fma_f32 v[132:133], v[120:121], v[126:127], v[130:131] neg_lo:[1,0,0] neg_hi:[1,0,0]\n"
+      "v_pk_fma_f32 v[134:135], v[146:147], v[152:153], v[150:151] neg_lo:[1,0,0] neg_hi:[1,0,0]\n"
+      "v_pk_add_f32 v[124:125], %[one], v[124:125] neg_lo:[0,1] neg_hi:[0,1]\n"
+      "v_pk_add_f32 v[154:155], %[one], v[154:155] neg_lo:[0,1] neg_hi:[0,1]\n"
+      "v_pk_fma_f32 v[126:127], v[132:133], v[122:123], v[126:127]\n"
+      "v_pk_fma_f32 v[152:153], v[134:135], v[148:149], v[152:153]\n"
+      "v_pk_fma_f32 v[132:133], v[120:121], v[126:127], v[130:131] neg_lo:[1,0,0] neg_hi:[1,0,0]\n"
+      "v_pk_fma_f32 v[134:135], v[146:147], v[152:153], v[150:151] neg_lo:[1,0,0] neg_hi:[1,0,0]\n"
+      "v_pk_fma_f32 v[126:127], v[132:133], v[122:123], v[126:127]\n"
+      "v_pk_fma_f32 v[152:153], v[134:135], v[148:149], v[152:153]\n"
+      "v_pk_mul_f32 v[126:127], v[126:127], v[126:127]\n"
+      "v_pk_mul_f32 v[152:153], v[152:153], v[152:153]\n"
+      "v_pk_add_f32 v[124:125], v[124:125], v[126:127] neg_lo:[0,1] neg_hi:[0,1]\n"
+      "v_pk_add_f32 v[154:155], v[154:155], v[152:153] neg_lo:[0,1] neg_hi:[0,1]\n"
+      "v_pk_mul_f32 v[124:125], %[p2], v[124:125]\n"
+      "v_pk_mul_f32 v[154:155], %[maxa], v[154:155]\n"
+#if FS_MIXED_A_NZ
+      "v_pk_add_f32 v[124:125], v[124:125], %[nz]\n"
+#endif
+#if FS_MIXED_A_RL
+      "v_cndmask_b32_e64 v124, v124, %[acta], %[rla]\n"
+      "v_cndmask_b32_e64 v125, v125, %[actb], %[rlb]\n"
+#endif
+      "v_cvt_f64_f32_e32 v[130:131], v124\n"
+      "v_cvt_f64_f32_e32 v[132:133], v125\n"
+      "v_cvt_f64_f32_e32 v[134:135], v154\n"
+      "v_cvt_f64_f32_e32 v[136:137], v155\n"
+      "v_mul_f64 v[130:131], v[130:131], %[dt]\n"
+      "v_mul_f64 v[132:133], v[132:133], %[dt]\n"
+      "v_mul_f64 v[134:135], v[134:135], %[dt]\n"
+      "v_mul_f64 v[136:137], v[136:137], %[dt]\n"
+      "v_add_f64 v[130:131], v[118:119], v[130:131]\n"
+      "v_add_f64 v[132:133], v[138:139], v[132:133]\n"
+      "v_add_f64 v[134:135], v[118:119], v[134:135]\n"
+      "v_add_f64 v[136:137], v[138:139], v[136:137]\n"
+#if FS_MIXED_A_RL
+      "v_max_f64 v[146:147], v[134:135], %[zero]\n"
+      "v_max_f64 v[148:149], v[136:137], %[zero]\n"
+#endif
+      "v_max_f64 v[130:131], v[130:131], %[zero]\n"
+      "v_max_f64 v[132:133], v[132:133], %[zero]\n"
+      "v_max_f64 v[134:135], v[134:135], %[fl0a]\n"
+      "v_max_f64 v[136:137], v[136:137], %[fl0b]\n"
+      "v_add_f64 v[130:131], v[130:131], -v[118:119]\n"
+      "v_add_f64 v[132:133], v[132:133], -v[138:139]\n"
+      "v_mul_f64 v[130:131], v[130:131], %[ramp]\n"
+      "v_mul_f64 v[132:133], v[132:133], %[ramp]\n"
+      "v_add_f64 v[130:131], v[118:119], v[130:131]\n"
+      "v_add_f64 v[132:133], v[138:139], v[132:133]\n"
+      "v_min_f64 v[130:131], v[130:131], v[134:135]\n"
+      "v_min_f64 v[132:133], v[132:133], v[136:137]\n"
+      "v_add_f64 v[134:135], v[118:119], %[adta]\n"
+      "v_add_f64 v[136:137], v[138:139], %[adtb]\n"
+      "v_min_f64 v[130:131], v[130:131], v[134:135]\n"
+      "v_min_f64 v[132:133], v[132:133], v[136:137]\n"
+      "v_add_f64 v[134:135], v[118:119], -%[ddta]\n"
+      "v_add_f64 v[136:137], v[138:139], -%[ddtb]\n"
+#if FS_MIXED_A_RL
+      "v_max_f64 v[130:131], v[130:131], v[134:135]\n"
+      "v_max_f64 v[132:133], v[132:133], v[136:137]\n"
+      "v_cndmask_b32_e64 v118, v146, v130, %[cmda]\n"
+      "v_cndmask_b32_e64 v119, v147, v131, %[cmda]\n"
+      "v_cndmask_b32_e64 v138, v148, v132, %[cmdb]\n"
+      "v_cndmask_b32_e64 v139, v149, v133, %[cmdb]\n"
+#else
+      "v_max_f64 v[118:119], v[130:131], v[134:135]\n"
+      "v_max_f64 v[138:139], v[132:133], v[136:137]\n"
+#endif
+      "v_mul_f64 v[130:131], v[118:119], %[dt]\n"
+      "v_mul_f64 v[132:133], v[138:139], %[dt]\n"
+      "v_add_f64 v[130:131], v[114:115], v[130:131]\n"
+      "v_add_f64 v[132:133], v[116:117], v[132:133]\n"
+      "v_add_f64 v[134:135], v[130:131], -%[L]\n"
+      "v_add_f64 v[136:137], v[132:133], -%[L]\n"
+#if FS_MIXED_A_RL
+      "v_cmp_gt_i32_e64 %[sa], 0, v135\n"
+      "v_cmp_gt_i32_e64 %[sb], 0, v137\n"
+      "v_cvt_f32_f64_e32 v112, v[118:119]\n"
+      "v_cvt_f32_f64_e32 v113, v[138:139]\n"
+#else
+      "v_cvt_f32_f64_e32 v112, v[118:119]\n"
+      "v_cvt_f32_f64_e32 v113, v[138:139]\n"
+      "v_cmp_gt_i32_e64 %[sa], 0, v135\n"
+      "v_cmp_gt_i32_e64 %[sb], 0, v137\n"
+      "v_mul_f64 v[120:121], v[118:119], %[rcms]\n"
+      "v_mul_f64 v[122:123], v[138:139], %[rcms]\n"
+#endif
+      "v_cndmask_b32_e64 v114, v134, v130, %[sa]\n"
+      "v_cndmask_b32_e64 v115, v135, v131, %[sa]\n"
+      "v_cndmask_b32_e64 v116, v136, v132, %[sb]\n"
+      "v_cndmask_b32_e64 v117, v137, v133, %[sb]\n"
+#if !FS_MIXED_A_RL
+      "v_cvt_f32_f64_e32 v128, v[120:121]\n"
+      "v_cvt_f32_f64_e32 v129, v[122:123]\n"
+#endif
+      : "+{v[112:113]}"(V32), "+{v[114:115]}"(XA), "+{v[116:117]}"(XB), "+{v[118:119]}"(VA), "+{v[138:139]}"(VB),
+        "+{v[140:141]}"(H), "+{v[142:143]}"(DVL),
+#if !FS_MIXED_A_RL
+        "={v[128:129]}"(OV),
+#endif
+        [sa] "=&s"(sa), [sb] "=&s"(sb)
+      : [c1e3] "v"(c.c1e3), [rcab] "v"(c.rc_ab), [tsab] "v"(c.tsab), [rcv0] "v"(c.rc_v0), [p0] "v"(c.p0),
+        [p1] "v"(c.p1), [p2] "v"(c.p2), [p5] "v"(c.p5), [one] "v"(c.one), [dt] "v"(c.dt), [ramp] "v"(c.ramp),
+        [L] "v"(c.L),
+#if !FS_MIXED_A_RL
+        [rcms] "v"(c.rc_ms),
+#endif
+        [zero] "v"(c.zero), [rcts] "v"(m.rc_ts), [ts] "v"(m.ts),
+        [rcsm] "v"(m.rc_smax), [smax] "v"(m.smax), [tau] "v"(m.tau), [mgap] "v"(m.min_gap), [maxa] "v"(m.maxa),
+        [fl0a] "v"(d.fl0a), [fl0b] "v"(d.fl0b), [adta] "v"(d.adta), [adtb] "v"(d.adtb), [ddta] "v"(d.ddta),
+        [ddtb] "v"(d.ddtb)
+#if FS_MIXED_A_NZ
+        , [nz] "v"(nz)
+#endif
+#if FS_MIXED_A_RL
+        , [acta] "v"(act.x), [actb] "v"(act.y), [rla] "s"(rla), [rlb] "s"(rlb), [cmda] "s"(cmda), [cmdb] "s"(cmdb)
+#endif
+      : "v120", "v121", "v122", "v123", "v124", "v125", "v126", "v127", "v130", "v131", "v132", "v133", "v134",
+        "v135", "v136", "v137", "v146", "v147", "v148", "v149", "v150", "v151", "v152", "v153", "v154", "v155");
+}
diff --git a/flow_amd/csrc/flowsim_pair.h b/flow_amd/csrc/flowsim_pair.h
--- a/flow_amd/csrc/flowsim_pair.h
+++ b/flow_amd/csrc/flowsim_pair.h
@@ -133,6 +133,8 @@
 #undef FS_PAIR_A_NAME
 #undef FS_PAIR_A_NZ
 #undef FS_PAIR_A_NZ_PARAM
+#define FS_PAIR_A_RL 0
+#define FS_PAIR_A_RL_PARAM
 #define FS_PAIR_A_NAME pair_step_asm_a_sm
 #define FS_PAIR_A_NZ 0
 #define FS_PAIR_A_NZ_PARAM
@@ -147,6 +149,8 @@
 #undef FS_PAIR_A_NAME
 #undef FS_PAIR_A_NZ
 #undef FS_PAIR_A_NZ_PARAM
+#undef FS_PAIR_A_RL
+#undef FS_PAIR_A_RL_PARAM
 __device__ __forceinline__ void pair_step_asm_b(f2& V, f2& X, f2& H, f2& DVL, f2& OV, unsigned& crash_bits, float& sq,
                                                 const PairConsts& c) {
   asm volatile(
@@ -267,131 +271,15 @@
         "v135", "v136", "v137");
 }
 struct MixedSumoConsts { double fl0a, fl0b, adta, adtb, ddta, ddtb; };
-__device__ __forceinline__ void mixed_step_asm_a_sm(f2& V32, double& XA, double& XB, double& VA, double& VB, f2& H,
-                                                    f2& DVL, f2& OV, const MixedConsts& c, const SumoPair& m,
-                                                    const MixedSumoConsts& d) {
-  unsigned long long sa, sb;
-  asm volatile(
-      "v_cmp_nlt_f32_e64 %[sa], |v140|, %[c1e3]\n"
-      "v_cmp_nlt_f32_e64 %[sb], |v141|, %[c1e3]\n"
-      "v_pk_mul_f32 v[124:125], v[112:113], v[142:143]\n"
-      "v_pk_mul_f32 v[126:127], v[124:125], %[rcab]\n"
-      "v_pk_mul_f32 v[150:151], v[124:125], %[rcts]\n"
-      "v_pk_fma_f32 v[130:131], v[126:127], %[tsab], v[124:125] neg_lo:[1,0,0] neg_hi:[1,0,0]\n"
-      "v_pk_fma_f32 v[152:153], v[150:151], %[ts], v[124:125] neg_lo:[1,0,0] neg_hi:[1,0,0]\n"
-      "v_pk_fma_f32 v[126:127], v[130:131], %[rcab], v[126:127]\n"
-      "v_pk_fma_f32 v[150:151], v[152:153], %[rcts], v[150:151]\n"
-      "v_cndmask_b32_e64 v120, %[c1e3], v140, %[sa]\n"
-      "v_cndmask_b32_e64 v121, %[c1e3], v141, %[sb]\n"
-      "v_max_f32_e32 v146, v140, %[c1e3]\n"
-      "v_max_f32_e32 v147, v141, %[c1e3]\n"
-      "v_pk_mul_f32 v[124:125], v[112:113], %[rcv0]\n"
-      "v_rcp_f32_e32 v122, v120\n"
-      "v_rcp_f32_e32 v123, v121\n"
-      "v_rcp_f32_e32 v148, v146\n"
-      "v_rcp_f32_e32 v149, v147\n"
-      "v_pk_fma_f32 v[130:131], v[124:125], %[p0], v[112:113] neg_lo:[1,0,0] neg_hi:[1,0,0]\n"
-      "v_pk_mul_f32 v[154:155], v[112:113], %[rcsm]\n"
-      "v_pk_fma_f32 v[124:125], v[130:131], %[rcv0], v[124:125]\n"
-      "v_pk_fma_f32 v[152:153], v[154:155], %[smax], v[112:113] neg_lo:[1,0,0] neg_hi:[1,0,0]\n"
-      "v_pk_mul_f32 v[130:131], v[112:113], %[p1]\n"
-      "v_pk_fma_f32 v[154:155], v[152:153], %[rcsm], v[154:155]\n"
-      "v_pk_add_f32 v[130:131], v[130:131], v[126:127]\n"
-      "v_pk_mul_f32 v[152:153], v[112:113], %[tau]\n"
-      "v_pk_fma_f32 v[126:127], v[120:121], v[122:123], %[one] neg_lo:[1,0,0] neg_hi:[1,0,0]\n"
-      "v_pk_add_f32 v[150:151], v[152:153], v[150:151]\n"
-      "v_pk_fma_f32 v[152:153], v[146:147], v[148:149], %[one] neg_lo:[1,0,0] neg_hi:[1,0,0]\n"
-      "v_max_f32_e32 v130, 0, v130\n"
-      "v_max_f32_e32 v131, 0, v131\n"
-      "v_max_f32_e32 v150, 0, v150\n"
-      "v_max_f32_e32 v151, 0, v151\n"
-      "v_pk_fma_f32 v[122:123], v[126:127], v[122:123], v[122:123]\n"
-      "v_pk_fma_f32 v[148:149], v[152:153], v[148:149], v[148:149]\n"
-      "v_pk_add_f32 v[130:131], %[p5], v[130:131]\n"
-      "v_pk_add_f32 v[150:151], %[mgap], v[150:151]\n"
-      "v_pk_mul_f32 v[124:125], v[124:125], v[124:125]\n"
-      "v_pk_mul_f32 v[154:155], v[154:155], v[154:155]\n"
-      "v_pk_mul_f32 v[126:127], v[130:131], v[122:123]\n"
-      "v_pk_mul_f32 v[152:153], v[150:151], v[148:149]\n"
-      "v_pk_mul_f32 v[124:125], v[124:125], v[124:125]\n"
-      "v_pk_mul_f32 v[154:155], v[154:155], v[154:155]\n"
-      "v_pk_fma_f32 v[132:133], v[120:121], v[126:127], v[130:131] neg_lo:[1,0,0] neg_hi:[1,0,0]\n"
-      "v_pk_fma_f32 v[134:135], v[146:147], v[152:153], v[150:151] neg_lo:[1,0,0] neg_hi:[1,0,0]\n"
-      "v_pk_add_f32 v[124:125], %[one], v[124:125] neg_lo:[0,1] neg_hi:[0,1]\n"
-      "v_pk_add_f32 v[154:155], %[one], v[154:155] neg_lo:[0,1] neg_hi:[0,1]\n"
-      "v_pk_fma_f32 v[126:127], v[132:133], v[122:123], v[126:127]\n"
-      "v_pk_fma_f32 v[152:153], v[134:135], v[148:149], v[152:153]\n"
-      "v_pk_fma_f32 v[132:133], v[120:121], v[126:127], v[130:131] neg_lo:[1,0,0] neg_hi:[1,0,0]\n"
-      "v_pk_fma_f32 v[134:135], v[146:147], v[152:153], v[150:151] neg_lo:[1,0,0] neg_hi:[1,0,0]\n"
-      "v_pk_fma_f32 v[126:127], v[132:133], v[122:123], v[126:127]\n"
-      "v_pk_fma_f32 v[152:153], v[134:135], v[148:149], v[152:153]\n"
-      "v_pk_mul_f32 v[126:127], v[126:127], v[126:127]\n"
-      "v_pk_mul_f32 v[152:153], v[152:153], v[152:153]\n"
-      "v_pk_add_f32 v[124:125], v[124:125], v[126:127] neg_lo:[0,1] neg_hi:[0,1]\n"
-      "v_pk_add_f32 v[154:155], v[154:155], v[152:153] neg_lo:[0,1] neg_hi:[0,1]\n"
-      "v_pk_mul_f32 v[124:125], %[p2], v[124:125]\n"
-      "v_pk_mul_f32 v[154:155], %[maxa], v[154:155]\n"
-      "v_cvt_f64_f32_e32 v[130:131], v124\n"
-      "v_cvt_f64_f32_e32 v[132:133], v125\n"
-      "v_cvt_f64_f32_e32 v[134:135], v154\n"
-      "v_cvt_f64_f32_e32 v[136:137], v155\n"
-      "v_mul_f64 v[130:131], v[130:131], %[dt]\n"
-      "v_mul_f64 v[132:133], v[132:133], %[dt]\n"
-      "v_mul_f64 v[134:135], v[134:135], %[dt]\n"
-      "v_mul_f64 v[136:137], v[136:137], %[dt]\n"
-      "v_add_f64 v[130:131], v[118:119], v[130:131]\n"
-      "v_add_f64 v[132:133], v[138:139], v[132:133]\n"
-      "v_add_f64 v[134:135], v[118:119], v[134:135]\n"
-      "v_add_f64 v[136:137], v[138:139], v[136:137]\n"
-      "v_max_f64 v[130:131], v[130:131], %[zero]\n"
-      "v_max_f64 v[132:133], v[132:133], %[zero]\n"
-      "v_max_f64 v[134:135], v[134:135], %[fl0a]\n"
-      "v_max_f64 v[136:137], v[136:137], %[fl0b]\n"
-      "v_add_f64 v[130:131], v[130:131], -v[118:119]\n"
-      "v_add_f64 v[132:133], v[132:133], -v[138:139]\n"
-      "v_mul_f64 v[130:131], v[130:131], %[ramp]\n"
-      "v_mul_f64 v[132:133], v[132:133], %[ramp]\n"
-      "v_add_f64 v[130:131], v[118:119], v[130:131]\n"
-      "v_add_f64 v[132:133], v[138:139], v[132:133]\n"
-      "v_min_f64 v[130:131], v[130:131], v[134:135]\n"
-      "v_min_f64 v[132:133], v[132:133], v[136:137]\n"
-      "v_add_f64 v[134:135], v[118:119], %[adta]\n"
-      "v_add_f64 v[136:137], v[138:139], %[adtb]\n"
-      "v_min_f64 v[130:131], v[130:131], v[134:135]\n"
-      "v_min_f64 v[132:133], v[132:133], v[136:137]\n"
-      "v_add_f64 v[134:135], v[118:119], -%[ddta]\n"
-      "v_add_f64 v[136:137], v[138:139], -%[ddtb]\n"
-      "v_max_f64 v[118:119], v[130:131], v[134:135]\n"
-      "v_max_f64 v[138:139], v[132:133], v[136:137]\n"
-      "v_mul_f64 v[130:131], v[118:119], %[dt]\n"
-      "v_mul_f64 v[132:133], v[138:139], %[dt]\n"
-      "v_add_f64 v[130:131], v[114:115], v[130:131]\n"
-      "v_add_f64 v[132:133], v[116:117], v[132:133]\n"
-      "v_add_f64 v[134:135], v[130:131], -%[L]\n"
-      "v_add_f64 v[136:137], v[132:133], -%[L]\n"
-      "v_cvt_f32_f64_e32 v112, v[118:119]\n"
-      "v_cvt_f32_f64_e32 v113, v[138:139]\n"
-      "v_cmp_gt_i32_e64 %[sa], 0, v135\n"
-      "v_cmp_gt_i32_e64 %[sb], 0, v137\n"
-      "v_mul_f64 v[120:121], v[118:119], %[rcms]\n"
-      "v_mul_f64 v[122:123], v[138:139], %[rcms]\n"
-      "v_cndmask_b32_e64 v114, v134, v130, %[sa]\n"
-      "v_cndmask_b32_e64 v115, v135, v131, %[sa]\n"
-      "v_cndmask_b32_e64 v116, v136, v132, %[sb]\n"
-      "v_cndmask_b32_e64 v117, v137, v133, %[sb]\n"
-      "v_cvt_f32_f64_e32 v128, v[120:121]\n"
-      "v_cvt_f32_f64_e32 v129, v[122:123]\n"
-      : "+{v[112:113]}"(V32), "+{v[114:115]}"(XA), "+{v[116:117]}"(XB), "+{v[118:119]}"(VA), "+{v[138:139]}"(VB),
-        "+{v[140:141]}"(H), "+{v[142:143]}"(DVL), "={v[128:129]}"(OV), [sa] "=&s"(sa), [sb] "=&s"(sb)
-      : [c1e3] "v"(c.c1e3), [rcab] "v"(c.rc_ab), [tsab] "v"(c.tsab), [rcv0] "v"(c.rc_v0), [p0] "v"(c.p0),
-        [p1] "v"(c.p1), [p2] "v"(c.p2), [p5] "v"(c.p5), [one] "v"(c.one), [dt] "v"(c.dt), [ramp] "v"(c.ramp),
-        [L] "v"(c.L), [rcms] "v"(c.rc_ms), [zero] "v"(c.zero), [rcts] "v"(m.rc_ts), [ts] "v"(m.ts),
-        [rcsm] "v"(m.rc_smax), [smax] "v"(m.smax), [tau] "v"(m.tau), [mgap] "v"(m.min_gap), [maxa] "v"(m.maxa),
-        [fl0a] "v"(d.fl0a), [fl0b] "v"(d.fl0b), [adta] "v"(d.adta), [adtb] "v"(d.adtb), [ddta] "v"(d.ddta),
-        [ddtb] "v"(d.ddtb)
-      : "v120", "v121", "v122", "v123", "v124", "v125", "v126", "v127", "v130", "v131", "v132", "v133", "v134",
-        "v135", "v136", "v137", "v146", "v147", "v148", "v149", "v150", "v151", "v152", "v153", "v154", "v155");
-}
+#define FS_MIXED_A_NAME mixed_step_asm_a_sm
+#define FS_MIXED_A_NZ 0
+#define FS_MIXED_A_RL 0
+#define FS_MIXED_A_PARAM
+#include "flowsim_mixed_step_a_sm.inc"
+#undef FS_MIXED_A_NAME
+#undef FS_MIXED_A_NZ
+#undef FS_MIXED_A_RL
+#undef FS_MIXED_A_PARAM
 __device__ __forceinline__ void mixed_step_asm_b(f2& V32, double& XA, double& XB, f2& H, f2& DVL, f2& OX,
                                                  unsigned& crash_bits, float& sq, const MixedConsts& c) {
   unsigned long long sa, sb;
diff --git a/flow_amd/csrc/flowsim_pair_step_a_sm.inc b/flow_amd/csrc/flowsim_pair_step_a_sm.inc
--- a/flow_amd/csrc/flowsim_pair_step_a_sm.inc
+++ b/flow_amd/csrc/flowsim_pair_step_a_sm.inc
@@ -1,5 +1,5 @@
 __device__ __forceinline__ void FS_PAIR_A_NAME(f2& V, f2& X, f2& H, f2& DVL, f2& OX, const PairConsts& c,
-                                                const SumoPair& m FS_PAIR_A_NZ_PARAM) {
+                                                const SumoPair& m FS_PAIR_A_NZ_PARAM FS_PAIR_A_RL_PARAM) {
   unsigned long long sa, sb;
   asm volatile(
       "v_cmp_nlt_f32_e64 %[sa], |v116|, %[c1e3]\n"
@@ -64,10 +64,18 @@
 #if FS_PAIR_A_NZ
       "v_pk_add_f32 v[124:125], v[124:125], %[nz]\n"
 #endif
+#if FS_PAIR_A_RL
+      "v_cndmask_b32_e64 v124, v124, %[acta], %[rla]\n"
+      "v_cndmask_b32_e64 v125, v125, %[actb], %[rlb]\n"
+#endif
       "v_pk_mul_f32 v[124:125], v[124:125], %[dt2]\n"
       "v_pk_mul_f32 v[146:147], v[146:147], %[dt2]\n"
       "v_pk_add_f32 v[124:125], v[112:113], v[124:125]\n"
       "v_pk_add_f32 v[146:147], v[112:113], v[146:147]\n"
+#if FS_PAIR_A_RL
+      "v_max_f32_e32 v132, 0, v146\n"
+      "v_max_f32_e32 v133, 0, v147\n"
+#endif
       "v_max_f32_e32 v124, 0, v124\n"
       "v_max_f32_e32 v125, 0, v125\n"
       "v_max_f32_e32 v146, %[fl0], v146\n"
@@ -81,26 +89,45 @@
       "v_min_f32_e32 v125, v125, v147\n"
       "v_min_f32_e32 v124, v124, v144\n"
       "v_min_f32_e32 v125, v125, v145\n"
+#if FS_PAIR_A_RL
+      "v_max_f32_e32 v124, v124, v142\n"
+      "v_max_f32_e32 v125, v125, v143\n"
+      "v_cndmask_b32_e64 v112, v132, v124, %[cmda]\n"
+      "v_cndmask_b32_e64 v113, v133, v125, %[cmdb]\n"
+#else
       "v_max_f32_e32 v112, v124, v142\n"
       "v_max_f32_e32 v113, v125, v143\n"
+#endif
       "v_pk_mul_f32 v[124:125], v[112:113], %[dt2]\n"
       "v_pk_add_f32 v[124:125], v[114:115], v[124:125]\n"
       "v_pk_add_f32 v[126:127], v[124:125], %[L2] neg_lo:[0,1] neg_hi:[0,1]\n"
       "v_min_u32_e32 v114, v126, v124\n"
       "v_min_u32_e32 v115, v127, v125\n"
+#if !FS_PAIR_A_RL
       "v_pk_mul_f32 v[124:125], v[114:115], %[rcL2]\n"
       "v_pk_fma_f32 v[126:127], v[124:125], %[L2], v[114:115] neg_lo:[1,0,0] neg_hi:[1,0,0]\n"
       "v_pk_fma_f32 %[ox], v[126:127], %[rcL2], v[124:125]\n"
-      : "+{v[112:113]}"(V), "+{v[114:115]}"(X), "+{v[116:117]}"(H), "+{v[118:119]}"(DVL), [ox] "=&v"(OX),
+#endif
+      : "+{v[112:113]}"(V), "+{v[114:115]}"(X), "+{v[116:117]}"(H), "+{v[118:119]}"(DVL),
+#if !FS_PAIR_A_RL
+        [ox] "=&v"(OX),
+#endif
         [sa] "=&s"(sa), [sb] "=&s"(sb)
       : [c1e3] "v"(c.c1e3), [rcab] "v"(c.rc_ab), [tsab] "v"(c.tsab), [rcv0] "v"(c.rc_v0), [p0] "v"(c.p0),
         [p1] "v"(c.p1), [p2] "v"(c.p2), [p5] "v"(c.p5), [one] "v"(c.one), [dt2] "v"(c.dt2), [ramp2] "v"(c.ramp2),
-        [L2] "v"(c.L2), [rcL2] "v"(c.rc_L2), [rcts] "v"(m.rc_ts), [ts] "v"(m.ts), [rcsm] "v"(m.rc_smax),
+        [L2] "v"(c.L2),
+#if !FS_PAIR_A_RL
+        [rcL2] "v"(c.rc_L2),
+#endif
+        [rcts] "v"(m.rc_ts), [ts] "v"(m.ts), [rcsm] "v"(m.rc_smax),
         [smax] "v"(m.smax), [tau] "v"(m.tau), [mgap] "v"(m.min_gap), [maxa] "v"(m.maxa), [fl0] "v"(m.floor0.x),
         [fl1] "v"(m.floor0.y), [adt] "v"(m.adt), [ddt] "v"(m.ddt)
 #if FS_PAIR_A_NZ
         , [nz] "v"(nz)
 #endif
+#if FS_PAIR_A_RL
+        , [acta] "v"(act.x), [actb] "v"(act.y), [rla] "s"(rla), [rlb] "s"(rlb), [cmda] "s"(cmda), [cmdb] "s"(cmdb)
+#endif
       : "v120", "v121", "v122", "v123", "v124", "v125", "v126", "v127", "v130", "v131", "v132", "v133", "v134", "v135",
         "v138", "v139", "v140", "v141", "v142", "v143", "v144", "v145", "v146", "v147");
 }
diff --git a/flow_amd/csrc/flowsim_ringrl.h b/flow_amd/csrc/flowsim_ringrl.h
--- a/flow_amd/csrc/flowsim_ringrl.h
+++ b/flow_amd/csrc/flowsim_ringrl.h
@@ -11,8 +11,102 @@
   }
 }
 
-template <typename T, int ROW, bool NOISE, bool FAST>
+#define FS_RING_RL_PARAM , f2 act, unsigned long long rla, unsigned long long rlb, unsigned long long cmda, unsigned long long cmdb
+#define FS_PAIR_A_RL 1
+#define FS_PAIR_A_RL_PARAM FS_RING_RL_PARAM
+#define FS_PAIR_A_NAME ring_step_asm_a
+#define FS_PAIR_A_NZ 0
+#define FS_PAIR_A_NZ_PARAM
+#include "flowsim_pair_step_a_sm.inc"
+#undef FS_PAIR_A_NAME
+#undef FS_PAIR_A_NZ
+#undef FS_PAIR_A_NZ_PARAM
+#define FS_PAIR_A_NAME ring_step_asm_a_nz
+#define FS_PAIR_A_NZ 1
+#define FS_PAIR_A_NZ_PARAM , f2 nz
+#include "flowsim_pair_step_a_sm.inc"
+#undef FS_PAIR_A_NAME
+#undef FS_PAIR_A_NZ
+#undef FS_PAIR_A_NZ_PARAM
+#undef FS_PAIR_A_RL
+#undef FS_PAIR_A_RL_PARAM
+#define FS_MIXED_A_RL 1
+#define FS_MIXED_A_NAME ring_mixed_asm_a
+#define FS_MIXED_A_NZ 0
+#define FS_MIXED_A_PARAM FS_RING_RL_PARAM
+#include "flowsim_mixed_step_a_sm.inc"
+#undef FS_MIXED_A_NAME
+#undef FS_MIXED_A_NZ
+#undef FS_MIXED_A_PARAM
+#define FS_MIXED_A_NAME ring_mixed_asm_a_nz
+#define FS_MIXED_A_NZ 1
+#define FS_MIXED_A_PARAM , f2 nz FS_RING_RL_PARAM
+#include "flowsim_mixed_step_a_sm.inc"
+#undef FS_MIXED_A_NAME
+#undef FS_MIXED_A_NZ
+#undef FS_MIXED_A_PARAM
+#undef FS_MIXED_A_RL
+#undef FS_RING_RL_PARAM
+__device__ __forceinline__ void ring_snapshot_asm(f2& V, f2& X, f2& H, f2& DVL, f2& DG, float& VLY, f2 L2, f2 len_lead,
+                                                  unsigned long long last_mask) {
+  asm volatile(
+      "v_sub_f32_e32 v118, v112, v113\n"
+      "v_sub_f32_e32 v132, v115, v114\n"
+      "v_mov_b32_dpp v137, v112 row_shl:1 row_mask:0xf bank_mask:0xf bound_ctrl:1\n"
+      "v_mov_b32_dpp v136, v112 row_newbcast:0 row_mask:0xf bank_mask:0xf\n"
+      "v_sub_f32_dpp v133, v114, v115 row_shl:1 row_mask:0xf bank_mask:0xf bound_ctrl:1\n"
+      "v_sub_f32_dpp v135, v114, v115 row_newbcast:0 row_mask:0xf bank_mask:0xf\n"
+      "v_cndmask_b32_e64 v137, v137, v136, %[last]\n"
+      "v_cndmask_b32_e64 v133, v133, v135, %[last]\n"
+      "v_pk_add_f32 v[126:127], v[132:133], %[L2]\n"
+      "v_sub_f32_e32 v119, v113, v137\n"
+      "v_min_u32_e32 v132, v132, v126\n"
+      "v_min_u32_e32 v133, v133, v127\n"
+      "v_pk_add_f32 v[116:117], v[132:133], %[lenlead] neg_lo:[0,1] neg_hi:[0,1]\n"
+      : "+{v[112:113]}"(V), "+{v[114:115]}"(X), "={v[116:117]}"(H), "={v[118:119]}"(DVL), "={v[132:133]}"(DG),
+        "={v137}"(VLY)
+      : [L2] "v"(L2), [lenlead] "v"(len_lead), [last] "s"(last_mask)
+      : "v126", "v127", "v135", "v136");
+}
+__device__ __forceinline__ void ring_mixed_snapshot_asm(f2& V32, double& XA, double& XB, f2& H, f2& DVL, double& DGA,
+                                                        double& DGB, float& VLY, double L, double len_b, double len_next,
+                                                        unsigned long long last_mask) {
+  unsigned long long sa, sb;
+  asm volatile(
+      "v_sub_f32_e32 v142, v112, v113\n"
+      "v_mov_b32_dpp v125, v112 row_shl:1 row_mask:0xf bank_mask:0xf bound_ctrl:1\n"
+      "v_mov_b32_dpp v124, v112 row_newbcast:0 row_mask:0xf bank_mask:0xf\n"
+      "v_mov_b32_dpp v130, v114 row_shl:1 row_mask:0xf bank_mask:0xf bound_ctrl:1\n"
+      "v_mov_b32_dpp v131, v115 row_shl:1 row_mask:0xf bank_mask:0xf bound_ctrl:1\n"
+      "v_mov_b32_dpp v132, v114 row_newbcast:0 row_mask:0xf bank_mask:0xf\n"
+      "v_mov_b32_dpp v133, v115 row_newbcast:0 row_mask:0xf bank_mask:0xf\n"
+      "v_cndmask_b32_e64 v125, v125, v124, %[last]\n"
+      "v_cndmask_b32_e64 v130, v130, v132, %[last]\n"
+      "v_cndmask_b32_e64 v131, v131, v133, %[last]\n"
+      "v_add_f64 v[134:135], v[116:117], -v[114:115]\n"
+      "v_add_f64 v[136:137], v[130:131], -v[116:117]\n"
+      "v_sub_f32_e32 v143, v113, v125\n"
+      "v_cmp_gt_i32_e64 %[sa], 0, v135\n"
+      "v_cmp_gt_i32_e64 %[sb], 0, v137\n"
+      "v_add_f64 v[130:131], v[134:135], %[L]\n"
+      "v_add_f64 v[132:133], v[136:137], %[L]\n"
+      "v_cndmask_b32_e64 v134, v134, v130, %[sa]\n"
+      "v_cndmask_b32_e64 v135, v135, v131, %[sa]\n"
+      "v_cndmask_b32_e64 v136, v136, v132, %[sb]\n"
+      "v_cndmask_b32_e64 v137, v137, v133, %[sb]\n"
+      "v_add_f64 v[130:131], v[134:135], -%[lenb]\n"
+      "v_add_f64 v[132:133], v[136:137], -%[lennext]\n"
+      "v_cvt_f32_f64_e32 v140, v[130:131]\n"
+      "v_cvt_f32_f64_e32 v141, v[132:133]\n"
+      : "+{v[112:113]}"(V32), "+{v[114:115]}"(XA), "+{v[116:117]}"(XB), "={v[140:141]}"(H), "={v[142:143]}"(DVL),
+        "={v[134:135]}"(DGA), "={v[136:137]}"(DGB), "={v125}"(VLY), [sa] "=&s"(sa), [sb] "=&s"(sb)
+      : [L] "v"(L), [lenb] "v"(len_b), [lennext] "v"(len_next), [last] "s"(last_mask)
+      : "v124", "v130", "v131", "v132", "v133");
+}
+
+template <typename T, int ROW, bool NOISE, bool FAST, bool HAND = false>
 struct RingPairCore {
+  static_assert(!HAND || (ROW == 16 && FAST), "the hand-written step: rows of 16 lanes, exponent 4, the exact reciprocal divisions");
   static constexpr bool MIXED = sizeof(T) == 8;
   static constexpr int RPW = 64 / ROW;
   const DevView<T>& s;
@@ -35,6 +129,8 @@
   f2 x, v;
   double xdA = 0, xdB = 0, vdA = 0, vdB = 0;
   f2 h, vl;
+  f2 dvl = {0.0f, 0.0f};
+  unsigned long long last_mask = 0, rl_maskA = 0, rl_maskB = 0;
   f2 dgap = {0.0f, 0.0f};
   double dgA = 0, dgB = 0;
 
@@ -55,6 +151,11 @@
     iB = iA + 1;
     rlA = s.ctrl[iA] == FS_CTRL_RL;
     rlB = s.ctrl[iB] == FS_CTRL_RL;
+    if constexpr (HAND) {
+      last_mask = __ballot(last);
+      rl_maskA = __ballot(rlA);
+      rl_maskB = __ballot(rlB);
+    }
 #pragma unroll
     for (int q = 0; q < 6; ++q) p[q] = f2{float(s.p[q * N + iA]), float(s.p[q * N + iB])};
     {
@@ -86,9 +187,13 @@
     one = splat(1.0f);
     dt2 = splat(dt);
     ramp2 = splat(float(s.ramp));
+    if constexpr (HAND) {
+      asm volatile("" : "+v"(one), "+v"(dt2), "+v"(ramp2));
+    }
     gap2 = splat(float(s.crash_gap));
     dt64 = double(s.dt);
     ramp64 = double(s.ramp);
+    if constexpr (HAND && MIXED) asm volatile("" : "+v"(dt64), "+v"(ramp64));
     len_lead = f2{float(lenB), float(len_nextA)};
     {
       const int mA = s.speed_mode[iA], mB = s.speed_mode[iB];
@@ -154,6 +259,7 @@
   __device__ __forceinline__ void snapshot() {
     h = headway();
     vl = f2{v.y, next_a<ROW>(v.x, last, lane)};
+    if constexpr (HAND) dvl = pk_sub(v, vl);
   }
   __device__ __forceinline__ float clip(float a) const { return hmin(hmax(a, act_lo), act_hi); }
 
@@ -192,6 +298,10 @@
 
   template <bool LIVE_ALL>
   __device__ __forceinline__ void advance(bool live_in, bool have_act, float ownA, float ownB, f2 nz_in = f2{-0.0f, -0.0f}) {
+    if constexpr (HAND && LIVE_ALL) {
+      advance_hand(have_act, ownA, ownB, nz_in);
+      return;
+    }
     const bool live = LIVE_ALL ? true : live_in;
     f2 acc = idm_pair<FAST, FAST>(v, vl, h, p, two_sqrt_ab, rc_ab, rc_v0, one);
     if constexpr (NOISE) acc = pk_add(acc, LIVE_ALL ? nz_in : noise_term(live));
@@ -249,6 +359,31 @@
     snapshot();
   }
 
+  __device__ __forceinline__ void advance_hand(bool have_act, float ownA, float ownB, f2 nz) {
+    const f2 act = {clip(ownA), clip(ownB)};
+    const unsigned long long cmdA = have_act ? ~0ull : ~rl_maskA, cmdB = have_act ? ~0ull : ~rl_maskB;
+    float vly;
+    f2 unused;
+    if constexpr (MIXED) {
+      MixedConsts c{};
+      c.p0 = p[0]; c.p1 = p[1]; c.p2 = p[2]; c.p5 = p[5]; c.rc_v0 = rc_v0; c.tsab = two_sqrt_ab; c.rc_ab = rc_ab;
+      c.one = one; c.c1e3 = 1e-3f; c.dt = dt64; c.ramp = ramp64; c.L = L64; c.zero = 0.0;
+      const MixedSumoConsts d = {floor0A, floor0B, adtA, adtB, ddtA, ddtB};
+      if constexpr (NOISE) ring_mixed_asm_a_nz(v, xdA, xdB, vdA, vdB, h, dvl, unused, c, sc, d, nz, act, rl_maskA, rl_maskB, cmdA, cmdB);
+      else ring_mixed_asm_a(v, xdA, xdB, vdA, vdB, h, dvl, unused, c, sc, d, act, rl_maskA, rl_maskB, cmdA, cmdB);
+      ring_mixed_snapshot_asm(v, xdA, xdB, h, dvl, dgA, dgB, vly, L64, double(lenB), double(len_nextA), last_mask);
+    } else {
+      PairConsts c{};
+      c.p0 = p[0]; c.p1 = p[1]; c.p2 = p[2]; c.p5 = p[5]; c.rc_v0 = rc_v0; c.tsab = two_sqrt_ab; c.rc_ab = rc_ab;
+      c.one = one; c.dt2 = dt2; c.ramp2 = ramp2; c.L2 = L2; c.c1e3 = 1e-3f;
+      if constexpr (NOISE) ring_step_asm_a_nz(v, x, h, dvl, unused, c, sc, nz, act, rl_maskA, rl_maskB, cmdA, cmdB);
+      else ring_step_asm_a(v, x, h, dvl, unused, c, sc, act, rl_maskA, rl_maskB, cmdA, cmdB);
+      ring_snapshot_asm(v, x, h, dvl, dgap, vly, L2, len_lead, last_mask);
+    }
+    vl = f2{v.y, vly};
+    tcount += 1;
+  }
+
   __device__ __forceinline__ unsigned step_flags() const {
     const f2 hc = pk_sub(h, gap2), vb = pk_sub(v, f2{-100.0f, -100.0f});
     return ((__builtin_bit_cast(unsigned, hmin(hc.x, hc.y)) >> 31) | ((__builtin_bit_cast(unsigned, hmin(vb.x, vb.y)) >> 31) << 1)) &
@@ -275,16 +410,16 @@
   return bad ? 0.0f : reward;
 }
 
-template <typename T, int ROW, int HEAD, bool NOISE, bool FAST, bool MC = false>
-__global__ __launch_bounds__(256) void k_ring_pair(DevView<T> s, int num_steps_arg, const uint8_t* __restrict__ mask,
-                                                   const float* __restrict__ actions, size_t act_stride,
-                                                   float* __restrict__ obs, float* __restrict__ rew,
-                                                   uint8_t* __restrict__ done, int obs_every_step) {
+template <typename T, int ROW, int HEAD, bool NOISE, bool FAST, bool MC, bool HAND>
+__device__ __forceinline__ void ring_pair_kernel(const DevView<T>& s, int num_steps_arg, const uint8_t* __restrict__ mask,
+                                                 const float* __restrict__ actions, size_t act_stride,
+                                                 float* __restrict__ obs, float* __restrict__ rew,
+                                                 uint8_t* __restrict__ done, int obs_every_step) {
   constexpr bool MIXED = sizeof(T) == 8;
   constexpr bool WA = HEAD == 1 || HEAD == 2;
   constexpr bool MA = HEAD >= 2;
   static_assert(!(MA && MIXED), "the multi-agent heads exist in float32 only");
-  RingPairCore<T, ROW, NOISE, FAST> core(s);
+  RingPairCore<T, ROW, NOISE, FAST, HAND> core(s);
   const int lane = core.lane, k = core.k, N = core.N, rr = core.rr, iA = core.iA, iB = core.iB;
   const bool rvalid = core.rvalid, valid = core.valid, last = core.last, rlA = core.rlA, rlB = core.rlB;
   const bool live_replica = mask == nullptr || mask[rr] != 0;
@@ -515,7 +650,7 @@
         unsigned crash_bits = 0u, bad_bits = 0u;
         static_for<4>([&](auto slot_c) {
           constexpr int slot = decltype(slot_c)::value;
-          const float a = deep ? dpp<DPP_ROW_NEWBCAST0 + slot>(a_cur) : 0.0f;
+          const float a = dpp<DPP_ROW_NEWBCAST0 + slot>(a_cur);
           f2 nz = {-0.0f, -0.0f};
           if constexpr (NOISE) nz = core.template noise_of<slot>();
           const float oA = MC ? qA[slot] : a, oB = MC ? qB[slot] : a;
@@ -579,4 +714,21 @@
   if (valid && live_replica) core.store_state();
 }
 
+template <typename T, int ROW, int HEAD, bool NOISE, bool FAST, bool MC = false>
+__global__ __launch_bounds__(256) void k_ring_pair(DevView<T> s, int num_steps_arg, const uint8_t* __restrict__ mask,
+                                                   const float* __restrict__ actions, size_t act_stride,
+                                                   float* __restrict__ obs, float* __restrict__ rew,
+                                                   uint8_t* __restrict__ done, int obs_every_step) {
+  ring_pair_kernel<T, ROW, HEAD, NOISE, FAST, MC, false>(s, num_steps_arg, mask, actions, act_stride, obs, rew, done,
+                                                         obs_every_step);
 }
+template <typename T, int HEAD, bool NOISE, bool MC = false>
+__global__ __launch_bounds__(256) void k_ring_pair_hand(DevView<T> s, int num_steps_arg, const uint8_t* __restrict__ mask,
+                                                        const float* __restrict__ actions, size_t act_stride,
+                                                        float* __restrict__ obs, float* __restrict__ rew,
+                                                        uint8_t* __restrict__ done, int obs_every_step) {
+  ring_pair_kernel<T, 16, HEAD, NOISE, true, MC, true>(s, num_steps_arg, mask, actions, act_stride, obs, rew, done,
+                                                       obs_every_step);
+}
+
+}
diff --git a/flow_amd/csrc/flowsim_sim.h b/flow_amd/csrc/flowsim_sim.h
--- a/flow_amd/csrc/flowsim_sim.h
+++ b/flow_amd/csrc/flowsim_sim.h
@@ -90,6 +90,7 @@
   bool no_loop_kernel = false;
   bool no_loop_full = false;
   bool no_ring_rl = false;
+  bool no_ring_asm = false;
   bool no_queue = false;
   int* d_qflag = nullptr;
   bool qflag_armed = false;
```

After: 13.46 billion. 0.989x the previous value.
